# mikhaildubov/AST-text-analysis

Hardware: AMD Instinct MI355X
Metric: corpus chars/sec (SA+annotation build + keyphrase score table) (higher is better)
Workload: dtype u32 (symbols/indices) + f64 (scores); 1 GPU; 1 synthetic 64 MiB random-ASCII word-stream doc(s) per GPU (text mode), 1000 keyphrases, normalized scores, easa-HIP; symbols_per_gpu=61142967, strings_per_gpu=2982949, parallelism=doc-shard x1, all_gather_bytes_per_rank=0

## Files before the change

### ast-text-analysis_amd/csrc/alphabet.h

```cpp
#pragma once
#include "common.h"

#define TEXT_SYMBOLS EAST_HIP_TERMINATOR_START
#define PRESENT_WORDS (TEXT_SYMBOLS / 32)
#define TERM_TAG EAST_HIP_TERMINATOR_TAG
#define HI_SYMBOLS (0x110000u - TEXT_SYMBOLS)
#define HI_WORDS (HI_SYMBOLS / 32u)

__global__ __launch_bounds__(BLOCK) void presence_kernel(const u32 *__restrict__ sym, u32 n, int vec,
                                                         u32 *__restrict__ present)
{
    __shared__ u32 bits[PRESENT_WORDS];
    if (threadIdx.x < PRESENT_WORDS) bits[threadIdx.x] = 0;
    __syncthreads();
    auto mark = [&](u32 c) {
        if (c < TEXT_SYMBOLS && !(((volatile u32 *)bits)[c >> 5] & (1u << (c & 31u))))
            atomicOr(&bits[c >> 5], 1u << (c & 31u));
    };
    const u32 stride = gridDim.x * BLOCK;
    const u32 n4 = vec ? n >> 2 : 0u;
    u32 i = blockIdx.x * BLOCK + threadIdx.x;
    for (; i + 3u * stride < n4; i += 4u * stride) {
        const uint4 a = reinterpret_cast<const uint4 *>(sym)[i], b = reinterpret_cast<const uint4 *>(sym)[i + stride];
        const uint4 c = reinterpret_cast<const uint4 *>(sym)[i + 2u * stride], d = reinterpret_cast<const uint4 *>(sym)[i + 3u * stride];
        mark(a.x); mark(a.y); mark(a.z); mark(a.w);
        mark(b.x); mark(b.y); mark(b.z); mark(b.w);
        mark(c.x); mark(c.y); mark(c.z); mark(c.w);
        mark(d.x); mark(d.y); mark(d.z); mark(d.w);
    }
    for (; i < n4; i += stride) {
        const uint4 c = reinterpret_cast<const uint4 *>(sym)[i];
        mark(c.x); mark(c.y); mark(c.z); mark(c.w);
    }
    for (u32 i = (n4 << 2) + blockIdx.x * BLOCK + threadIdx.x; i < n; i += stride) mark(sym[i]);
    __syncthreads();
    if (threadIdx.x < PRESENT_WORDS && bits[threadIdx.x]) atomicOr(&present[threadIdx.x], bits[threadIdx.x]);
}

#define FLAG_CAPPED 0
#define FLAG_STATUS 1
#define FLAG_SIGMA 2
#define FLAG_KEEP 3
#define FLAG_FAIL 4
#define FLAG_SIGMA_HI 5
#define FLAG_PLACE_FAIL 6
#define FLAG_KG_BAD 7
#define FLAG_SAMPLE 8
#define FLAG_WORDS 32
#define STATUS_NO_TERMINATOR 1u
#define STATUS_N_STRINGS 2u
#define STATUS_SIGMA_GUESS 4u
#define STATUS_BAD_SYMBOL 8u
__device__ __forceinline__ void codemap_block(const u32 *__restrict__ present, u32 assumed, u32 *__restrict__ code_map,
                                              u32 *__restrict__ flags, u32 *__restrict__ guess, int check)
{
    if (guess && threadIdx.x < PRESENT_WORDS) {
        u32 *gp = guess + TEXT_SYMBOLS;
        if (check && gp[threadIdx.x] != present[threadIdx.x]) atomicOr(&flags[FLAG_STATUS], STATUS_SIGMA_GUESS);
        gp[threadIdx.x] = present[threadIdx.x];
    }
    static_assert(TEXT_SYMBOLS == BLOCK * 10, "ten code points per thread");
    __shared__ u32 lds4[WAVES_PER_BLOCK];
    const u32 c0 = threadIdx.x * 10u;
    u32 bits = 0, cnt = 0;
#pragma unroll
    for (u32 i = 0; i < 10; i++) {
        const u32 b = (present[(c0 + i) >> 5] >> ((c0 + i) & 31u)) & 1u;
        bits |= b << i;
        cnt += b;
    }
    u32 total;
    u32 run = block_exclusive_sum(cnt, lds4, total);
#pragma unroll
    for (u32 i = 0; i < 10; i++) {
        const u32 code = ((bits >> i) & 1u) ? ++run : 0u;
        code_map[c0 + i] = code;
        if (guess) guess[c0 + i] = code;
    }
    if (threadIdx.x == 0) {
        flags[FLAG_SIGMA] = total;
        u32 st = 0;
        if (assumed != 0xFFFFFFFFu && assumed != total) st |= STATUS_SIGMA_GUESS;
        if (st) atomicOr(&flags[FLAG_STATUS], st);
    }
}

__global__ __launch_bounds__(BLOCK) void validate_codemap_kernel(const u32 *__restrict__ sym, const u32 *__restrict__ doc_off,
                                                                 u32 n_docs, u32 tagged, const u32 *__restrict__ present,
                                                                 u32 assumed, u32 *__restrict__ code_map,
                                                                 u32 *__restrict__ flags, u32 *__restrict__ guess, int check)
{
    const u32 d = blockIdx.x * BLOCK + threadIdx.x;
    if (d < n_docs) {
        const u32 c = sym[doc_off[d + 1] - 1];
        if (tagged ? !(c >> 31) : c < TEXT_SYMBOLS) atomicOr(&flags[FLAG_STATUS], STATUS_NO_TERMINATOR);
    }
    if (blockIdx.x == 0) codemap_block(present, assumed, code_map, flags, guess, check);
}

#define SAMPLE_N 8192
// ... 256 lines not shown
```

### ast-text-analysis_amd/csrc/build.h

```cpp
#pragma once
#include "dc3.h"
#include "score.h"
#include "tables.h"
#include "upload.h"
#include <chrono>

static bool kgram_reserve(east_hip_index *h, u64 bins, u32 n_docs);

static void annotate(east_hip_index *h, Ctx &ctx, u32 *listed_total = nullptr)
{
    const Pyramid &pyr = h->pyr;
    const u32 n = pyr.len[0];
    Arena &ar = *ctx.arena;
    const size_t mark = ar.mark();
    const u32 n_tiles = ceil_div_u32(n, ANN_TILE);
    u32 *wide_list = ar.alloc<u32>((size_t)n_tiles * ANN_TILE);
    u32 *wide_count = ar.alloc<u32>(n_tiles);
    const bool has_lvl1 = pyr.levels > 1;
    const bool has_lvl2 = pyr.levels > 2;
    LAUNCH(ctx, ann_stream_kernel, n_tiles, pyr.ptr[0], (const u32 *)h->doc_off, (const u32 *)h->n_strings,
           h->build_docs, n, h->ann, has_lvl1 ? (u32 *)pyr.ptr[1] : (u32 *)nullptr, has_lvl1 ? pyr.len[1] : 0u,
           has_lvl1 ? pyr_padded(pyr.len[1]) : 0u, wide_list, wide_count, h->lcp,
           has_lvl2 ? (u32 *)pyr.ptr[2] : (u32 *)nullptr, has_lvl2 ? pyr.len[2] : 0u, has_lvl2 ? pyr_padded(pyr.len[2]) : 0u);
    int l = 3;
// ... 99 lines not shown
    ctx.ht_mean_len = h->ht_mean_len;
}

static void build_impl(east_hip_index *h, Ctx &ctx, const u32 *d_sym, u32 n, u32 n_docs,
                       const i64 *doc_offsets, const int32_t *n_strings, u32 spec_sigma = 0, bool tagged = false)
{
    Arena &ar = *ctx.arena;
    ar.release(0);
    h->s = ar.alloc<u32>((size_t)n + 3);
    h->s8 = ar.alloc<uint8_t>((size_t)n + 64);
    h->sa = ar.alloc<u32>(n);
    h->lcp = ar.alloc<u32>(pyr_padded(n));
    h->ann = ar.alloc<u32>(n);
    h->up = ar.alloc<u32>(n);
    h->down = ar.alloc<u32>(n);
    h->next = ar.alloc<u32>(n);
    h->doc_off = ar.alloc<u32>(2 * (size_t)n_docs + 1);
    h->n_strings = h->doc_off + n_docs + 1;
    constexpr size_t ZEROED_WORDS = FLAG_WORDS + PRESENT_WORDS + 1 + LCP_BUDGET_SLOTS, TOTAL_WORDS = (size_t)RS_TOTAL_SHARDS * RS_BINS;
    h->code_map = ar.alloc<u32>(TEXT_SYMBOLS + ZEROED_WORDS + 3 * TOTAL_WORDS);
    h->hi_bits = tagged ? ar.alloc<u32>(HI_WORDS) : nullptr;
    h->hi_rank = tagged ? ar.alloc<u32>(HI_WORDS) : nullptr;
    Pyramid pyr;
    pyr.levels = 1;
    pyr.ptr[0] = h->lcp;
    pyr.len[0] = n;
    while (pyr.len[pyr.levels - 1] > PYR_FAN) {
        if (pyr.levels >= PYR_MAX_LEVELS) east_throw(EAST_HIP_ERR_INTERNAL, "pyramid too deep");
        const u32 len = ceil_div_u32(pyr.len[pyr.levels - 1], PYR_FAN);
        pyr.ptr[pyr.levels] = ar.alloc<u32>(pyr_padded(len));
        pyr.len[pyr.levels] = len;
        pyr.levels++;
    }
    h->pyr = pyr;
    h->build_docs = n_docs;

    std::vector<u32> off32(2 * (size_t)n_docs + 1);
    u32 longest_doc = ctx.dry ? n : 0;
    if (!ctx.dry) {
        for (u32 d = 0; d <= n_docs; d++) off32[d] = (u32)doc_offsets[d];
        for (u32 d = 0; d < n_docs; d++) longest_doc = std::max(longest_doc, off32[d + 1] - off32[d]);
        for (u32 d = 0; d < n_docs; d++) off32[(size_t)n_docs + 1 + d] = (u32)n_strings[d];
        HIP_CHECK(hipMemcpyAsync(h->doc_off, off32.data(), off32.size() * 4, hipMemcpyHostToDevice, ctx.stream));
    }

    const u32 gn = ceil_div_u32(n, BLOCK);
    u32 sigma_t = TEXT_SYMBOLS - 1, m_total = n;
    u32 sigma_hi = tagged ? HI_SYMBOLS : 0;
    u32 *flags = h->code_map + TEXT_SYMBOLS;
    u32 *capped = flags + FLAG_CAPPED, *status = flags + FLAG_STATUS;
    u32 *present = flags + FLAG_WORDS;
    if (!ctx.dry) HIP_CHECK(hipMemsetAsync(flags, 0, (ZEROED_WORDS + 3 * TOTAL_WORDS) * sizeof(u32), ctx.stream));
    ctx.zeroed_totals = ctx.dry ? nullptr : flags + ZEROED_WORDS + TOTAL_WORDS;
    RsFirstHist first_hist;
    ctx.first_hist = nullptr;
    const Ctx::FirstPassPlan fp = ctx.spec && ctx.knobs.first_hist && n_docs == 1 && !tagged ? h->first_plan : Ctx::FirstPassPlan();
    if (ctx.dry || fp.valid) {
        first_hist.n = n;
        first_hist.n_tiles = ceil_div_u32(n, RS_TILE);
        first_hist.n_groups = ceil_div_u32(first_hist.n_tiles, RS_GROUP);
        first_hist.hist = ar.alloc<u32>((size_t)RS_BINS * first_hist.n_tiles);
        first_hist.group_sum = ar.alloc<u32>((size_t)RS_BINS * first_hist.n_groups);
        first_hist.digit_total = flags + ZEROED_WORDS;
    }
    ctx.lcp_budget.slots = ctx.dry ? nullptr : present + PRESENT_WORDS + 1;
    ctx.lcp_budget.per_slot = std::max<u32>(n / 256u / LCP_BUDGET_SLOTS, 4u);
    ctx.spec_out = flags + FLAG_KEEP;
    ctx.zeroed_word = ctx.dry ? nullptr : flags + FLAG_PLACE_FAIL;
    ctx.spec_fail = flags + FLAG_PLACE_FAIL;
    ctx.kg_bad = ctx.dry ? nullptr : flags + FLAG_KG_BAD;
    {
        const size_t mark = ar.mark();
        u32 *term_ex = ar.alloc<u32>((size_t)n + 1);
        const int vec = ((uintptr_t)d_sym & 15u) == 0;
        const bool fused = ctx.spec && vec && h->guess.p;
        ctx.map_checked = fused && !ctx.dry;
        if (fused && fp.valid && !ctx.dry) {
            first_hist.s8 = h->s8;
            first_hist.key_bytes = fp.key_bytes; first_hist.w = fp.w; first_hist.b = fp.b; first_hist.spare = fp.spare;
            first_hist.term_first = fp.term_first; first_hist.shift = fp.shift; first_hist.mask = fp.mask;
            if (fp.key_bytes == 8)
                LAUNCH_NAMED(ctx, "presence_remap_hist_kernel", (presence_remap_hist_kernel<u64, TextWindowGen<u64>>), first_hist.n_groups,
                             d_sym, n, h->guess.as<const u32>(), present, h->s8,
                             TextWindowGen<u64>{h->s8, n, fp.w, fp.b, fp.spare, fp.term_first, DocKey()}, fp.shift, fp.mask,
                             first_hist.n_tiles, first_hist.hist, first_hist.group_sum, first_hist.digit_total);
            else
                LAUNCH_NAMED(ctx, "presence_remap_hist_kernel", (presence_remap_hist_kernel<u32, TextWindowGen<u32>>), first_hist.n_groups,
                             d_sym, n, h->guess.as<const u32>(), present, h->s8,
                             TextWindowGen<u32>{h->s8, n, fp.w, fp.b, fp.spare, fp.term_first, DocKey()}, fp.shift, fp.mask,
                             first_hist.n_tiles, first_hist.hist, first_hist.group_sum, first_hist.digit_total);
            ctx.first_hist = &first_hist;
        } else if (fused) LAUNCH(ctx, presence_remap_kernel, std::min<u32>(gn, 2048), d_sym, n, h->guess.as<const u32>(), present, h->s8);
        else LAUNCH(ctx, presence_kernel, std::min<u32>(gn, 2048), d_sym, n, vec, present);
        if (tagged) {
            if (!ctx.dry) HIP_CHECK(hipMemsetAsync(h->hi_bits, 0, HI_WORDS * 4, ctx.stream));
            LAUNCH_BLOCK(ctx, presence_hi_kernel, std::min<u32>(ceil_div_u32(n, PRESENCE_HI_THREADS), 256), PRESENCE_HI_THREADS,
                         d_sym, n, h->hi_bits, status);
            LAUNCH(ctx, hi_rank_kernel, 1, (const u32 *)h->hi_bits, h->hi_rank, flags);
        }
        LAUNCH(ctx, validate_codemap_kernel, ceil_div_u32(n_docs, BLOCK), d_sym, (const u32 *)h->doc_off, n_docs, (u32)tagged,
               (const u32 *)present, ctx.spec ? spec_sigma : 0xFFFFFFFFu, h->code_map, flags, h->guess.as<u32>(), (int)fused);
        ctx.sample_n = 0;
        ctx.rep_n = ctx.rep_dup = 0;
        bool sample_plans = false;
        if (!ctx.dry && !ctx.spec && !tagged && n >= 1024u) {
            u32 dl = 0;
            for (u32 d = 1; d < n_docs; d++)
                if (off32[d + 1] - off32[d] > off32[dl + 1] - off32[dl]) dl = d;
            const u32 len = off32[dl + 1] - off32[dl], cnt = std::min<u32>(SAMPLE_N, len);
            sample_plans = n >= 4 * SAMPLE_N && cnt >= SAMPLE_N / 4;
            if (cnt >= 512u)
                LAUNCH_BLOCK(ctx, sample_prefix_kernel, SAMPLE_MAX_L, SAMPLE_THREADS, d_sym, n, off32[dl] + (len - cnt) / 2, cnt,
                             flags + FLAG_SAMPLE);
        }
        if (!ctx.dry) {
            if (ctx.spec) {
                sigma_t = spec_sigma;
            } else {
                u32 hf[FLAG_WORDS];
                HIP_CHECK(hipMemcpyAsync(hf, flags, sizeof(hf), hipMemcpyDeviceToHost, ctx.stream));
                HIP_CHECK(sync_stream(ctx.stream));
                if (hf[FLAG_STATUS] & STATUS_NO_TERMINATOR)
                    east_throw(EAST_HIP_ERR_DOMAIN, tagged ? "a document does not end in a (tagged) string terminator"
                                                           : "a document does not end in a string terminator (>= U+0A00)");
                if (hf[FLAG_STATUS] & STATUS_BAD_SYMBOL)
                    east_throw(EAST_HIP_ERR_DOMAIN, "a symbol is neither a tagged terminator nor a code point < U+110000");
                sigma_t = hf[FLAG_SIGMA];
                sigma_hi = tagged ? hf[FLAG_SIGMA_HI] : 0;
                ctx.sample_n = hf[FLAG_SAMPLE + 2 * SAMPLE_MAX_L];
                for (int l = 1; l <= SAMPLE_MAX_L; l++) {
                    ctx.sample_dup2[l] = hf[FLAG_SAMPLE + 2 * (l - 1)];
                    ctx.sample_dup4[l] = hf[FLAG_SAMPLE + 2 * (l - 1) + 1];
                }
                ctx.rep_n = ctx.sample_n;
                ctx.rep_dup = ctx.sample_dup4[SAMPLE_MAX_L];
                if (!sample_plans) ctx.sample_n = 0;
                if (g_trace && ctx.sample_n) {
                    fprintf(stderr, "[east_hip] sample of %u suffixes, shared prefixes (>= 2 / >= 4 of the sample) by length:", ctx.sample_n);
                    for (int l = 1; l <= SAMPLE_MAX_L; l++) fprintf(stderr, " %d: %u/%u", l, ctx.sample_dup2[l], ctx.sample_dup4[l]);
                    fprintf(stderr, "\n");
                }
            }
// ... 261 lines not shown
    }
    if (sym_on_host) {
        staging = (u32 *)(h->arena.base + (h->arena.cap - (((size_t)n * 4 + 255) & ~(size_t)255)));
        int went = 0;
        if (narrow) {
            static const bool no_bytes = getenv("EAST_HIP_NO_SYMBOL_BYTES") != nullptr;
            bool bytes = !no_bytes && !h->bytes_refused;
            for (u32 i = 0; bytes && i < std::min<u32>(n, 65536u); i++) bytes = sym[i] < 0xFFu || sym[i] >= TEXT_SYMBOLS;
            if (bytes && upload_symbols_narrow<uint8_t>(h, sym, n, staging, (uint8_t *)((char *)staging - narrow_bytes))) went = 2;
            else {
                if (bytes) h->bytes_refused = true;
                (void)upload_symbols_narrow<uint16_t>(h, sym, n, staging, (uint16_t *)((char *)staging - narrow_bytes));
                went = 1;
            }
        } else HIP_CHECK(hipMemcpyAsync(staging, sym, (size_t)n * 4, hipMemcpyHostToDevice, h->stream));
        h->narrow_upload = went;
        sym = staging;
    } else h->narrow_upload = 0;
    h->stats = Stats();
    h->arena.high = 0;
    Ctx ctx = handle_ctx(h, &h->arena, &h->stats);
    ctx.knobs = kn;
    ctx.lean = lean;
    u32 flags[FLAG_WORDS] = {0};
    auto run = [&](bool spec, bool spec_rounds) -> bool {
        ctx.spec = spec;
        ctx.spec_rounds = spec && spec_rounds;
        ctx.plan_wide = spec ? h->plan_wide : -1;
        ctx.plan_fused = spec ? h->plan_fused : -1;
        ctx.plan_ht = spec ? h->plan_ht : -1;
        ctx.plan_persist = spec ? h->plan_persist : -1;
        ctx.did_first = Ctx::FirstPassPlan();
        try {
            build_impl(h, ctx, sym, n, (u32)n_docs, doc_offsets, n_strings, h->hint_sigma, tagged);
        } catch (const SpecAbort &) {
            HIP_CHECK(hipStreamSynchronize(h->stream));
            return false;
        } catch (const EastError &) {
            if (!spec) throw;
            (void)hipStreamSynchronize(h->stream);
            return false;
        }
        HIP_CHECK(hipEventRecord(h->ev1, h->stream));
        HIP_CHECK(hipMemcpyAsync(flags, h->code_map + TEXT_SYMBOLS, sizeof(flags), hipMemcpyDeviceToHost, h->stream));
        HIP_CHECK(sync_stream(h->stream));
        return true;
    };
    HIP_CHECK(hipEventRecord(h->ev0, h->stream));
    const bool speculate = kn.speculate && kn.window_sort && h->hint_valid && h->hint_window && h->hint_sigma <= 254 && !tagged;
    const bool spec_rounds = speculate && h->hint_no_rounds;
    const bool went_through = run(speculate, spec_rounds);
    const bool repeat = speculate && (!went_through || (flags[FLAG_STATUS] & STATUS_SIGMA_GUESS) ||
                                      (spec_rounds && (flags[FLAG_KEEP] || flags[FLAG_FAIL] || flags[FLAG_PLACE_FAIL])));
    if (repeat) {
        if (g_trace) fprintf(stderr, "[east_hip] speculative build guessed wrong: building again\n");
        h->stats = Stats();
        run(false, false);
    }
    const bool map_confirmed = speculate && !repeat && ctx.map_checked;
    const u32 status = flags[FLAG_STATUS];
    if (status & STATUS_NO_TERMINATOR)
        east_throw(EAST_HIP_ERR_DOMAIN, "a document does not end in a string terminator (>= U+0A00)");
    if (flags[FLAG_CAPPED] && !(status & STATUS_N_STRINGS)) {
        finish_capped_lcp(h, ctx);
        HIP_CHECK(hipEventRecord(h->ev1, h->stream));
        HIP_CHECK(hipStreamSynchronize(h->stream));
    }
    if (status & STATUS_N_STRINGS)
        east_throw(EAST_HIP_ERR_DOMAIN, tagged ? "n_strings does not match the tagged terminators found in a document"
                                               : "n_strings does not match the terminators found in a document "
                                                 "(text symbols must be < U+0A00 unless the terminators are tagged)");
    if (flags[FLAG_KG_BAD]) h->kg_marked = false;
    h->hint_valid = !tagged || h->sigma_hi == 0;
    h->hint_sigma = h->sigma_t;
    h->hint_window = h->stats.window_sorted != 0;
    h->plan_wide = h->stats.window_sorted ? ctx.did_wide : -1;
    if (ctx.did_wide && h->stats.first_n > 0 && h->stats.first_kept * 50 < h->stats.first_n) h->plan_wide = -1;
    h->plan_fused = h->stats.window_sorted ? ctx.did_fused : -1;
    h->plan_ht = h->stats.window_sorted ? ctx.did_ht : -1;
    h->plan_persist = h->stats.window_sorted ? ctx.did_persist : -1;
    if (h->stats.first_n > 0 && ((ctx.did_fused && h->stats.first_kept * 20 > h->stats.first_n) ||
                                 (!ctx.did_fused && h->stats.first_kept * 50 < h->stats.first_n)))
        h->plan_fused = -1;
    h->first_plan = h->stats.window_sorted && h->plan_wide >= 0 && h->plan_fused >= 0 ? ctx.did_first : Ctx::FirstPassPlan();
    h->hint_no_rounds = h->stats.window_sorted && h->stats.refine_rounds == 0 && !h->stats.long_repeats;
    h->prof.collect();
    HIP_CHECK(hipEventElapsedTime(&h->last_build_ms, h->ev0, h->ev1));
    h->n = n;
    if (h->n_docs != (u32)n_docs) h->n_kp = 0;
    h->n_docs = (u32)n_docs;
    h->h_doc_off.assign(doc_offsets, doc_offsets + n_docs + 1);
    h->h_n_strings.assign(n_strings, n_strings + n_docs);
    if (map_confirmed) h->map_epoch = map_epoch_before;
    h->built = true;
    ring_pin_later(h);
}
```

### ast-text-analysis_amd/csrc/common.h

```cpp
#pragma once

#include <hip/hip_runtime.h>
#include <stdint.h>
#include <stdio.h>
#include <stdlib.h>
#include <algorithm>
#include <mutex>
#include <string>
#include <type_traits>
#include <vector>

typedef uint32_t u32;
typedef uint64_t u64;
typedef int64_t i64;

#include "../../include/east_hip.h"

#define LCP_DIRECT_CAP (1u << 14)
#define LCP_SOFT_CAP 256u
#define LCP_PARTIAL_BIT 0x80000000u
#define LCP_BUDGET_SLOTS 64u
struct LcpBudget {
    u32 *slots = nullptr;
    u32 per_slot = 0;
// ... 36 lines not shown
        off = end;
        if (off > high) high = off;
        return dry ? (void *)(uintptr_t)(0x1000 + a) : (void *)(base + a);
    }
    template <class T> T *alloc(size_t count) { return (T *)alloc_bytes(count * sizeof(T)); }
};

struct DevBuf {
    char *p = nullptr;
    size_t cap = 0;
    bool try_ensure(size_t bytes, hipStream_t drain = nullptr)
    {
        if (bytes <= cap) return true;
        if (drain) HIP_CHECK(hipStreamSynchronize(drain));
        release();
        void *q = nullptr;
        if (hipMalloc(&q, bytes) != hipSuccess) { (void)hipGetLastError(); return false; }
        p = (char *)q;
        cap = bytes;
        return true;
    }
    void ensure(size_t bytes, const char *what, hipStream_t drain = nullptr)
    {
        if (!try_ensure(bytes, drain))
            east_throw(EAST_HIP_ERR_OOM, "hipMalloc of " + std::to_string(bytes) + " bytes for " + what + " failed");
    }
    void release()
    {
        if (p) (void)hipFree(p);
        p = nullptr;
        cap = 0;
    }
    template <class T> T *as() const { return (T *)p; }
    Arena arena() const
    {
        Arena a;
        a.base = p;
        a.cap = cap;
        return a;
    }
};

struct Stats {
    i64 levels = 0, levels_resolved = 0, refine_rounds = 0, window_sorted = 0, merge_elems = 0, radix_passes = 0, radix_elems = 0, radix_elem_bytes = 0;
    i64 radix_elems_u32 = 0, radix_elems_u64 = 0, radix_passes_u32 = 0, radix_passes_u64 = 0;
    i64 long_repeats = 0;
    i64 lds_sorted = 0;
    i64 first_kept = 0, first_n = 0;
    i64 fused_finish = 0;
    i64 ht_keys = 0;
    i64 seg_sort = 0;
    i64 persist_rounds = 0;
    i64 first_hist_fused = 0;
};

struct Profiler {
    struct Rec { const char *name; hipEvent_t e0, e1; };
    struct Sum { std::string name; i64 count; double ms; };
    std::vector<Rec> recs;
    std::vector<hipEvent_t> pool;
    std::vector<Sum> sums;
    bool enabled = false;
    std::string only;
    bool skipped = false;

    hipEvent_t get()
    {
        if (!pool.empty()) { hipEvent_t e = pool.back(); pool.pop_back(); return e; }
        hipEvent_t e;
        if (hipEventCreate(&e) != hipSuccess) east_throw(EAST_HIP_ERR_HIP, "hipEventCreate failed");
        return e;
    }
    void begin(const char *name, hipStream_t st)
    {
        skipped = !only.empty() && only != name;
        if (skipped) return;
        Rec r{name, get(), get()};
        (void)hipEventRecord(r.e0, st);
        recs.push_back(r);
    }
    void end(hipStream_t st)
    {
        if (!skipped) (void)hipEventRecord(recs.back().e1, st);
    }
    void collect()
    {
        for (auto &r : recs) {
            float ms = 0.f;
            (void)hipEventElapsedTime(&ms, r.e0, r.e1);
            bool found = false;
            for (auto &s : sums)
                if (s.name == r.name) { s.count++; s.ms += ms; found = true; break; }
            if (!found) sums.push_back(Sum{r.name, 1, ms});
            pool.push_back(r.e0);
            pool.push_back(r.e1);
        }
        recs.clear();
    }
    void reset() { collect(); sums.clear(); }
    ~Profiler()
    {
        for (auto &r : recs) { (void)hipEventDestroy(r.e0); (void)hipEventDestroy(r.e1); }
        for (auto e : pool) (void)hipEventDestroy(e);
    }
};

#define SCORE_SCRATCH_BYTES ((size_t)1 << 30)
#define SCORE_GRID_BLOCKS ((u64)1 << 22)
#define TP_RING_SLOT ((size_t)8 << 20)
static int env_int(const char *name, int absent) { const char *v = getenv(name); return v ? atoi(v) : absent; }
struct Knobs {
    bool window_sort = true;
    bool force_lean = false;
    bool force_wide_keys = getenv("EAST_HIP_WIDE_KEYS") != nullptr;
    bool fused_finish = getenv("EAST_HIP_NO_FUSED_FINISH") == nullptr;
    bool force_fused = getenv("EAST_HIP_FORCE_FUSED") != nullptr;
    int ht_mode = env_int("EAST_HIP_HT", -1);
    int seg_mode = env_int("EAST_HIP_SEG", -1);
    bool lds_rounds = getenv("EAST_HIP_NO_LDS_ROUNDS") == nullptr;
    bool fused_classify = getenv("EAST_HIP_NO_FUSED_CLASSIFY") == nullptr;
    bool persist = getenv("EAST_HIP_NO_PERSIST") == nullptr;
    bool persist_large = getenv("EAST_HIP_NO_PERSIST_LARGE") == nullptr;
    bool persist_force_large = getenv("EAST_HIP_PERSIST_FORCE_LARGE") != nullptr;
    int persist_max_wgs = env_int("EAST_HIP_PERSIST_WGS", 0);
    size_t rank_bucket_bytes = (size_t)192 << 20;
    bool speculate = getenv("EAST_HIP_NO_SPECULATION") == nullptr;
    bool first_hist = getenv("EAST_HIP_NO_FIRST_HIST") == nullptr;
    bool kg_pairs = getenv("EAST_HIP_NO_KG_PAIRS") == nullptr;
    bool kg_pairs_forced = false;
    bool score_fused = getenv("EAST_HIP_SCORE_UNFUSED") == nullptr;
    int score_endgame = env_int("EAST_HIP_SCORE_ENDGAME", 1);
    size_t score_scratch_bytes = SCORE_SCRATCH_BYTES;
    u64 score_grid_blocks = SCORE_GRID_BLOCKS;
    i64 tp_stream = getenv("EAST_HIP_TEXT_STREAM") ? atoll(getenv("EAST_HIP_TEXT_STREAM")) : -1;
    int tp_ring = env_int("EAST_HIP_TEXT_RING", -1);
    size_t tp_ring_slot = getenv("EAST_HIP_RING_SLOT") ? std::min<size_t>(TP_RING_SLOT, (size_t)std::max(64, atoi(getenv("EAST_HIP_RING_SLOT")))) : TP_RING_SLOT;
    int term_hash_bits = 0;
    int syn_chunk = 128;
    int top_tile = 64;
    i64 related_chunk = 0;
    i64 cosine_texts_batch = 0;
    u32 plan_epoch = 1;
};
static Knobs g_knobs;
static std::mutex g_knobs_mutex;
static inline Knobs knobs_snapshot()
{
    std::lock_guard<std::mutex> lock(g_knobs_mutex);
    return g_knobs;
}
template <class F> static inline void knobs_update(F f)
{
    std::lock_guard<std::mutex> lock(g_knobs_mutex);
    f(g_knobs);
}

struct Ctx {
    Knobs knobs = knobs_snapshot();
    hipStream_t stream = nullptr;
    Arena *arena = nullptr;
    bool dry = false;
    bool lean = false;
    bool spec = false;
    bool spec_rounds = false;
    u32 *spec_out = nullptr;
    bool map_checked = false;
    u32 *spec_fail = nullptr;
    u32 *zeroed_word = nullptr;
    u32 *zeroed_totals = nullptr;
    const struct RsFirstHist *first_hist = nullptr;
    struct FirstPassPlan {
        bool valid = false;
        int key_bytes = 0, w = 0, b = 0, spare = 0, shift = 0;
        u32 term_first = 0, mask = 0;
    } did_first;
    u32 *kg_bad = nullptr;
    u32 sample_n = 0, sample_dup2[9] = {0}, sample_dup4[9] = {0};
    u32 rep_n = 0, rep_dup = 0;
    int plan_wide = -1, plan_fused = -1;
    int did_wide = 0, did_fused = 0;
    const u32 *ht_enc = nullptr;
    const uint16_t *ht_dec = nullptr;
    int ht_max_len = 0;
    double ht_mean_len = 0.0;
    int plan_ht = -1, did_ht = 0;
    int plan_persist = -1, did_persist = 0;
    int did_seg = 0;
    std::vector<u32> seg_host;
    LcpBudget lcp_budget;
    Stats *stats = nullptr;
    Profiler *prof = nullptr;
};

static bool g_spin_sync = getenv("EAST_HIP_NO_SPIN_SYNC") == nullptr;
static inline hipError_t sync_stream(hipStream_t stream)
{
    if (g_spin_sync) {
        bool waited = false;
        for (int i = 0; i < 20000; i++) {
            const hipError_t e = hipStreamQuery(stream);
            if (e == hipSuccess) {
                if (waited) (void)hipGetLastError();
                return hipSuccess;
            }
            if (e != hipErrorNotReady) return e;
            waited = true;
        }
        (void)hipGetLastError();
    }
    return hipStreamSynchronize(stream);
}

static inline u32 ceil_div_u32(u64 a, u64 b) { return (u32)((a + b - 1) / b); }
static inline int bit_width_u32(u32 x) { int b = 0; while (x) { b++; x >>= 1; } return b; }

#define LAUNCH(ctx, kernel, grid, ...) LAUNCH_NAMED(ctx, #kernel, kernel, grid, __VA_ARGS__)

#define LAUNCH_NAMED(ctx, name, kernel, grid, ...)                                         \
    do {                                                                                   \
        if (!(ctx).dry) {                                                                  \
            const bool _p = (ctx).prof && (ctx).prof->enabled;                             \
            if (_p) (ctx).prof->begin(name, (ctx).stream);                                 \
            hipLaunchKernelGGL(kernel, dim3(grid), dim3(BLOCK), 0, (ctx).stream, __VA_ARGS__); \
            HIP_CHECK(hipGetLastError());                                                  \
            if (_p) (ctx).prof->end((ctx).stream);                                         \
        }                                                                                  \
    } while (0)

// ... 117 lines not shown
```

### ast-text-analysis_amd/csrc/debug_api.h

```cpp
#pragma once

struct DebugScope {
    hipStream_t stream = nullptr;
    Arena arena;
    Stats stats;
    Ctx ctx;
    DebugScope(int device, size_t bytes)
    {
        int c = 0;
        if (hipGetDeviceCount(&c) != hipSuccess || c <= 0)
            east_throw(EAST_HIP_ERR_NO_DEVICE, "no HIP device available (this library has no CPU fallback)");
        if (device < 0 || device >= c) east_throw(EAST_HIP_ERR_NO_DEVICE, "device ordinal out of range");
        use_device_ordinal(device);
        HIP_CHECK(hipStreamCreateWithFlags(&stream, hipStreamNonBlocking));
        void *p = nullptr;
        HIP_CHECK(hipMalloc(&p, bytes));
        arena.base = (char *)p;
        arena.cap = bytes;
        ctx.stream = stream;
        ctx.arena = &arena;
        ctx.stats = &stats;
    }
    ~DebugScope()
    {
// ... 125 lines not shown
    if (!lcp || !doc_off || !n_strings || !up_out || !down_out || !next_out || !left_out || !geometry_out || !listed_out ||
        n64 < 1 || n64 >= (i64)0x7FFFFFF0 || n_docs < 1 || doc_off[0] != 0 || doc_off[n_docs] != n64)
        east_throw(EAST_HIP_ERR_INVALID, "bad child table arguments");
    for (int32_t d = 0; d < n_docs; d++) {
        if (doc_off[d + 1] <= doc_off[d] || doc_off[d + 1] > n64) east_throw(EAST_HIP_ERR_INVALID, "document offsets must increase");
        if (lcp[doc_off[d]] != 0) east_throw(EAST_HIP_ERR_INVALID, "the table must hold 0 at a document's first rank: it bounds the searches");
    }
    for (i64 k = 0; k < n64; k++)
        if (lcp[k] > 0x7FFFFFEFu) east_throw(EAST_HIP_ERR_INVALID, "a value above 0x7FFFFFEF: an LCP value is below n");
    const u32 n = (u32)n64;
    DebugScope sc(device, ((size_t)pyr_padded(n) * 6 + (size_t)n / 8 + (size_t)ceil_div_u32(n, ANN_TILE) * (ANN_TILE + 1) +
                           (size_t)ceil_div_u32(n, CH_TILE) * (CH_TILE + 1) + 2 * (size_t)n_docs) * 4 + (1u << 20));
    Arena &ar = sc.arena;
    east_hip_index h;
    h.up = ar.alloc<u32>(n);
    h.down = ar.alloc<u32>(n);
    h.next = ar.alloc<u32>(n);
    u32 *left = ar.alloc<u32>(n);
    for (u32 *t : {h.up, h.down, h.next, left}) HIP_CHECK(hipMemsetAsync(t, 0xEE, (size_t)n * 4, sc.stream));
    debug_table_handle(sc, h, lcp, n, doc_off, n_docs, n_strings);
    annotate(&h, sc.ctx);
    child_tables(&h, sc.ctx, listed_out);
    for (int32_t d = 0; d < n_docs; d++)
        interval_lefts(&h, sc.ctx, (u32)doc_off[d], (u32)(doc_off[d + 1] - doc_off[d]), left + doc_off[d]);
    HIP_CHECK(hipMemcpyAsync(up_out, h.up, (size_t)n * 4, hipMemcpyDeviceToHost, sc.stream));
    HIP_CHECK(hipMemcpyAsync(down_out, h.down, (size_t)n * 4, hipMemcpyDeviceToHost, sc.stream));
    HIP_CHECK(hipMemcpyAsync(next_out, h.next, (size_t)n * 4, hipMemcpyDeviceToHost, sc.stream));
    HIP_CHECK(hipMemcpyAsync(left_out, left, (size_t)n * 4, hipMemcpyDeviceToHost, sc.stream));
    HIP_CHECK(hipStreamSynchronize(sc.stream));
    geometry_out[0] = CH_TILE;
    geometry_out[1] = CH_HALO;
    geometry_out[2] = CH_NEAR;
    geometry_out[3] = CH_LOCAL;
}

extern "C" {

int east_hip_debug_set_rank_bucket_bytes(int64_t bytes)
{
    if (bytes < 0) return EAST_HIP_ERR_INVALID;
    knobs_update([&](Knobs &k) { k.rank_bucket_bytes = (size_t)bytes; k.plan_epoch++; });
    return EAST_HIP_OK;
}

int east_hip_debug_set_window_sort(int enabled)
{
    knobs_update([&](Knobs &k) {
    k.window_sort = enabled != 0;
    k.force_lean = enabled == 2;
    k.force_wide_keys = enabled == 3 || enabled == 5;
    k.fused_finish = enabled != 4 && enabled != 5 && enabled != 9 && getenv("EAST_HIP_NO_FUSED_FINISH") == nullptr;
    k.force_fused = enabled == 6 || getenv("EAST_HIP_FORCE_FUSED") != nullptr;
    k.ht_mode = enabled == 7 || enabled == 9 ? 1 : enabled == 8 ? 0 : env_int("EAST_HIP_HT", -1);
    k.plan_epoch++;
    });
    return EAST_HIP_OK;
}

int east_hip_debug_set_segmented_sort(int mode)
{
    knobs_update([&](Knobs &k) { k.seg_mode = mode < 0 ? env_int("EAST_HIP_SEG", -1) : (mode != 0); k.plan_epoch++; });
    return EAST_HIP_OK;
}

int east_hip_debug_alphabetic_code(const uint64_t *weights, int32_t n, uint32_t *code, int32_t *len)
{
    if (!weights || !code || !len || n < 1) return EAST_HIP_ERR_INVALID;
    std::vector<u64> w(weights, weights + n);
    std::vector<u32> c;
    std::vector<int> l;
    if (!ht_build_code(w, c, l)) return EAST_HIP_ERR_DOMAIN;
    for (int i = 0; i < n; i++) { code[i] = c[i]; len[i] = l[i]; }
    return EAST_HIP_OK;
}

int east_hip_debug_narrow_symbols(const uint32_t *symbols, int64_t n, uint16_t *out, int vector)
{
    if (!symbols || !out || n < 0) return EAST_HIP_ERR_INVALID;
    if (vector) narrow_symbols(symbols, out, (size_t)n);
    else
        for (int64_t i = 0; i < n; i++) out[i] = symbols[i] < TEXT_SYMBOLS ? (uint16_t)symbols[i] : (uint16_t)SYM_TERMINATOR16;
    return vector && g_have_avx2 ? 1 : EAST_HIP_OK;
}

int east_hip_debug_narrow_symbols8(const uint32_t *symbols, int64_t n, uint8_t *out, int vector)
{
    if (!symbols || !out || n < 0) return EAST_HIP_ERR_INVALID;
    bool ok = true;
    if (vector) ok = narrow_symbols8(symbols, out, (size_t)n);
    else
        for (int64_t i = 0; i < n; i++) { const u32 c = symbols[i]; ok &= !(c >= 0xFFu && c < TEXT_SYMBOLS); out[i] = c < 0xFFu ? (uint8_t)c : (uint8_t)0xFFu; }
    return (ok ? 1 : 0) + (vector && g_have_avx2 ? 2 : 0);
}

int east_hip_debug_set_lds_rounds(int enabled)
{
    knobs_update([&](Knobs &k) {
        k.lds_rounds = enabled != 0;
        k.fused_classify = enabled != 2 && getenv("EAST_HIP_NO_FUSED_CLASSIFY") == nullptr;
        k.persist = enabled == 1 && getenv("EAST_HIP_NO_PERSIST") == nullptr;
    });
    return EAST_HIP_OK;
}

int east_hip_debug_set_persist(int force_large, int max_workgroups)
{
// ... 151 lines not shown
```

### ast-text-analysis_amd/csrc/east_hip.hip

```cpp
#include "common.h"
#include "alphabet.h"
#include "handle.h"
#include "consumer.h"
#include "upload.h"
#include "build.h"
#include "textfront.h"
#include "score_host.h"
#include <string.h>

static thread_local std::string g_last_error;

template <class F> static int guarded(F f)
{
    int rc = EAST_HIP_OK;
    try {
        f();
    } catch (const EastError &e) {
        g_last_error = e.msg;
        rc = e.code;
    } catch (const std::exception &e) {
        g_last_error = e.what();
        rc = EAST_HIP_ERR_INTERNAL;
    }
    restore_device();
// ... 256 lines not shown
        h->arena.release(mark);
    });
}

int east_hip_reset(east_hip_handle_t h)
{
    return guarded([&] {
        if (!h) east_throw(EAST_HIP_ERR_INVALID, "null handle");
        use_device(h);
        HIP_CHECK(hipStreamSynchronize(h->stream));
        h->built = false;
        h->table_scored = false;
        h->n = 0;
        h->n_docs = 0;
        h->n_kp = 0;
        h->n_q = 0;
        h->q_code_epoch = 0;
        h->kg_built = false;
        h->child_built = false;
        h->prep_n = 0;
        h->prep_doc_off.clear();
        h->prep_n_strings.clear();
        h->prep_tagged = false;
        h->tagged_input = false;
        h->sigma_hi = 0;
        h->prof.enabled = false;
        h->prof.only.clear();
        h->plan_wide = h->plan_fused = h->plan_ht = h->plan_persist = -1;
        h->first_plan = Ctx::FirstPassPlan();
        h->ht_valid = false;
        h->stats = Stats();
        const size_t keep = (size_t)64 << 20;
        for (DevBuf *b : h->bufs)
            if (b->cap > keep) b->release();
        for (Consumer *c : h->consumers)
            if (c) c->reset();
    });
}

int east_hip_synchronize(east_hip_handle_t h)
{
    return guarded([&] {
        if (!h) east_throw(EAST_HIP_ERR_INVALID, "null handle");
        use_device(h);
        HIP_CHECK(hipStreamSynchronize(h->stream));
    });
}

void *east_hip_stream(east_hip_handle_t h) { return h ? (void *)h->stream : nullptr; }

int east_hip_build_info(east_hip_handle_t h, int64_t *out, int32_t cap)
{
    if (!h || !out) return EAST_HIP_ERR_INVALID;
    const int64_t v[28] = {h->n, h->n_docs, h->m_total, h->sigma_t, h->bits0, h->stats.levels,
                           (int64_t)h->arena.cap, (int64_t)h->arena.high, h->stats.radix_passes,
                           h->stats.radix_elems, h->stats.radix_elem_bytes, h->stats.radix_passes_u32,
                           h->stats.radix_elems_u32, h->stats.radix_passes_u64, h->stats.radix_elems_u64,
                           h->stats.levels_resolved, h->stats.merge_elems, h->stats.refine_rounds,
                           h->stats.window_sorted, h->stats.lds_sorted, h->stats.fused_finish, h->stats.first_kept,
                           h->stats.first_n, h->stats.ht_keys, h->stats.seg_sort, h->narrow_upload,
                           h->stats.persist_rounds, h->stats.first_hist_fused};
    for (int i = 0; i < 28 && i < cap; i++) out[i] = v[i];
    return 28;
}

int east_hip_profile_enable(east_hip_handle_t h, int on)
{
    if (!h) return EAST_HIP_ERR_INVALID;
    return guarded([&] {
        use_device(h);
        HIP_CHECK(hipStreamSynchronize(h->stream));
        h->prof.reset();
        h->prof.enabled = on != 0;
    });
}

int east_hip_profile_only(east_hip_handle_t h, const char *kernel)
{
    if (!h) return EAST_HIP_ERR_INVALID;
    h->prof.only = kernel ? kernel : "";
    return EAST_HIP_OK;
}

int64_t east_hip_profile_report(east_hip_handle_t h, char *buf, int64_t cap)
{
    if (!h || !buf || cap < 1) return EAST_HIP_ERR_INVALID;
    int cur = -1;
    (void)hipGetDevice(&cur);
    (void)hipSetDevice(h->device);
    (void)hipStreamSynchronize(h->stream);
    h->prof.collect();
    if (cur >= 0 && cur != h->device) (void)hipSetDevice(cur);
    std::string out;
    for (auto &s : h->prof.sums) {
        char line[256];
        snprintf(line, sizeof(line), "%s\t%lld\t%.6f\n", s.name.c_str(), (long long)s.count, s.ms);
        out += line;
    }
    const int64_t nb = (int64_t)out.size() < cap - 1 ? (int64_t)out.size() : cap - 1;
    memcpy(buf, out.data(), (size_t)nb);
    buf[nb] = 0;
    return (int64_t)out.size();
}

int64_t east_hip_plan_arena_bytes(int64_t n_total, int32_t n_docs)
{
    if (n_total < 1 || n_total >= (i64)0x7FFFFFF0 || n_docs < 1) return EAST_HIP_ERR_INVALID;
    int64_t r = EAST_HIP_ERR_INTERNAL;
    guarded([&] { r = (int64_t)plan_arena_bytes((u32)n_total, (u32)n_docs); });
    return r;
}

int64_t east_hip_plan_arena_bytes_lean(int64_t n_total, int32_t n_docs)
{
    if (n_total < 1 || n_total >= (i64)0x7FFFFFF0 || n_docs < 1) return EAST_HIP_ERR_INVALID;
    int64_t r = EAST_HIP_ERR_INTERNAL;
// ... 21 lines not shown
```

### ast-text-analysis_amd/csrc/persist_rounds.h

```cpp
#pragma once
#include "lds_group_sort.h"

#define PR_MAX_ROUNDS 40
#define PR_CTL_BARRIER 0
#define PR_CTL_BAIL 1
#define PR_CTL_ROUNDS 2
#define PR_CTL_ABORT 3
#define PR_CTL_OPEN 8
#ifdef PR_STAMPS
#define PR_CTL_STAMPS (PR_CTL_OPEN + PR_MAX_ROUNDS)
#define PR_CTL_WORDS (PR_CTL_STAMPS + 2 * 8 * PR_MAX_ROUNDS)
#define PR_STAMP(k) do { if (blockIdx.x == 0 && threadIdx.x == 0) ((unsigned long long *)(a.ctl + PR_CTL_STAMPS))[round * 8 + (k)] = wall_clock64(); } while (0)
#else
#define PR_CTL_WORDS (PR_CTL_OPEN + PR_MAX_ROUNDS)
#define PR_STAMP(k) do { } while (0)
#endif
#ifndef PR_FENCE_MODE
#define PR_FENCE_MODE 3
#endif
#define PR_SPIN_LIMIT (1u << 20)

struct PrArgs {
    const u32 *elems, *gstart, *slots;
    u32 m;
    u32 depth;
    int name_bits;
    u32 *name0, *name1;
    u32 *order_g;
    u32 *lcp_hint;
    u32 *ctl;
};

__global__ __launch_bounds__(BLOCK) void persist_names_init_kernel(const u32 *__restrict__ order_g, const u32 *__restrict__ alt,
                                                                   const u64 *__restrict__ keep, u32 n,
                                                                   u32 *__restrict__ name0, u32 *__restrict__ name1)
{
    const u32 i = blockIdx.x * BLOCK + threadIdx.x;
    if (i >= n) return;
    const u32 e = alt && ((keep[i >> 6] >> (i & 63u)) & 1u) ? alt[i] : order_g[i];
    name0[e] = i;
    name1[e] = i;
}

__device__ __forceinline__ void pr_store(u32 *p, u32 v) { __hip_atomic_store(p, v, __ATOMIC_RELAXED, __HIP_MEMORY_SCOPE_AGENT); }
__device__ __forceinline__ u32 pr_load(const u32 *p) { return __hip_atomic_load(p, __ATOMIC_RELAXED, __HIP_MEMORY_SCOPE_AGENT); }

__device__ __forceinline__ bool pr_grid_barrier(u32 *ctl, u32 index, u32 *lds_flag)
{
    asm volatile("s_waitcnt vmcnt(0)" ::: "memory");
    __syncthreads();
    if (threadIdx.x == 0) {
#if PR_FENCE_MODE & 2
        __builtin_amdgcn_fence(__ATOMIC_RELEASE, "agent");
        asm volatile("s_waitcnt vmcnt(0)" ::: "memory");
#endif
        __hip_atomic_fetch_add(&ctl[PR_CTL_BARRIER], 1u, __ATOMIC_RELAXED, __HIP_MEMORY_SCOPE_AGENT);
        const u32 target = gridDim.x * index;
        u32 spins = 0, ok = 1;
        while (__hip_atomic_load(&ctl[PR_CTL_BARRIER], __ATOMIC_RELAXED, __HIP_MEMORY_SCOPE_AGENT) < target) {
            __builtin_amdgcn_s_sleep(4);
            if ((++spins & 63u) == 0u && __hip_atomic_load(&ctl[PR_CTL_ABORT], __ATOMIC_RELAXED, __HIP_MEMORY_SCOPE_AGENT)) { ok = 0; break; }
            if (spins > PR_SPIN_LIMIT) {
                __hip_atomic_store(&ctl[PR_CTL_ABORT], 1u, __ATOMIC_RELAXED, __HIP_MEMORY_SCOPE_AGENT);
                ok = 0;
                break;
            }
        }
#if PR_FENCE_MODE & 1
        __builtin_amdgcn_fence(__ATOMIC_ACQUIRE, "agent");
        asm volatile("s_waitcnt vmcnt(0)" ::: "memory");
#endif
        *lds_flag = ok;
    }
    __syncthreads();
    return *lds_flag != 0u;
}

__device__ __forceinline__ u32 pr_group_start(const u64 *bits, u32 local)
{
    u32 wi = local >> 6;
    u64 x = bits[wi] & (((u64)2 << (local & 63u)) - 1ull);
    while (!x) x = bits[--wi];
    return wi * 64u + 63u - (u32)__builtin_clzll(x);
}

template <int MIN_WAVES>
__global__ __launch_bounds__(LG_THREADS, MIN_WAVES) void refine_persist_kernel(PrArgs a)
{
    __shared__ LgLds lds;
    __shared__ u32 bar_flag, wg_count;
    const u32 lane = lane_id(), w = wave_id();
    const u32 base = blockIdx.x * LG_CHUNK;
// ... 528 lines not shown
```

### ast-text-analysis_amd/csrc/radix_sort.h

```cpp
#pragma once
#include "common.h"
#include "alphabet.h"
#include "scan.h"

#define RS_THREADS 1024
#ifndef RS_IPT
#define RS_IPT 4
#endif
#define RS_TILE (RS_THREADS * RS_IPT)
#define RS_DB 8
#define RS_BINS 256
#ifndef RS_GROUP
#define RS_GROUP 8
#endif
#define RS_HIST_THREADS 256
#ifndef RS_TOTAL_SHARDS
#define RS_TOTAL_SHARDS 8
#endif

#define RS_SEG_MAX_DOCS 65535
struct RsSeg {
    const u32 *group_doc = nullptr;
    const u32 *doc_group0 = nullptr;
    const u32 *doc_off = nullptr;
    u32 n_docs = 0;
    u32 n_groups = 0;
    u32 shards = 1;
    const u32 *big_docs = nullptr;
    u32 n_big = 0;
};
#define RS_SPINE_DOC_GROUPS 64
__device__ __forceinline__ void rs_tile_range(const RsSeg &seg, u32 n, u32 tile, u32 &base, u32 &count)
{
    if (!seg.n_docs) {
        base = tile * (u32)RS_TILE;
        count = n - base < (u32)RS_TILE ? n - base : (u32)RS_TILE;
        return;
    }
    const u32 d = seg.group_doc[tile / RS_GROUP];
    const u32 t_in = tile - seg.doc_group0[d] * RS_GROUP;
    const u32 end = seg.doc_off[d + 1];
    base = seg.doc_off[d] + t_in * (u32)RS_TILE;
    count = base < end ? (end - base < (u32)RS_TILE ? end - base : (u32)RS_TILE) : 0u;
}

template <class K> struct PairSrc {
    static constexpr int MODE = 0;
    const K *keys;
    const u32 *vals;
    __device__ __forceinline__ K key(u32 i) const { return keys[i]; }
    __device__ __forceinline__ u32 val(u32 i) const { return vals[i]; }
};

template <bool CHECK = true> __device__ __forceinline__ void radix_hist_add(u32 *mine, u32 digit)
{
    if constexpr (!CHECK) { atomicAdd(&mine[digit], 1u); return; }
    const u32 first = __builtin_amdgcn_readfirstlane(digit);
    const u64 active = __ballot(1);
    if (__ballot(digit == first) == active) {
        if (digit == first && lane_id() == (u32)(__ffsll((unsigned long long)active) - 1))
            atomicAdd(&mine[first], (u32)__popcll(active));
    } else {
        atomicAdd(&mine[digit], 1u);
    }
}

#ifndef RS_HIST_BATCH
#define RS_HIST_BATCH 8
#endif
#ifndef RS_HIST_COPIES
#define RS_HIST_COPIES 2
#endif
template <class K, class Src, bool CHECK = true>
__global__ __launch_bounds__(RS_HIST_THREADS) void radix_hist_kernel(Src src, u32 n, int shift, u32 mask, u32 n_tiles,
                                                                     u32 *__restrict__ hist, u32 *__restrict__ group_sum,
                                                                     u32 *__restrict__ digit_total, RsSeg seg)
{
    constexpr int UW = RS_HIST_THREADS / WAVE;
    static_assert(RS_HIST_THREADS == RS_BINS, "thread d owns digit d");
    __shared__ u32 bins[RS_GROUP][RS_HIST_COPIES][RS_BINS];
    if constexpr (Src::MODE == 2) src.prepare();
#pragma unroll
    for (int k = 0; k < RS_GROUP; k++)
#pragma unroll
        for (int c = 0; c < RS_HIST_COPIES; c++) bins[k][c][threadIdx.x] = 0;
    __syncthreads();
    const u32 g = blockIdx.x, lane = lane_id();
    const u32 t0 = g * RS_GROUP, t1 = t0 + RS_GROUP < n_tiles ? t0 + RS_GROUP : n_tiles;
    for (u32 tile = t0 + wave_id(); tile < t1; tile += UW) {
        u32 *mine = bins[tile - t0][lane & (RS_HIST_COPIES - 1)];
        u32 base, count;
        rs_tile_range(seg, n, tile, base, count);
        if (count == 0) continue;
        if constexpr (Src::MODE == 0) {
            constexpr u32 PER = 16 / sizeof(K);
            constexpr int LOADS = RS_TILE / (WAVE * PER);
            static_assert(LOADS % RS_HIST_BATCH == 0, "batches of loads");
            if (count == (u32)RS_TILE) {
                const char *p = reinterpret_cast<const char *>(src.keys + base) + 16u * lane;
                for (int j0 = 0; j0 < LOADS; j0 += RS_HIST_BATCH) {
                    uint4 q[RS_HIST_BATCH];
#pragma unroll
                    for (int j = 0; j < RS_HIST_BATCH; j++) __builtin_memcpy(&q[j], p + (size_t)(j0 + j) * WAVE * 16u, 16);
                    __builtin_amdgcn_sched_barrier(0);
#pragma unroll
                    for (int j = 0; j < RS_HIST_BATCH; j++) {
                        if constexpr (sizeof(K) == 8) {
                            const u64 ka = ((u64)q[j].y << 32) | q[j].x, kb = ((u64)q[j].w << 32) | q[j].z;
                            radix_hist_add<CHECK>(mine, (u32)(ka >> shift) & mask);
                            radix_hist_add<CHECK>(mine, (u32)(kb >> shift) & mask);
                        } else {
                            radix_hist_add<CHECK>(mine, (u32)(q[j].x >> shift) & mask);
                            radix_hist_add<CHECK>(mine, (u32)(q[j].y >> shift) & mask);
                            radix_hist_add<CHECK>(mine, (u32)(q[j].z >> shift) & mask);
                            radix_hist_add<CHECK>(mine, (u32)(q[j].w >> shift) & mask);
                        }
                    }
                }
            } else {
                for (u32 i = lane; i < count; i += WAVE) radix_hist_add<CHECK>(mine, (u32)(src.keys[base + i] >> shift) & mask);
            }
        } else if constexpr (Src::MODE == 1) {
            for (u32 i = lane; i < count; i += WAVE) radix_hist_add<CHECK>(mine, (u32)(src.key(base + i) >> shift) & mask);
        } else {
            src.template hist_tile<CHECK>(mine, base, base + count, shift, mask);
        }
    }
    syncthreads_after_lds_atomics();
    u32 run = 0;
#pragma unroll
    for (int k = 0; k < RS_GROUP; k++) {
        if (t0 + k < t1) hist[(size_t)(t0 + k) * RS_BINS + threadIdx.x] = run;
#pragma unroll
        for (int c = 0; c < RS_HIST_COPIES; c++) run += bins[k][c][threadIdx.x];
    }
    group_sum[(size_t)g * RS_BINS + threadIdx.x] = run;
    const u32 row = seg.n_docs ? seg.group_doc[g] * seg.shards + g % seg.shards : g % RS_TOTAL_SHARDS;
    if (run) atomicAdd(&digit_total[(size_t)row * RS_BINS + threadIdx.x], run);
}

#define RS_FIRST_HALO 16u
#ifndef RS_FIRST_PARTS
#define RS_FIRST_PARTS 2
#endif
#define RS_GEN_RUN 8
struct RsFirstHist {
    u32 *hist = nullptr, *group_sum = nullptr, *digit_total = nullptr;
    const uint8_t *s8 = nullptr;
    u32 n = 0, n_tiles = 0, n_groups = 0;
    int key_bytes = 0, w = 0, b = 0, spare = 0;
    u32 term_first = 0;
    int shift = 0;
    u32 mask = 0;
};
template <class Gen> static inline bool rs_first_hist_counted_for(const RsFirstHist &, const Gen &) { return false; }

template <class K, class Gen>
__global__ __launch_bounds__(RS_HIST_THREADS) void presence_remap_hist_kernel(const u32 *__restrict__ sym, u32 n,
                                                                              const u32 *__restrict__ guess, u32 *__restrict__ present,
                                                                              uint8_t *__restrict__ s8, Gen gen, int shift, u32 mask,
                                                                              u32 n_tiles, u32 *__restrict__ hist,
                                                                              u32 *__restrict__ group_sum, u32 *__restrict__ digit_total)
{
    constexpr int UW = RS_HIST_THREADS / WAVE;
    constexpr int PARTS = RS_FIRST_PARTS, SUB = RS_TILE / PARTS;
    constexpr int LOADS = SUB / (WAVE * 4);
    static_assert(SUB * PARTS == RS_TILE && SUB % (WAVE * RS_GEN_RUN) == 0, "stretches of whole runs for every lane");
    static_assert(RS_HIST_THREADS == RS_BINS, "thread d owns digit d");
    static_assert(RS_TILE % (WAVE * RS_GEN_RUN) == 0 && RS_FIRST_HALO % 4 == 0 && RS_FIRST_HALO / 4 <= WAVE, "whole runs, a halo of whole words");
    __shared__ u32 bins[RS_GROUP][RS_HIST_COPIES][RS_BINS];
    __shared__ __attribute__((aligned(16))) u32 tab[TEXT_SYMBOLS / 2];
    __shared__ __attribute__((aligned(16))) u32 bytes[UW][(SUB + RS_FIRST_HALO) / 4];
    typedef uint16_t __attribute__((may_alias)) tab16_t;
    const tab16_t *tab16 = reinterpret_cast<const tab16_t *>(tab);
#pragma unroll
    for (int k = 0; k < RS_GROUP; k++)
#pragma unroll
        for (int c = 0; c < RS_HIST_COPIES; c++) bins[k][c][threadIdx.x] = 0;
    {
        static_assert(TEXT_SYMBOLS % 4 == 0, "whole 16-byte groups");
        constexpr u32 GROUPS = TEXT_SYMBOLS / 4, ROUNDS = (GROUPS + RS_HIST_THREADS - 1) / RS_HIST_THREADS;
        uint4 q[ROUNDS];
#pragma unroll
        for (u32 r = 0; r < ROUNDS; r++) {
            const u32 g = threadIdx.x + r * RS_HIST_THREADS;
            q[r] = reinterpret_cast<const uint4 *>(guess)[g < GROUPS ? g : 0u];
        }
#pragma unroll
        for (u32 r = 0; r < ROUNDS; r++) {
            const u32 g = threadIdx.x + r * RS_HIST_THREADS;
            if (g < GROUPS)
                reinterpret_cast<uint2 *>(tab)[g] = uint2{(q[r].x & 0xFFu) | ((q[r].y & 0xFFu) << 16), (q[r].z & 0xFFu) | ((q[r].w & 0xFFu) << 16)};
        }
    }
    __syncthreads();
    auto mark = [&](u32 c) {
        if (c < TEXT_SYMBOLS) atomicOr(&tab[c >> 1], 0x100u << (16u * (c & 1u)));
    };
    auto word = [&](const uint4 q) -> u32 {
        const u32 vx = tab16[q.x < TEXT_SYMBOLS ? q.x : 0u], vy = tab16[q.y < TEXT_SYMBOLS ? q.y : 0u];
        const u32 vz = tab16[q.z < TEXT_SYMBOLS ? q.z : 0u], vw = tab16[q.w < TEXT_SYMBOLS ? q.w : 0u];
        const u32 bx = q.x < TEXT_SYMBOLS ? vx : 0x1FFu, by = q.y < TEXT_SYMBOLS ? vy : 0x1FFu;
        const u32 bz = q.z < TEXT_SYMBOLS ? vz : 0x1FFu, bw = q.w < TEXT_SYMBOLS ? vw : 0x1FFu;
        if (!(bx & by & bz & bw & 0x100u)) { mark(q.x); mark(q.y); mark(q.z); mark(q.w); }
        return (bx & 0xFFu) | ((by & 0xFFu) << 8) | ((bz & 0xFFu) << 16) | (bw << 24);
    };
    auto code = [&](u32 c) -> u32 {
        if (c >= TEXT_SYMBOLS) return 0xFFu;
        const u32 v = tab16[c];
        if (!(v & 0x100u)) mark(c);
        return v & 0xFFu;
    };
    auto word_slow = [&](u32 g) -> u32 {
        u32 v = 0;
#pragma unroll
        for (u32 k = 0; k < 4; k++) {
            const u64 p = (u64)g * 4u + k;
            if (p < n) v |= code(sym[p]) << (8u * k);
        }
        return v;
    };
    const u32 g = blockIdx.x, lane = lane_id(), n4 = n >> 2;
    const u32 t0 = g * RS_GROUP, t1 = t0 + RS_GROUP < n_tiles ? t0 + RS_GROUP : n_tiles;
    u32 *mine_bytes = bytes[wave_id()];
    u32 *out = reinterpret_cast<u32 *>(s8);
    uint4 q[LOADS];
    auto request = [&](u32 tile, u32 part) {
        const u32 g0 = tile * (u32)(RS_TILE / 4) + part * (u32)(SUB / 4) + lane;
#pragma unroll
        for (int j = 0; j < LOADS; j++) {
            const u32 gi = g0 + (u32)j * WAVE;
            q[j] = gi < n4 ? reinterpret_cast<const uint4 *>(sym)[gi] : uint4{0u, 0u, 0u, 0u};
        }
    };
    u32 tile = t0 + wave_id(), part = 0;
    if (tile < t1) request(tile, 0);
    while (tile < t1) {
        const u32 g0 = tile * (u32)(RS_TILE / 4) + part * (u32)(SUB / 4) + lane;
        const u32 base = tile * (u32)RS_TILE + part * (u32)SUB;
        const u32 count = base < n ? (n - base < (u32)SUB ? n - base : (u32)SUB) : 0u;
#pragma unroll
        for (int j = 0; j < LOADS; j++) {
            const u32 gi = g0 + (u32)j * WAVE;
            u32 v;
            if (gi < n4) { v = word(q[j]); out[gi] = v; }
            else v = word_slow(gi);
            mine_bytes[(u32)j * WAVE + lane] = v;
        }
        if (lane < RS_FIRST_HALO / 4u) {
            const u32 gi = (base + (u32)SUB) / 4u + lane;
            u32 v = 0;
#pragma unroll
            for (u32 k = 0; k < 4; k++) {
                const u64 p = (u64)gi * 4u + k;
                if (p < n) { const u32 c = sym[p]; v |= (c < TEXT_SYMBOLS ? (u32)tab16[c] & 0xFFu : 0xFFu) << (8u * k); }
            }
            mine_bytes[SUB / 4 + lane] = v;
        }
        const u32 next_part = part + 1u < (u32)PARTS ? part + 1u : 0u, next_tile = next_part ? tile : tile + UW;
        if (next_tile < t1) request(next_tile, next_part);
        __builtin_amdgcn_sched_barrier(0);
        __builtin_amdgcn_fence(__ATOMIC_RELEASE, "wavefront");
        __builtin_amdgcn_wave_barrier();
        __builtin_amdgcn_fence(__ATOMIC_ACQUIRE, "wavefront");
        u32 *mine = bins[tile - t0][lane & (RS_HIST_COPIES - 1)];
        for (u32 r0 = lane * RS_GEN_RUN; r0 < count; r0 += WAVE * RS_GEN_RUN) {
            u32 x[6];
            K k[RS_GEN_RUN];
            const uint2 a = *reinterpret_cast<const uint2 *>(&mine_bytes[r0 / 4]), c = *reinterpret_cast<const uint2 *>(&mine_bytes[r0 / 4 + 2]);
            const uint2 e = *reinterpret_cast<const uint2 *>(&mine_bytes[r0 / 4 + 4]);
            x[0] = a.x; x[1] = a.y; x[2] = c.x; x[3] = c.y; x[4] = e.x; x[5] = e.y;
            gen.keys_of_run(x, k);
#pragma unroll
            for (int qq = 0; qq < RS_GEN_RUN; qq++)
                if (r0 + qq < count) radix_hist_add<false>(mine, (u32)(k[qq] >> shift) & mask);
        }
        __builtin_amdgcn_fence(__ATOMIC_RELEASE, "wavefront");
        __builtin_amdgcn_wave_barrier();
        tile = next_tile;
        part = next_part;
    }
    if (blockIdx.x == 0 && threadIdx.x < 20u) {
        const u32 j = (n4 << 2) + threadIdx.x;
        if (j < n) { const u32 c = sym[j]; s8[j] = (uint8_t)(c < TEXT_SYMBOLS ? (u32)tab16[c] & 0xFFu : 0xFFu); }
        else if (j < n + 16u) s8[j] = 0;
    }
    syncthreads_after_lds_atomics();
    u32 run = 0;
#pragma unroll
    for (int k = 0; k < RS_GROUP; k++) {
        if (t0 + k < t1) hist[(size_t)(t0 + k) * RS_BINS + threadIdx.x] = run;
#pragma unroll
        for (int c = 0; c < RS_HIST_COPIES; c++) run += bins[k][c][threadIdx.x];
    }
    group_sum[(size_t)g * RS_BINS + threadIdx.x] = run;
    if (run) atomicAdd(&digit_total[(size_t)(g % RS_TOTAL_SHARDS) * RS_BINS + threadIdx.x], run);
    if (threadIdx.x < PRESENT_WORDS) {
        u32 bits = 0;
#pragma unroll
        for (u32 k = 0; k < 16; k++) {
            const u32 v = tab[threadIdx.x * 16u + k];
            bits |= (((v >> 8) & 1u) | ((v >> 23) & 2u)) << (2u * k);
        }
        if (bits) atomicOr(&present[threadIdx.x], bits);
    }
}

#ifndef RS_SPINE_COLS
#define RS_SPINE_COLS 8
#endif
#define RS_SPINE_PARTS (BLOCK / RS_SPINE_COLS)
#define RS_SPINE_HELD 64u
__global__ __launch_bounds__(BLOCK) void radix_spine_kernel(const u32 *__restrict__ group_sum, u32 n_groups,
                                                            const u32 *__restrict__ digit_total,
                                                            u32 *__restrict__ next_total, u32 *__restrict__ group_prefix,
                                                            RsSeg seg)
{
    static_assert(RS_BINS == BLOCK, "one digit per thread in the scan of the totals");
    __shared__ u32 base_of[RS_BINS];
    __shared__ u32 part_total[RS_SPINE_PARTS][RS_SPINE_COLS];
    __shared__ u32 lds4[WAVES_PER_BLOCK];
    const u32 doc = seg.big_docs ? seg.big_docs[blockIdx.y] : blockIdx.y;
    const u32 g_first = seg.n_docs ? seg.doc_group0[doc] : 0u;
    const u32 g_count = seg.n_docs ? seg.doc_group0[doc + 1] - g_first : n_groups;
    const u32 shards = seg.n_docs ? seg.shards : (u32)RS_TOTAL_SHARDS;
    {
        const size_t row0 = (size_t)doc * shards * RS_BINS;
        u32 t = 0;
        for (u32 k = 0; k < shards; k++) t += digit_total[row0 + k * RS_BINS + threadIdx.x];
        u32 total;
        base_of[threadIdx.x] = block_exclusive_sum(t, lds4, total) + (seg.n_docs ? seg.doc_off[doc] : 0u);
        if (blockIdx.x == 0)
            for (u32 k = 0; k < shards; k++) next_total[row0 + k * RS_BINS + threadIdx.x] = 0;
    }
    const u32 c = threadIdx.x & (RS_SPINE_COLS - 1u), part = threadIdx.x / RS_SPINE_COLS;
    const u32 col = blockIdx.x * RS_SPINE_COLS + c;
    const u32 per = (g_count + RS_SPINE_PARTS - 1u) / RS_SPINE_PARTS;
    const u32 r0 = g_first + (part * per < g_count ? part * per : g_count);
    const u32 r1 = r0 + per < g_first + g_count ? r0 + per : g_first + g_count;
    u32 run = 0;
    if (per <= RS_SPINE_HELD) {
        u32 x[RS_SPINE_HELD];
#pragma unroll
        for (u32 i = 0; i < RS_SPINE_HELD; i++) x[i] = group_sum[(size_t)(r0 + i < r1 ? r0 + i : 0u) * RS_BINS + col];
#pragma unroll
        for (u32 i = 0; i < RS_SPINE_HELD; i++) run += r0 + i < r1 ? x[i] : 0u;
        part_total[part][c] = run;
        __syncthreads();
        u32 before = base_of[col];
        for (u32 k = 0; k < part; k++) before += part_total[k][c];
        run = before;
#pragma unroll
        for (u32 i = 0; i < RS_SPINE_HELD; i++) {
            if (r0 + i < r1) group_prefix[(size_t)(r0 + i) * RS_BINS + col] = run;
            run += x[i];
        }
        return;
    }
#pragma unroll 8
    for (u32 r = r0; r < r1; r++) run += group_sum[(size_t)r * RS_BINS + col];
    part_total[part][c] = run;
    __syncthreads();
    u32 before = base_of[col];
    for (u32 k = 0; k < part; k++) before += part_total[k][c];
    run = before;
#pragma unroll 8
    for (u32 r = r0; r < r1; r++) {
        const u32 v = group_sum[(size_t)r * RS_BINS + col];
        group_prefix[(size_t)r * RS_BINS + col] = run;
        run += v;
    }
}

__global__ __launch_bounds__(BLOCK) void radix_spine_docs_kernel(const u32 *__restrict__ group_sum,
                                                                 const u32 *__restrict__ digit_total,
                                                                 u32 *__restrict__ next_total, u32 *__restrict__ group_prefix,
                                                                 RsSeg seg)
{
    static_assert(RS_BINS == BLOCK, "one digit per thread");
    __shared__ u32 lds4[WAVES_PER_BLOCK];
    const u32 doc = blockIdx.x;
    const u32 g0 = seg.doc_group0[doc], g1 = seg.doc_group0[doc + 1];
    if (g1 - g0 > (u32)RS_SPINE_DOC_GROUPS) return;
    const size_t row0 = (size_t)doc * seg.shards * RS_BINS;
    u32 x[RS_SPINE_DOC_GROUPS];
#pragma unroll
    for (u32 i = 0; i < RS_SPINE_DOC_GROUPS; i++) x[i] = group_sum[(size_t)(g0 + i < g1 ? g0 + i : 0u) * RS_BINS + threadIdx.x];
    u32 t = 0;
    for (u32 k = 0; k < seg.shards; k++) {
        t += digit_total[row0 + k * RS_BINS + threadIdx.x];
        next_total[row0 + k * RS_BINS + threadIdx.x] = 0;
    }
    u32 total;
    u32 run = block_exclusive_sum(t, lds4, total) + seg.doc_off[doc];
#pragma unroll
    for (u32 i = 0; i < RS_SPINE_DOC_GROUPS; i++) {
        if (g0 + i < g1) group_prefix[(size_t)(g0 + i) * RS_BINS + threadIdx.x] = run;
        run += x[i];
    }
}

template <class K> struct ScatterLds {
    alignas(16) K s_keys[RS_TILE];
    u32 wave_cnt[RS_THREADS / WAVE][RS_BINS / 2];
    u32 digit_start[RS_BINS];
    u32 global_base[RS_BINS];
    u32 wsum[RS_THREADS / WAVE];
};

template <class K, class Src, bool FULL>
__device__ __forceinline__ void radix_scatter_tile(ScatterLds<K> &lds, const Src &src, K *__restrict__ keys_out,
                                                   u32 *__restrict__ vals_out, int shift, u32 mask,
                                                   const u32 *__restrict__ hist, const u32 *__restrict__ group_prefix,
                                                   u32 tile, u32 tile_base, u32 tile_count)
{
    constexpr int WAVES = RS_THREADS / WAVE, IPT = RS_IPT, THREADS = RS_THREADS, BINS = RS_BINS, DB = RS_DB;
    constexpr int WAVE_ITEMS = WAVE * IPT;
    u32 *s_vals = reinterpret_cast<u32 *>(lds.s_keys);
    const u32 tid = threadIdx.x, lane = lane_id(), w = wave_id();

    K key[IPT];
    u32 val[IPT];
    if constexpr (Src::MODE != 2) {
#pragma unroll
        for (int j = 0; j < IPT; j++) {
            const u32 local = w * WAVE_ITEMS + j * WAVE + lane;
            const bool valid = FULL || local < tile_count;
            key[j] = valid ? src.key(tile_base + local) : (K)0;
            val[j] = valid ? src.val(tile_base + local) : 0u;
        }
    }
    uint2 out_base = {0u, 0u};
    if (tid < BINS / 2) {
        const uint2 a = reinterpret_cast<const uint2 *>(hist + (size_t)tile * BINS)[tid];
        const uint2 b = reinterpret_cast<const uint2 *>(group_prefix + (size_t)(tile / RS_GROUP) * BINS)[tid];
        out_base = uint2{a.x + b.x, a.y + b.y};
    }
    if constexpr (Src::MODE == 2) {
        src.prepare();
        src.fill_tile(lds.s_keys, tile_base, tile_count);
        __syncthreads();
    }
    for (u32 i = tid; i < WAVES * (BINS / 2); i += THREADS) (&lds.wave_cnt[0][0])[i] = 0;
    __syncthreads();

    u32 slot[IPT];
    if constexpr (Src::MODE == 2) {
#pragma unroll
        for (int j = 0; j < IPT; j++) {
            const u32 local = w * WAVE_ITEMS + j * WAVE + lane;
            key[j] = lds.s_keys[local];
            val[j] = tile_base + local;
        }
    }
#pragma unroll
    for (int j = 0; j < IPT; j++) {
        const u32 local = w * WAVE_ITEMS + j * WAVE + lane;
        const bool valid = FULL || local < tile_count;
        const u32 digit = (u32)(key[j] >> shift) & mask;
        u32 diff_lo = 0, diff_hi = 0;
#pragma unroll
        for (int bit = 0; bit < DB; bit++) {
            const u32 sbit = (u32)__builtin_amdgcn_sbfe((int)digit, (u32)bit, 1u);
            const u64 bal = __ballot((int)sbit < 0);
            diff_lo |= (u32)bal ^ sbit;
            diff_hi |= (u32)(bal >> 32) ^ sbit;
        }
        u64 same = ~(((u64)diff_hi << 32) | diff_lo);
        if (!FULL) {
            same &= __ballot(valid);
            if (!valid) same = 1ull << lane;
        }
        const u32 cnt = (u32)__popcll(same);
        const u32 before = __builtin_amdgcn_mbcnt_hi((u32)(same >> 32), __builtin_amdgcn_mbcnt_lo((u32)same, 0u));
        const int leader = __ffsll((unsigned long long)same) - 1;
        const u32 half = (digit & 1u) * 16u;
        u32 prior = 0;
        if (valid && before == 0) prior = atomicAdd(&lds.wave_cnt[w][digit >> 1], cnt << half);
        prior = (__shfl(prior, leader, WAVE) >> half) & 0xFFFFu;
        slot[j] = prior + before;
    }
    __syncthreads();

    constexpr int PAIRS = BINS / 2;
    u32 tot_lo = 0, tot_hi = 0;
    if (tid < (u32)PAIRS) {
        u32 run = 0;
#pragma unroll
        for (int k = 0; k < WAVES; k++) {
            const u32 c = lds.wave_cnt[k][tid];
            lds.wave_cnt[k][tid] = run;
            run += c;
        }
        tot_lo = run & 0xFFFFu;
        tot_hi = run >> 16;
    }
    const u32 tsum = tot_lo + tot_hi;
    const u32 inc = wave_inclusive_sum(tsum);
    if (lane == 63 && w < (u32)(PAIRS / WAVE)) lds.wsum[w] = inc;
    __syncthreads();
    if (tid < (u32)PAIRS) {
        u32 start = inc - tsum;
#pragma unroll
        for (int k = 0; k < PAIRS / WAVE; k++)
            if ((u32)k < w) start += lds.wsum[k];
        lds.digit_start[2 * tid] = start;
        lds.global_base[2 * tid] = out_base.x - start;
        start += tot_lo;
        lds.digit_start[2 * tid + 1] = start;
        lds.global_base[2 * tid + 1] = out_base.y - start;
    }
    __syncthreads();

#pragma unroll
    for (int j = 0; j < IPT; j++) {
        const u32 local = w * WAVE_ITEMS + j * WAVE + lane;
        if (FULL || local < tile_count) {
            const u32 digit = (u32)(key[j] >> shift) & mask;
            slot[j] = lds.digit_start[digit] + ((lds.wave_cnt[w][digit >> 1] >> ((digit & 1u) * 16u)) & 0xFFFFu) + slot[j];
            lds.s_keys[slot[j]] = key[j];
        }
    }
    __syncthreads();
    u32 dst[IPT];
#pragma unroll
    for (int j = 0; j < IPT; j++) {
        const u32 pos = j * THREADS + tid;
        if (FULL || pos < tile_count) {
            const K k = lds.s_keys[pos];
            dst[j] = lds.global_base[(u32)(k >> shift) & mask] + pos;
            keys_out[dst[j]] = k;
        }
    }
    __syncthreads();
#pragma unroll
    for (int j = 0; j < IPT; j++) {
        const u32 local = w * WAVE_ITEMS + j * WAVE + lane;
        if (FULL || local < tile_count) s_vals[slot[j]] = val[j];
    }
    __syncthreads();
#pragma unroll
    for (int j = 0; j < IPT; j++) {
        const u32 pos = j * THREADS + tid;
        if (FULL || pos < tile_count) vals_out[dst[j]] = s_vals[pos];
    }
}

template <class K, class Src>
__global__ __launch_bounds__(RS_THREADS, (RS_IPT <= 4 ? 8 : 4)) void radix_scatter_kernel(
    Src src, K *__restrict__ keys_out, u32 *__restrict__ vals_out, u32 n, int shift, u32 mask,
    const u32 *__restrict__ hist, const u32 *__restrict__ group_prefix, u32 n_tiles, RsSeg seg)
{
    const u32 per_xcd = (n_tiles + 7u) / 8u;
    const u32 tile = (blockIdx.x & 7u) * per_xcd + (blockIdx.x >> 3);
    if (tile >= n_tiles) return;
    u32 tile_base, tile_count;
    rs_tile_range(seg, n, tile, tile_base, tile_count);
    if (tile_count == 0) return;
    __shared__ ScatterLds<K> lds;
    if (tile_count == (u32)RS_TILE)
        radix_scatter_tile<K, Src, true>(lds, src, keys_out, vals_out, shift, mask, hist, group_prefix, tile, tile_base, tile_count);
    else
        radix_scatter_tile<K, Src, false>(lds, src, keys_out, vals_out, shift, mask, hist, group_prefix, tile, tile_base, tile_count);
}

template <class K> struct SortBufs {
    K *keys[2];
    u32 *vals[2];
};

struct NoGen {
    static constexpr int MODE = 0;
};

static inline int radix_pass_count(int bits) { return (bits + RS_DB - 1) / RS_DB; }

static inline void radix_account(Ctx &ctx, size_t key_bytes, u32 n, bool generated)
{
    if (!ctx.stats) return;
    ctx.stats->radix_passes++;
    if (!generated) {
        ctx.stats->radix_elems += n;
        if (key_bytes == 8) { ctx.stats->radix_elems_u64 += n; ctx.stats->radix_passes_u64++; }
        else { ctx.stats->radix_elems_u32 += n; ctx.stats->radix_passes_u32++; }
    }
    if ((i64)(key_bytes + 4) > ctx.stats->radix_elem_bytes) ctx.stats->radix_elem_bytes = key_bytes + 4;
}

template <class K, class Gen = NoGen>
static int radix_sort_pairs(Ctx &ctx, SortBufs<K> &b, u32 n, int bits, int begin_bit = 0, Gen gen = Gen(), int check_from_bit = 0,
                            RsSeg seg = RsSeg(), const RsFirstHist *pre = nullptr)
{
    constexpr bool HAS_GEN = !std::is_same<Gen, NoGen>::value;
    if (n == 0 || bits <= begin_bit) return 0;
    const u32 n_groups = seg.n_docs ? seg.n_groups : ceil_div_u32(ceil_div_u32(n, RS_TILE), RS_GROUP);
    const u32 n_tiles = seg.n_docs ? n_groups * RS_GROUP : ceil_div_u32(n, RS_TILE);
    const size_t total_words = seg.n_docs ? (size_t)seg.n_docs * seg.shards * RS_BINS : (size_t)RS_TOTAL_SHARDS * RS_BINS;
    const size_t mark = ctx.arena->mark();
    u32 *hist = ctx.arena->alloc<u32>((size_t)RS_BINS * n_tiles);
    u32 *group_sum = ctx.arena->alloc<u32>((size_t)RS_BINS * n_groups);
    u32 *group_prefix = ctx.arena->alloc<u32>((size_t)RS_BINS * n_groups);
    u32 *totals = ctx.arena->alloc<u32>(2 * total_words);
    if (!ctx.dry && !seg.n_docs && ctx.zeroed_totals) {
        totals = ctx.zeroed_totals;
        ctx.zeroed_totals = nullptr;
    } else if (!ctx.dry) HIP_CHECK(hipMemsetAsync(totals, 0, 2 * total_words * sizeof(u32), ctx.stream));
    const bool prof = ctx.prof && ctx.prof->enabled;
    bool counted = false;
    if constexpr (HAS_GEN) {
        counted = pre && !ctx.dry && !seg.n_docs && pre->hist && pre->key_bytes == (int)sizeof(K) && pre->n == n &&
                  pre->n_tiles == n_tiles && pre->n_groups == n_groups && pre->shift == begin_bit &&
                  pre->mask == (1u << std::min(RS_DB, bits - begin_bit)) - 1u && rs_first_hist_counted_for(*pre, gen);
    }
    if (counted && ctx.stats) ctx.stats->first_hist_fused = 1;
    int cur = 0, pass = 0;
    bool first = HAS_GEN;
    for (int shift = begin_bit; shift < bits; shift += RS_DB, pass++) {
        const u32 mask = (1u << std::min(RS_DB, bits - shift)) - 1u;
        const PairSrc<K> src{b.keys[cur], b.vals[cur]};
        const int out = first ? 0 : cur ^ 1;
        u32 *tot = totals + (pass & 1) * total_words, *tot_next = totals + ((pass & 1) ^ 1) * total_words;
        const bool have = first && counted;
        u32 *hist_p = have ? pre->hist : hist, *group_sum_p = have ? pre->group_sum : group_sum;
        if (have) tot = pre->digit_total;
        const char *name_hist = sizeof(K) == 8 ? (first ? "radix_hist_kernel<u64,gen>" : "radix_hist_kernel<u64>")
                                               : (first ? "radix_hist_kernel<u32,gen>" : "radix_hist_kernel<u32>");
        const char *name_scatter = sizeof(K) == 8 ? (first ? "radix_scatter_kernel<u64,gen>" : "radix_scatter_kernel<u64>")
                                                  : (first ? "radix_scatter_kernel<u32,gen>" : "radix_scatter_kernel<u32>");
        if (!ctx.dry && !have) {
            if (prof) ctx.prof->begin(name_hist, ctx.stream);
            const bool check = shift + RS_DB > check_from_bit;
            if constexpr (HAS_GEN) {
                if (first && check)
                    hipLaunchKernelGGL((radix_hist_kernel<K, Gen, true>), dim3(n_groups), dim3(RS_HIST_THREADS), 0, ctx.stream, gen, n,
                                       shift, mask, n_tiles, hist, group_sum, tot, seg);
                else if (first)
                    hipLaunchKernelGGL((radix_hist_kernel<K, Gen, false>), dim3(n_groups), dim3(RS_HIST_THREADS), 0, ctx.stream, gen, n,
                                       shift, mask, n_tiles, hist, group_sum, tot, seg);
            }
            if (!first && check)
                hipLaunchKernelGGL((radix_hist_kernel<K, PairSrc<K>, true>), dim3(n_groups), dim3(RS_HIST_THREADS), 0, ctx.stream, src,
                                   n, shift, mask, n_tiles, hist, group_sum, tot, seg);
            else if (!first)
                hipLaunchKernelGGL((radix_hist_kernel<K, PairSrc<K>, false>), dim3(n_groups), dim3(RS_HIST_THREADS), 0, ctx.stream, src,
                                   n, shift, mask, n_tiles, hist, group_sum, tot, seg);
            HIP_CHECK(hipGetLastError());
            if (prof) ctx.prof->end(ctx.stream);
        }
        if (seg.n_docs) {
            if (seg.n_big < seg.n_docs)
                LAUNCH(ctx, radix_spine_docs_kernel, seg.n_docs, (const u32 *)group_sum_p, (const u32 *)tot, tot_next, group_prefix, seg);
            if (seg.n_big)
                LAUNCH(ctx, radix_spine_kernel, dim3(RS_BINS / RS_SPINE_COLS, seg.n_big), (const u32 *)group_sum_p, n_groups,
                       (const u32 *)tot, tot_next, group_prefix, seg);
        } else {
            LAUNCH(ctx, radix_spine_kernel, dim3(RS_BINS / RS_SPINE_COLS, 1u), (const u32 *)group_sum_p, n_groups, (const u32 *)tot,
                   tot_next, group_prefix, seg);
        }
        if (!ctx.dry) {
            if (prof) ctx.prof->begin(name_scatter, ctx.stream);
            const dim3 grid(8 * ((n_tiles + 7) / 8));
            if constexpr (HAS_GEN) {
                if (first)
                    hipLaunchKernelGGL((radix_scatter_kernel<K, Gen>), grid, dim3(RS_THREADS), 0, ctx.stream, gen, b.keys[out],
                                       b.vals[out], n, shift, mask, (const u32 *)hist_p, (const u32 *)group_prefix, n_tiles, seg);
            }
            if (!first)
                hipLaunchKernelGGL((radix_scatter_kernel<K, PairSrc<K>>), grid, dim3(RS_THREADS), 0, ctx.stream, src, b.keys[out],
                                   b.vals[out], n, shift, mask, (const u32 *)hist_p, (const u32 *)group_prefix, n_tiles, seg);
            HIP_CHECK(hipGetLastError());
            if (prof) ctx.prof->end(ctx.stream);
        }
        cur = out;
        radix_account(ctx, sizeof(K), n, first);
        first = false;
    }
    ctx.arena->release(mark);
    return cur;
}
```

### ast-text-analysis_amd/csrc/window_sort.h

```cpp
#pragma once
#include "common.h"
#include "radix_sort.h"
#include "scan.h"
#include "ht_code.h"
#include <math.h>
#include <algorithm>

__device__ __forceinline__ u32 dc3_sample_pos(u32 t, u32 n0)
{
    return t < n0 ? 3u * t + 1u : 3u * (t - n0) + 2u;
}

__device__ __forceinline__ u32 lvl0_pos(u32 t, u32 n0) { return n0 ? dc3_sample_pos(t, n0) : t; }
#include "lds_group_sort.h"
#include "persist_rounds.h"
static const bool g_trace = getenv("EAST_HIP_TRACE") != nullptr;
struct FusedAbort {};

#define RESOLVE_MAX_LEN 2048

struct DocKey {
    const u32 *doc_off = nullptr;
    u32 n_docs = 1;
    int bits = 0;
// ... 27 lines not shown
struct SegRanks {
    const u32 *doc_off = nullptr;
    u32 n_docs = 0;
};
struct DocHint {
    u32 d0, lo, hi;
};
__device__ __forceinline__ void seg_doc_bounds(const SegRanks &sr, const DocHint &h, u32 j, u32 &lo, u32 &hi)
{
    if (j < h.hi) { lo = h.lo; hi = h.hi; return; }
    u32 d = h.d0 + 1u;
    while (d + 1 < sr.n_docs && j >= sr.doc_off[d + 1]) d++;
    lo = sr.doc_off[d];
    hi = sr.doc_off[d + 1];
}
__device__ __forceinline__ DocHint doc_hint_of_rank(const u32 *__restrict__ doc_off, u32 n_docs, u32 j)
{
    const u32 d = doc_of_rank(doc_off, n_docs, j);
    return DocHint{d, doc_off[d], doc_off[d + 1]};
}

template <class K, int SEG = 2>
__device__ __forceinline__ void kg_mark_key(const KgMark &km, int w, int b, int spare, u32 j, K k, K kp, u32 v,
                                            const DocHint &hint = DocHint{0u, 0u, 0u})
{
    const int top = spare + (w - km.k) * b;
    const bool same = j != 0 && (K)(k >> top) == (K)(kp >> top);
    u32 d = 0, dlo = 0;
    bool by_rank = true;
    if (SEG == 1 || (SEG == 2 && km.by_rank)) {
        if (same && ((u32)(k >> (spare + (w - 1) * b)) & ((1u << b) - 1u)) != km.A - 1u) return;
        d = hint.d0;
        dlo = hint.lo;
        if (j >= hint.hi) {
            d++;
            while (d + 1 < km.n_docs && j >= km.doc_off[d + 1]) d++;
            dlo = km.doc_off[d];
        }
        if (same && j != dlo) return;
    } else {
        if (same) return;
        d = km.n_docs > 1 ? (u32)(k >> (w * b + spare)) : 0u;
        by_rank = false;
    }
    u32 code = 0;
    for (int q = 0; q < km.k; q++) code = code * km.A + ((u32)(k >> (spare + (w - 1 - q) * b)) & ((1u << b) - 1u));
    if (code >= km.bins) return;
    if (!by_rank) dlo = km.n_docs > 1 ? km.doc_off[d] : 0u;
    const u32 jl = j - dlo;
    if (!km.pairs) { km.kg[(size_t)d * (km.bins + 1) + code] = jl; return; }
    reinterpret_cast<uint2 *>(km.kg)[(size_t)d * (km.bins + 1) + code] = uint2{jl, v};
    const int top3 = top + b;
    if (j == 0 || jl == 0 || (K)(k >> top3) != (K)(kp >> top3)) km.kg3[(size_t)d * (km.bins / km.A + 1) + code / km.A] = jl;
}

__global__ __launch_bounds__(BLOCK) void doc_tiles_kernel(const u32 *__restrict__ doc_off, u32 n_docs, u32 n_tiles,
                                                          u32 *__restrict__ tile_doc)
{
    const u32 t = blockIdx.x * BLOCK + threadIdx.x;
    if (t >= n_tiles) return;
    const u32 p = t << DOC_TILE_SHIFT;
    u32 lo = 0, hi = n_docs;
    while (hi - lo > 1) {
        const u32 mid = (lo + hi) >> 1;
        if (doc_off[mid] <= p) lo = mid; else hi = mid;
    }
    tile_doc[t] = lo;
}

template <class K> struct WindowSrc {
    static constexpr int MODE = 1;
    const uint8_t *s8;
    u32 n0;
    int w, b, spare;
    u32 term_first;
    DocKey docs;
    __device__ __forceinline__ K key(u32 u) const
    {
        K key = window(u);
        if (docs.bits) {
            u32 lo = docs.tile_doc[u >> DOC_TILE_SHIFT];
            while (lo + 1 < docs.n_docs && docs.doc_off[lo + 1] <= u) lo++;
            key |= (K)lo << (w * b + spare);
        }
        return key;
    }
    __device__ __forceinline__ K window(u32 u) const
    {
        const u32 p = n0 ? 3u * (u >> 1) + 1u + (u & 1u) : u;
        u64 lo8, hi8;
        __builtin_memcpy(&lo8, s8 + p, 8);
        __builtin_memcpy(&hi8, s8 + p + 8, 8);
        K key = 0;
        bool ended = false;
        for (int i = 0; i < w; i++) {
            const u32 byte = (u32)((i < 8 ? lo8 >> (8 * i) : hi8 >> (8 * (i - 8))) & 0xFFu);
            const u32 x = ended ? 0u : byte;
            ended = ended || x == 0xFFu;
            key = (key << b) | (K)(x == 0xFFu ? term_first : x);
        }
        if (spare > 0) {
            const u32 byte = (u32)((w < 8 ? lo8 >> (8 * w) : hi8 >> (8 * (w - 8))) & 0xFFu);
            const u32 x = ended ? 0u : (byte == 0xFFu ? term_first : byte);
            key = (key << spare) | (K)(x >> (b - spare));
        }
        return key;
    }
    __device__ __forceinline__ u32 val(u32 u) const { return n0 ? ((u & 1u) ? n0 + (u >> 1) : (u >> 1)) : u; }
    __device__ __forceinline__ u32 low_digit(u32 u) const
    {
        const u32 p = n0 ? 3u * (u >> 1) + 1u + (u & 1u) : u;
        u64 lo8, hi8;
        __builtin_memcpy(&lo8, s8 + p, 8);
        __builtin_memcpy(&hi8, s8 + p + 8, 8);
        const u64 zl = ~lo8, zh = ~hi8;
        const u64 tl = (zl - 0x0101010101010101ull) & ~zl & 0x8080808080808080ull;
        const u64 th = (zh - 0x0101010101010101ull) & ~zh & 0x8080808080808080ull;
        const int tpos = tl ? __builtin_ctzll(tl) >> 3 : (th ? 8 + (__builtin_ctzll(th) >> 3) : 16);
        const int m = (8 - spare + b - 1) / b < w ? (8 - spare + b - 1) / b : w;
        u32 acc = 0;
        for (int i = w - m; i < w; i++) {
            const u32 byte = (u32)((i < 8 ? lo8 >> (8 * i) : hi8 >> (8 * (i - 8))) & 0xFFu);
            const u32 x = i > tpos ? 0u : byte;
            acc = (acc << b) | (x == 0xFFu ? term_first : x);
        }
        if (spare > 0) {
            const u32 byte = (u32)((w < 8 ? lo8 >> (8 * w) : hi8 >> (8 * (w - 8))) & 0xFFu);
            const u32 x = w > tpos ? 0u : (byte == 0xFFu ? term_first : byte);
            acc = (acc << spare) | (x >> (b - spare));
        }
        return acc & 255u;
    }
};

#define TW_RUN 8
template <class K> struct TextWindowGen {
    static constexpr int MODE = 2;
    const uint8_t *s8;
    u32 n;
    int w, b, spare;
    u32 term_first;
    DocKey docs;

    __device__ __forceinline__ void prepare() const {}
    template <int RUN = TW_RUN>
    __device__ __forceinline__ void keys_of_run(const u32 (&x)[6], K (&out)[RUN]) const
    {
        const int top = spare + (w - 1) * b;
        const K fmask = ((K)1 << b) - 1;
        K key = 0;
#pragma unroll
        for (int q = RUN + 12; q >= 0; q--) {
            if (q > RUN + w) continue;
            const u32 c = (x[q >> 2] >> ((q & 3) * 8)) & 0xFFu;
            const bool term = c == 0xFFu;
            const K body = key >> spare;
            const K rest = (K)((body >> b) << spare) | (K)((body & fmask) >> (b - spare));
            key = ((K)(term ? term_first : c) << top) | (term ? (K)0 : rest);
            if (q < RUN) out[q] = key;
        }
    }
    __device__ __forceinline__ void load_run(u32 p0, u32 (&x)[6]) const
    {
        uint2 a, c, e;
        __builtin_memcpy(&a, s8 + p0, 8);
        __builtin_memcpy(&c, s8 + p0 + 8, 8);
        __builtin_memcpy(&e, s8 + p0 + 16, 8);
        x[0] = a.x; x[1] = a.y; x[2] = c.x; x[3] = c.y; x[4] = e.x; x[5] = e.y;
    }
    __device__ __forceinline__ void add_docs(u32 p0, K (&out)[TW_RUN]) const
    {
        u32 lo = docs.tile_doc[p0 >> DOC_TILE_SHIFT];
        const int at = w * b + spare;
        while (lo + 1 < docs.n_docs && docs.doc_off[lo + 1] <= p0) lo++;
        u32 next_off = lo + 1 < docs.n_docs ? docs.doc_off[lo + 1] : 0xFFFFFFFFu;
#pragma unroll
        for (int q = 0; q < TW_RUN; q++) {
            while (p0 + q >= next_off) {
                lo++;
                next_off = lo + 1 < docs.n_docs ? docs.doc_off[lo + 1] : 0xFFFFFFFFu;
            }
            out[q] |= (K)lo << at;
        }
    }
    __device__ __forceinline__ void fill_tile(K *s_keys, u32 tile_base, u32 tile_count) const
    {
        if (!docs.bits) {
            constexpr int HALF = TW_RUN / 2;
            for (u32 r = threadIdx.x; r < (u32)RS_TILE / HALF; r += RS_THREADS) {
                if (r * HALF >= tile_count) break;
                u32 x[6];
                K k[HALF];
                load_run(tile_base + r * HALF, x);
                keys_of_run<HALF>(x, k);
                if constexpr (sizeof(K) == 4) *reinterpret_cast<uint4 *>(&s_keys[r * HALF]) = uint4{(u32)k[0], (u32)k[1], (u32)k[2], (u32)k[3]};
                else {
#pragma unroll
                    for (int q = 0; q < HALF; q++) s_keys[r * HALF + q] = k[q];
                }
            }
            return;
        }
        for (u32 r = threadIdx.x; r < (u32)RS_TILE / TW_RUN; r += RS_THREADS) {
            if (r * TW_RUN >= tile_count) break;
            u32 x[6];
            K k[TW_RUN];
            load_run(tile_base + r * TW_RUN, x);
            keys_of_run(x, k);
            if (docs.bits) add_docs(tile_base + r * TW_RUN, k);
#pragma unroll
            for (int q = 0; q < TW_RUN; q++) s_keys[r * TW_RUN + q] = k[q];
        }
    }
    template <bool CHECK = true> __device__ __forceinline__ void hist_tile(u32 *mine, u32 e0, u32 e1, int shift, u32 mask) const
    {
        const bool need_docs = docs.bits && w * b + spare < shift + 12;
        for (u32 p0 = e0 + lane_id() * TW_RUN; p0 < e1; p0 += WAVE * TW_RUN) {
            u32 x[6];
            K k[TW_RUN];
            load_run(p0, x);
            keys_of_run(x, k);
            if (need_docs) add_docs(p0, k);
#pragma unroll
            for (int q = 0; q < TW_RUN; q++)
                if (p0 + q < e1) radix_hist_add<CHECK>(mine, (u32)(k[q] >> shift) & mask);
        }
    }
};

static_assert(TW_RUN == RS_GEN_RUN, "presence_remap_hist_kernel rolls out the same runs");
template <class K> static inline bool rs_first_hist_counted_for(const RsFirstHist &p, const TextWindowGen<K> &g)
{
    return !g.docs.bits && !g.docs.seg.n_docs && p.s8 == g.s8 && p.n == g.n && p.key_bytes == (int)sizeof(K) && p.w == g.w &&
           p.b == g.b && p.spare == g.spare && p.term_first == g.term_first;
}

__device__ __forceinline__ u32 *ht_enc_lds()
{
    __shared__ u32 t[256];
    return t;
}
static_assert(HT_MAX_STREAM / HT_MIN_LEN <= 16, "HtWindowGen looks 16 symbols ahead: a key must not hold more");
template <class K> struct HtWindowGen {
    static constexpr int MODE = 2;
    const uint8_t *s8;
    u32 n;
    int sb;
    const u32 *enc;
    DocKey docs;

    __device__ __forceinline__ void prepare() const
    {
        u32 *t = ht_enc_lds();
        for (u32 i = threadIdx.x; i < 256u; i += blockDim.x) t[i] = enc[i];
        __syncthreads();
    }
    __device__ __forceinline__ void keys_of_run(const u32 (&x)[6], K (&out)[TW_RUN]) const
    {
        const u32 *t = ht_enc_lds();
        K st = 0;
#pragma unroll
        for (int q = 23; q >= 0; q--) {
            const u32 c = (x[q >> 2] >> ((q & 3) * 8)) & 0xFFu;
            const u32 e = t[c];
            const int len = (int)(e & 0xFFu);
            const K rest = c == 0xFFu ? (K)0 : (K)(st >> len);
            st = ((K)(e >> 8) << (sb - len)) | rest;
            if (q < TW_RUN) out[q] = st;
        }
    }
    __device__ __forceinline__ void load_run(u32 p0, u32 (&x)[6]) const
    {
        uint2 a, c, e;
        __builtin_memcpy(&a, s8 + p0, 8);
        __builtin_memcpy(&c, s8 + p0 + 8, 8);
        __builtin_memcpy(&e, s8 + p0 + 16, 8);
        x[0] = a.x; x[1] = a.y; x[2] = c.x; x[3] = c.y; x[4] = e.x; x[5] = e.y;
    }
    __device__ __forceinline__ void add_docs(u32 p0, K (&out)[TW_RUN]) const
    {
        u32 lo = docs.tile_doc[p0 >> DOC_TILE_SHIFT];
        while (lo + 1 < docs.n_docs && docs.doc_off[lo + 1] <= p0) lo++;
        u32 next_off = lo + 1 < docs.n_docs ? docs.doc_off[lo + 1] : 0xFFFFFFFFu;
#pragma unroll
        for (int q = 0; q < TW_RUN; q++) {
            while (p0 + q >= next_off) {
                lo++;
                next_off = lo + 1 < docs.n_docs ? docs.doc_off[lo + 1] : 0xFFFFFFFFu;
            }
            out[q] |= (K)lo << sb;
        }
    }
    __device__ __forceinline__ void fill_tile(K *s_keys, u32 tile_base, u32 tile_count) const
    {
        for (u32 r = threadIdx.x; r < (u32)RS_TILE / TW_RUN; r += RS_THREADS) {
            if (r * TW_RUN >= tile_count) break;
            u32 x[6];
            K k[TW_RUN];
            load_run(tile_base + r * TW_RUN, x);
            keys_of_run(x, k);
            if (docs.bits) add_docs(tile_base + r * TW_RUN, k);
#pragma unroll
            for (int q = 0; q < TW_RUN; q++) s_keys[r * TW_RUN + q] = k[q];
        }
    }
    template <bool CHECK = true> __device__ __forceinline__ void hist_tile(u32 *mine, u32 e0, u32 e1, int shift, u32 mask) const
    {
        const bool need_docs = docs.bits && sb < shift + 12;
        for (u32 p0 = e0 + lane_id() * TW_RUN; p0 < e1; p0 += WAVE * TW_RUN) {
            u32 x[6];
            K k[TW_RUN];
            load_run(p0, x);
            keys_of_run(x, k);
            if (need_docs) add_docs(p0, k);
#pragma unroll
            for (int q = 0; q < TW_RUN; q++)
                if (p0 + q < e1) radix_hist_add<CHECK>(mine, (u32)(k[q] >> shift) & mask);
        }
    }
};

static int lvl0_spare_bits(int used, int key_bits, int bt, int w)
{
    const int total = std::min(radix_pass_count(used) * RS_DB, key_bits);
    return w < 12 ? std::min(total - used, bt - 1) : 0;
}

template <class K> struct KeyNeqWindowIn {
    static constexpr bool HAS_KEYS = true;
    const K *keys;
    K rep_t, ones, highs;
    int ht_sb = 0, ht_wmin = 0;
    const uint16_t *ht_dec = nullptr;
    __device__ __forceinline__ K ht_stream(K k) const
    {
        return ht_sb >= (int)sizeof(K) * 8 ? k : (K)(k << ((int)sizeof(K) * 8 - ht_sb));
    }
    __device__ __forceinline__ int ht_common_bits(K k, K kp) const
    {
        const K d = k ^ kp;
        if (!d) return ht_sb;
        int hb;
        if constexpr (sizeof(K) == 4) hb = 31 - __clz((u32)d); else hb = 63 - __clzll((u64)d);
        return hb >= ht_sb ? -1 : ht_sb - 1 - hb;
    }
    template <class Table> __device__ __forceinline__ HtScan ht_read(K k, K kp, const Table &dec, int tb = 0) const
    {
        const int cb = ht_common_bits(k, kp);
        return ht_scan<K>(ht_stream(k), ht_sb, dec, cb < 0 ? 0 : cb, tb);
    }
    static KeyNeqWindowIn make(const K *keys, int w, int b, int spare, u32 term_first)
    {
        KeyNeqWindowIn f{keys, 0, 0, 0};
        for (int j = 0; j < w; j++) {
            f.rep_t |= (K)term_first << (spare + j * b);
            f.ones |= (K)1 << (spare + j * b);
            f.highs |= (K)1 << (spare + j * b + b - 1);
        }
        return f;
    }
    __device__ __forceinline__ u32 operator()(u32 i) const
    {
        const K k = keys[i];
        if (ht_sb) return (i == 0 || k != keys[i - 1] || ht_read(k, k, ht_dec).term) ? 1u : 0u;
        const K x = k ^ rep_t;
        const bool has_term = ((x - ones) & ~x & highs) != 0;
        return (i == 0 || has_term || k != keys[i - 1]) ? 1u : 0u;
    }
};

__global__ __launch_bounds__(BLOCK) void dc3_scatter_names_kernel(const u32 *__restrict__ vals,
                                                                  const u32 *__restrict__ names,
                                                                  u32 n02, u32 *__restrict__ s12)
// ... 139 lines not shown
            const u64 v = first_step ? ns.k2[x - ns.first] : load_u64_unaligned(s8 + p2 + h);
            const u64 d = u ^ v, z = ~u;
            const u64 tz = (z - 0x0101010101010101ull) & ~z & 0x8080808080808080ull;
            const u32 mism = d ? (u32)__builtin_ctzll(d) >> 3 : 8u;
            const u32 term = tz ? (u32)__builtin_ctzll(tz) >> 3 : 8u;
            if (term < mism) { less = p2 < p; decided = true; h += term; break; }
            if (mism < 8u) { less = ((v >> (8 * mism)) & 0xFFu) < ((u >> (8 * mism)) & 0xFFu); decided = true; h += mism; break; }
        }
        if (!decided) {
            if (lr.mode == 1) atomicOr(&lr.bad[a >> 5], 1u << (a & 31u));
            else atomicOr(fail, 1u);
            return 0;
        }
        if (less) { r++; best = h > best ? h : best; }
    }
    if (lr.mode == 1) return 0;
    const u32 at = a + r;
    const u32 at_g = first ? at : slot[at];
    order_g[at_g] = e;
    if (names_g) names_g[first ? j : slot[j]] = 1;
    if (name_of) name_of[p] = at_g;
    if (lcp_g) {
        if (r > 0) lcp_g[at_g] = best;
        else if (first) lcp_g[at_g] = lcp_first(at);
    }
    return 0;
}

template <class K> __device__ __forceinline__ void fin_load4(const K *p, K (&out)[5])
{
    if constexpr (sizeof(K) == 4) {
        const uint4 q = *reinterpret_cast<const uint4 *>(p);
        out[0] = q.x; out[1] = q.y; out[2] = q.z; out[3] = q.w;
    } else {
        const uint4 q0 = reinterpret_cast<const uint4 *>(p)[0], q1 = reinterpret_cast<const uint4 *>(p)[1];
        out[0] = ((u64)q0.y << 32) | q0.x; out[1] = ((u64)q0.w << 32) | q0.z;
        out[2] = ((u64)q1.y << 32) | q1.x; out[3] = ((u64)q1.w << 32) | q1.z;
    }
}

struct NoLcp {
    __device__ __forceinline__ u32 operator()(u32) const { return 0u; }
};

#define PLACE_IPT 4
template <class K, bool ENDGAME_LIMITS, bool OPTIMISTIC, bool HT = false>
__global__ __launch_bounds__(BLOCK) void lvl0_place_kernel(KeyNeqWindowIn<K> f, const u32 *__restrict__ vals, u32 m,
                                                          const uint8_t *__restrict__ s8, u32 n0, int w, int b,
                                                          int spare, u32 *__restrict__ order_g,
                                                          u32 *__restrict__ names_g, u32 *__restrict__ lcp_g,
                                                          u64 *__restrict__ keep, u32 *__restrict__ block_keep,
                                                          u32 *__restrict__ fail, LongRepeats lr_arg, KgMark km,
                                                          uint8_t *__restrict__ xdep0 = nullptr, SegRanks sr = SegRanks(),
                                                          u32 *__restrict__ spec_keep = nullptr)
{
    const LongRepeats lr = OPTIMISTIC ? LongRepeats() : lr_arg;
    constexpr u32 limit = ENDGAME_LIMITS ? REFINE_ENDGAME_GROUP : REFINE_SMALL_GROUP;
    constexpr u32 max_len = ENDGAME_LIMITS ? REFINE_ENDGAME_LEN : RESOLVE_MAX_LEN;
    __shared__ u32 keep_bits[BLOCK * PLACE_IPT / 32];
    __shared__ u32 work[BLOCK * PLACE_IPT];
    __shared__ u64 next8[BLOCK * PLACE_IPT];
    __shared__ __attribute__((aligned(16))) K key_tile[BLOCK * PLACE_IPT + 2 * PLACE_HALO];
    __shared__ __attribute__((aligned(16))) u32 val_tile[BLOCK * PLACE_IPT + 2 * PLACE_HALO];
    __shared__ u32 n_keep, n_work;
    constexpr int TB_WORDS = (BLOCK * PLACE_IPT + 2 * PLACE_HALO + 31) / 32 + 1;
    __shared__ __attribute__((aligned(16))) uint16_t dec_lds[HT ? HT_DEC_SIZE : 8];
    __shared__ u32 term_bits[HT ? TB_WORDS : 1];
    __shared__ uint8_t dep_tile[HT ? BLOCK * PLACE_IPT : 1];
    __shared__ DocHint kg_hint;
    if (threadIdx.x < BLOCK * PLACE_IPT / 32) keep_bits[threadIdx.x] = 0;
    if (threadIdx.x == 0) { n_keep = 0; n_work = 0; }
    if constexpr (HT) {
        static_assert(HT_DEC_SIZE == BLOCK * 16, "two 16-byte loads per thread");
        const uint4 *src = reinterpret_cast<const uint4 *>(f.ht_dec) + threadIdx.x * 2u;
        const uint4 d0 = src[0], d1 = src[1];
        uint4 *dst = reinterpret_cast<uint4 *>(dec_lds) + threadIdx.x * 2u;
        dst[0] = d0; dst[1] = d1;
        if (threadIdx.x < TB_WORDS) term_bits[threadIdx.x] = 0;
    }
    const u32 j0 = (blockIdx.x * BLOCK + threadIdx.x) * PLACE_IPT;
    u32 my_keep = 0;
    const u32 stretch0 = blockIdx.x * (BLOCK * PLACE_IPT);
    const bool halo_left = threadIdx.x < PLACE_HALO;
    const u32 halo_q = halo_left ? threadIdx.x : threadIdx.x - PLACE_HALO;
    const u64 halo_g = halo_left ? (u64)stretch0 + halo_q - PLACE_HALO : (u64)stretch0 + BLOCK * PLACE_IPT + halo_q;
    const bool has_halo = threadIdx.x < 2 * PLACE_HALO && (!halo_left || stretch0 >= PLACE_HALO) && halo_g < (u64)m + 8;
    const u64 halo_at = has_halo ? halo_g : 0u;
    const K halo_k = f.keys[halo_at];
    const u32 halo_v = vals[halo_at];
    K k[PLACE_IPT + 2];
    u32 v[PLACE_IPT];
    u32 work_mask = 0;
    {
        const u32 jl = j0 < m ? j0 : 0u;
        K k4[5];
        fin_load4<K>(f.keys + jl, k4);
#pragma unroll
        for (int e = 0; e < PLACE_IPT; e++) k[e + 1] = k4[e];
        const uint4 q = *reinterpret_cast<const uint4 *>(vals + jl);
        v[0] = q.x; v[1] = q.y; v[2] = q.z; v[3] = q.w;
        if constexpr (HT) {
            k[0] = jl > 0 ? f.keys[jl - 1] : (K)0;
            k[PLACE_IPT + 1] = f.keys[jl + PLACE_IPT];
        }
    }
    if (threadIdx.x == 0)
        kg_hint = sr.n_docs ? doc_hint_of_rank(sr.doc_off, sr.n_docs, blockIdx.x * (BLOCK * PLACE_IPT)) : DocHint{0u, 0u, 0u};
    __syncthreads();
    if (has_halo) {
        const u32 at = halo_left ? halo_q : PLACE_HALO + BLOCK * PLACE_IPT + halo_q;
        key_tile[at] = halo_k;
// ... 155 lines not shown
        const u32 j = work[i];
        const u32 dep = HT ? (u32)dep_tile[j - stretch] : (u32)w;
        next8[j - stretch] = load_u64_unaligned(s8 + lvl0_pos(val_tile[PLACE_HALO + j - stretch], n0) + dep);
    }
    __syncthreads();
    const NextSymbols ns{next8, stretch, (u32)(BLOCK * PLACE_IPT)};
    const u32 t_first = stretch >= PLACE_HALO ? stretch - PLACE_HALO : stretch;
    const u32 t_skip = stretch >= PLACE_HALO ? 0u : (u32)PLACE_HALO;
    const u64 t_end = std::min<u64>((u64)stretch + BLOCK * PLACE_IPT + PLACE_HALO, (u64)m + 8);
    const u32 t_count = (u32)(t_end - t_first);
    const TileStarts<K> tstarts{f, key_tile + t_skip, t_first, t_count, HT ? term_bits : (const u32 *)nullptr, t_skip};
    const TileElems telems{vals, val_tile + t_skip, t_first, t_count};
    for (u32 i = threadIdx.x; i < todo; i += BLOCK) {
        const u32 j = work[i];
        auto lcp_first = [&](u32 at) -> u32 {
            bool whole;
            if constexpr (HT) return at > 0 ? f.ht_read(tstarts.key(at), tstarts.key(at - 1), dec_lds).common : 0u;
            else return at > 0 ? lvl0_lcp_of_key_pair(f, w, b, spare, tstarts.key(at), tstarts.key(at - 1), whole) : 0u;
        };
        const u32 dep = HT ? (u32)dep_tile[j - stretch] : (u32)w;
        if (lvl0_place_tied(j, telems, tstarts, (const u32 *)nullptr, m, s8, n0, dep, order_g, names_g, lcp_g, lcp_first, fail,
                            limit, max_len, (u32 *)nullptr, lr, ns)) {
            const u32 local = j - blockIdx.x * (BLOCK * PLACE_IPT);
            atomicOr(&keep_bits[local >> 5], 1u << (local & 31u));
            my_keep++;
        }
    }
    my_keep = wave_sum(my_keep);
    if (lane_id() == 0 && my_keep) atomicAdd(&n_keep, my_keep);
    __syncthreads();
    if (threadIdx.x < BLOCK * PLACE_IPT / 64)
        keep[(size_t)blockIdx.x * (BLOCK * PLACE_IPT / 64) + threadIdx.x] =
            ((u64)keep_bits[2 * threadIdx.x + 1] << 32) | keep_bits[2 * threadIdx.x];
    if (threadIdx.x == 0) {
        block_keep[blockIdx.x] = n_keep;
        if (spec_keep && n_keep) spec_keep[0] = 1u;
    }
}

#define FIN_IPT 4
#define FIN_CHUNK (BLOCK * FIN_IPT)
template <int G> struct FinGeom {
    static constexpr int LEFT = G + 4;
    static constexpr int RIGHT = G + 4;
    static constexpr int STAGE = LEFT + FIN_CHUNK + RIGHT;
    static constexpr int WORDS = (STAGE + 31) / 32 + 1;
    static constexpr int SCAN_WORDS = (G + 4 + 31) / 32 + 1;
};

template <class K> struct FinishArgs {
    const K *keys;
    const u32 *vals;
    u32 m;
    const uint8_t *s8;
    int w, b, spare, low_bits;
    u32 inv_b;
    K rep_t, ones, highs;
    K top_mask;
    int kg_top;
    u32 *order_g, *lcp_g;
    u64 *keep, *gstart;
    u32 *block_keep, *fail, *kg_bad;
    u32 *spec_keep = nullptr;
    KgMark km;
    int ht_sb = 0, ht_wmin = 0;
    const uint16_t *ht_dec = nullptr;
    uint8_t *xdep0 = nullptr;
};

template <class GE> __device__ __forceinline__ int fin_prev_bit(const u32 *fl, int i, int lo)
{
    int found = -1;
    int wi = i >> 5;
    u32 word = fl[wi] & (0xFFFFFFFFu >> (31 - (i & 31)));
#pragma unroll
    for (int step = 0; step < GE::SCAN_WORDS; step++) {
        if (found < 0 && word) found = (wi << 5) + 31 - __clz(word);
        if (found < 0 && wi > 0) { wi--; word = fl[wi]; } else word = 0;
    }
    return found >= lo ? found : -1;
}
template <class GE> __device__ __forceinline__ int fin_next_bit(const u32 *fl, int i, int hi)
{
    int found = -1;
    int wi = i >> 5;
    u32 word = fl[wi] & (0xFFFFFFFFu << (i & 31));
#pragma unroll
    for (int step = 0; step < GE::SCAN_WORDS; step++) {
        if (found < 0 && word) found = (wi << 5) + __ffs(word) - 1;
        if (found < 0 && wi + 1 < GE::WORDS) { wi++; word = fl[wi]; } else word = 0;
    }
    return found >= 0 && found <= hi ? found : -1;
}

template <class K>
__device__ __forceinline__ u32 fin_lcp_of_key_pair(const FinishArgs<K> &a, K k, K kp)
{
    const int w = a.w, b = a.b, spare = a.spare;
    const K d = k ^ kp;
    u32 mism = (u32)w;
    if (d) {
        int hb;
        if constexpr (sizeof(K) == 4) hb = 31 - __clz((u32)d); else hb = 63 - __clzll((u64)d);
        if (hb >= spare + w * b) mism = 0;
        else if (hb >= spare) mism = (u32)w - 1u - (((u32)(hb - spare) * a.inv_b) >> 16);
    }
// ... 42 lines not shown
            else h += 4;
        }
        for (; h < depth + max_len && !decided; h += 8) {
            const u64 u = load_u64_unaligned(s8 + p + h), v = load_u64_unaligned(s8 + p2 + h);
            const u64 d = u ^ v, z = ~u;
            const u64 tz = (z - 0x0101010101010101ull) & ~z & 0x8080808080808080ull;
            const u32 mism = d ? (u32)__builtin_ctzll(d) >> 3 : 8u;
            const u32 term = tz ? (u32)__builtin_ctzll(tz) >> 3 : 8u;
            if (term < mism) { less = p2 < p; decided = true; h += term; break; }
            if (mism < 8u) { less = ((v >> (8 * mism)) & 0xFFu) < ((u >> (8 * mism)) & 0xFFu); decided = true; h += mism; break; }
        }
        if (!decided) { atomicOr(a.fail, 1u); return 0; }
        if (less) { r++; best = h > best ? h : best; }
    }
    const int at = lo + (int)r;
    const u32 at_g = base + (u32)at;
    a.order_g[at_g] = p;
    if (a.lcp_g) {
        u32 h = best;
        if (r == 0) {
            if (at_g == 0) h = 0;
            else if (a.ht_sb) {
                const KeyNeqWindowIn<K> hf{nullptr, 0, 0, 0, a.ht_sb, a.ht_wmin, a.ht_dec};
                h = hf.ht_read(kt[at], kt[at - 1], dec8).common;
            } else h = fin_lcp_of_key_pair(a, kt[at], kt[at - 1]);
        }
        a.lcp_g[at_g] = h;
    }
    return 0;
}

template <class K, bool ENDGAME_LIMITS, int FIN_G, bool HT = false, bool SEG = false>
__global__ __launch_bounds__(BLOCK) void lvl0_finish_kernel(FinishArgs<K> a)
{
    using GE = FinGeom<FIN_G>;
    constexpr int FIN_LEFT = GE::LEFT, FIN_STAGE = GE::STAGE, FIN_WORDS = GE::WORDS;
    constexpr u32 limit = ENDGAME_LIMITS ? (REFINE_ENDGAME_GROUP < FIN_G ? REFINE_ENDGAME_GROUP : FIN_G) : REFINE_SMALL_GROUP;
    constexpr u32 max_len = ENDGAME_LIMITS ? REFINE_ENDGAME_LEN : RESOLVE_MAX_LEN;
    constexpr int HELD = FIN_IPT + 1;
    constexpr int G = FIN_G;
    __shared__ __attribute__((aligned(16))) K kt[FIN_STAGE];
    __shared__ __attribute__((aligned(16))) u32 vt[FIN_STAGE];
    __shared__ u32 next4[FIN_STAGE];
    __shared__ uint16_t work[FIN_CHUNK + FIN_G];
    __shared__ u32 fl[FIN_WORDS];
    __shared__ u32 keep_bits[FIN_WORDS], gs_bits[FIN_WORDS];
    __shared__ u32 n_keep, n_work;
    __shared__ DocHint kg_hint;
    __shared__ __attribute__((aligned(16))) uint8_t dec8[HT ? HT_DEC_SIZE : 16];
    __shared__ uint8_t wdep[HT ? FIN_CHUNK + FIN_G : 1];
    const KeyNeqWindowIn<K> hf{a.keys, a.rep_t, a.ones, a.highs, a.ht_sb, a.ht_wmin, a.ht_dec};
    u32 *comp = next4;
    const u32 m = a.m;
    const u32 c0 = blockIdx.x * FIN_CHUNK;
    const u32 base = c0 - FIN_LEFT;
    const int L = a.low_bits;
    const u32 tid = threadIdx.x;
    if (tid < FIN_WORDS) { fl[tid] = 0; keep_bits[tid] = 0; gs_bits[tid] = 0; }
    if (tid == 0) {
        n_keep = 0; n_work = 0;
        if constexpr (SEG) kg_hint = doc_hint_of_rank(a.km.doc_off, a.km.n_docs, c0);
    }
    K key[HELD];
    u32 val[HELD];
    const int i0 = (int)(FIN_LEFT + tid * FIN_IPT);
    const int ih = (int)(FIN_LEFT + FIN_CHUNK + tid);
    const u32 j0 = c0 + tid * FIN_IPT;
    u32 valid = 0;
    {
        if (j0 + FIN_IPT <= m) {
            fin_load4<K>(a.keys + j0, key);
            const uint4 q = *reinterpret_cast<const uint4 *>(a.vals + j0);
            val[0] = q.x; val[1] = q.y; val[2] = q.z; val[3] = q.w;
            valid = 15u;
        } else {
#pragma unroll
            for (int e = 0; e < FIN_IPT; e++) {
                const bool ok = j0 + e < m;
                key[e] = ok ? a.keys[j0 + e] : (K)0;
                val[e] = ok ? a.vals[j0 + e] : 0u;
                valid |= ok ? 1u << e : 0u;
            }
        }
        key[FIN_IPT] = 0; val[FIN_IPT] = 0;
        if (tid <= (u32)G) {
            const u32 jr = c0 + FIN_CHUNK + tid;
            if (jr < m) { key[FIN_IPT] = a.keys[jr]; val[FIN_IPT] = a.vals[jr]; valid |= 16u; }
        }
        K key_l = 0;
        u32 val_l = 0;
        if (tid < (u32)FIN_LEFT) {
            const u32 jl = base + tid;
            if (jl < m) { key_l = a.keys[jl]; val_l = a.vals[jl]; }
        }
        if constexpr (HT) {
            static_assert(HT_DEC_SIZE == BLOCK * 16, "two 16-byte loads per thread");
            const uint4 *src = reinterpret_cast<const uint4 *>(a.ht_dec) + tid * 2u;
            const uint4 d0 = src[0], d1 = src[1];
            auto lows = [](u32 x, u32 y) { return (x & 0xFFu) | ((x >> 8) & 0xFF00u) | ((y & 0xFFu) << 16) | ((y << 8) & 0xFF000000u); };
            *reinterpret_cast<uint4 *>(&dec8[tid * 16u]) = uint4{lows(d0.x, d0.y), lows(d0.z, d0.w), lows(d1.x, d1.y), lows(d1.z, d1.w)};
        }
        if constexpr (sizeof(K) == 4) *reinterpret_cast<uint4 *>(&kt[i0]) = uint4{(u32)key[0], (u32)key[1], (u32)key[2], (u32)key[3]};
        else {
#pragma unroll
            for (int e = 0; e < FIN_IPT; e++) kt[i0 + e] = key[e];
        }
// ... 593 lines not shown
    int sb = 0;
};
template <class K>
static bool dc3_level0_bytes(Ctx &ctx, const uint8_t *s8, u32 n0, u32 n02, int w, int bt, u32 term_first, u32 *sa12,
                             u32 *s12, u32 &n_names, u32 *lcp_out = nullptr, u32 *lcp_capped = nullptr,
                             DocKey docs = DocKey(), KgMark *kg_mark = nullptr, bool allow_fused = false, u32 longest = 0,
                             const HtKeys *ht = nullptr)
{
    Arena &ar = *ctx.arena;
    const u32 g02 = ceil_div_u32((u64)n02 + 1, BLOCK);
    const int ht_sb = ht ? ht->sb : 0;
    const int spare = ht ? 0 : lvl0_spare_bits(w * bt + docs.bits, (int)sizeof(K) * 8, bt, w);
    const int total_bits = ht ? ht_sb + docs.bits : w * bt + spare + docs.bits;
    int depth0 = 0;
    for (int j = 0; j < w; j++)
        if (spare + j * bt >= FIN_LOW_BITS) depth0++;
    if (ht) depth0 = (ht_sb - FIN_LOW_BITS) / ht->max_len;
    bool fused = allow_fused && ctx.knobs.fused_finish && n0 == 0 && total_bits >= 2 * FIN_LOW_BITS && depth0 >= 1;
    bool fin_small_halo = false;
    if (fused && !ctx.dry) {
        if (ctx.knobs.force_fused) {
        } else if (ctx.plan_fused >= 0) {
            fused = ctx.plan_fused != 0;
            fin_small_halo = ctx.plan_fused == 2 && !ht;
        } else if (ht) {
        } else {
            double top_codes = pow((double)term_first, depth0);
            const int part = (spare + (w - depth0) * bt) - FIN_LOW_BITS;
            if (part > 0) top_codes *= std::max(1.0, (double)term_first / (double)(1u << (bt - part)));
            const double expected = (double)(longest ? longest : n02) / top_codes;
            fused = expected <= FIN_MAX_EXPECTED;
            fin_small_halo = expected <= 10.0;
            if (fused && ctx.sample_n && sizeof(K) == 4)
                fused = (u64)ctx.sample_dup4[std::min(depth0 + 1, 8)] * 20u <= ctx.sample_n;
        }
    }
    const int low_bits = fused ? FIN_LOW_BITS : 0;
    if (g_trace && n0 == 0 && !ctx.dry)
        fprintf(stderr, "[east_hip] level-0 keys: %d-bit, w = %d x %d bits + %d spare%s, %d key bits, global passes from bit %d, fused finish %d%s, "
                        "top part holds %d symbols, segmented by document %d\n", (int)sizeof(K) * 8, w, bt, spare, ht ? " (variable-length)" : "",
                total_bits, low_bits, (int)fused, fin_small_halo ? " (halo 32)" : "", depth0, (int)(docs.seg.n_docs != 0));
    if (ht) w = fused ? depth0 : ht_sb / ht->max_len;
    if (n0 == 0) ctx.did_fused = fused ? (fin_small_halo ? 2 : 1) : 0;
    if (ctx.stats && n0 == 0) ctx.stats->fused_finish = fused;
    SortBufs<K> sb;
    const size_t n_alloc = (size_t)(n02 > 56 ? n02 : 56) + 8;
    for (int k = 0; k < 2; k++) { sb.keys[k] = ar.alloc<K>(n_alloc); sb.vals[k] = ar.alloc<u32>(n_alloc); }
    if (docs.bits) {
        const u32 n_dt = (n02 >> DOC_TILE_SHIFT) + 1;
        u32 *tile_doc = ar.alloc<u32>(n_dt);
        LAUNCH(ctx, doc_tiles_kernel, ceil_div_u32(n_dt, BLOCK), docs.doc_off, docs.n_docs, n_dt, tile_doc);
        docs.tile_doc = tile_doc;
    }
    const int r = n0 ? radix_sort_pairs<K, WindowSrc<K>>(ctx, sb, n02, total_bits, 0,
                                                         WindowSrc<K>{s8, n0, w, bt, spare, term_first, docs})
                : ht ? radix_sort_pairs<K, HtWindowGen<K>>(ctx, sb, n02, total_bits, low_bits,
                                                           HtWindowGen<K>{s8, n02, ht_sb, ht->enc, docs},
                                                           docs.bits ? total_bits - docs.bits : total_bits + RS_DB, docs.seg)
                     : radix_sort_pairs<K, TextWindowGen<K>>(ctx, sb, n02, total_bits, low_bits,
                                                             TextWindowGen<K>{s8, n02, w, bt, spare, term_first, docs},
                                                             docs.bits ? total_bits - docs.bits : total_bits + RS_DB, docs.seg,
                                                             ctx.first_hist);
    if (n0 == 0 && !ctx.dry) {
        Ctx::FirstPassPlan &fp = ctx.did_first;
        fp.valid = !ht && !docs.bits && !docs.seg.n_docs && total_bits > low_bits;
        fp.key_bytes = (int)sizeof(K); fp.w = w; fp.b = bt; fp.spare = spare; fp.term_first = term_first;
        fp.shift = low_bits; fp.mask = (1u << std::min(RS_DB, total_bits - low_bits)) - 1u;
    }
    KeyNeqWindowIn<K> starts = KeyNeqWindowIn<K>::make(sb.keys[r], ht ? 0 : w, bt, spare, term_first);
    if (ht) { starts.ht_sb = ht_sb; starts.ht_wmin = w; starts.ht_dec = ht->dec; }
    const u32 *sorted_vals = sb.vals[r];
    u64 *keep = (u64 *)sb.keys[r ^ 1];
    u64 *gstart_bits = ar.alloc<u64>(((size_t)n02 >> 6) + 2);
    u32 *idx = sb.vals[r ^ 1];
    u32 *names_g = s12 ? ar.alloc<u32>(n02) : nullptr;
    u32 *fail = ar.alloc<u32>(1);
    const bool fail_is_zero = ctx.zeroed_word != nullptr;
    if (fail_is_zero) { fail = ctx.zeroed_word; ctx.zeroed_word = nullptr; }
    const u32 gp = ceil_div_u32((u64)n02 + 1, BLOCK * PLACE_IPT);
    u32 *block_keep = ar.alloc<u32>(gp);
    const u32 nb = ceil_div_u32(gp, SCAN_TILE);
    u32 *block_sums = ar.alloc<u32>(nb);
    u32 *bad = ar.alloc<u32>(((size_t)n02 >> 5) + 2);
    uint8_t *xdep0 = ht || ctx.dry ? ar.alloc<uint8_t>((size_t)n02 + 16) : nullptr;
    if (!ctx.dry && !fail_is_zero) HIP_CHECK(hipMemsetAsync(fail, 0, sizeof(u32), ctx.stream));

    KgMark km;
    ClearRegions clears;
    const bool repetitive_text = n0 == 0 && !ctx.dry && ctx.knobs.lds_rounds && ctx.knobs.persist && n02 >= 4u * PR_CTL_WORDS &&
                                 (ctx.rep_n ? ctx.rep_dup * 2u > ctx.rep_n : ctx.plan_persist == 1);
    const bool small_input = n02 <= REFINE_SMALL_INPUT && !repetitive_text;
    if (kg_mark) kg_mark->k = kg_mark->kg && n0 == 0 && !ctx.dry && !small_input && !ht ? kg_mark->k : 0;
    if (kg_mark && kg_mark->k > 0) {
        km = *kg_mark;
        km.k = std::min(km.k, w);
        km.bins = 1;
        for (int i = 0; i < km.k; i++) km.bins *= km.A;
        km.pairs = km.kg3 && km.k >= 2;
        km.by_rank = docs.seg.n_docs != 0;
        clear_add(ctx, clears, km.kg, (size_t)(km.bins + 1) * km.n_docs * (km.pairs ? 8 : 4), 0xFF);
        if (km.pairs) clear_add(ctx, clears, km.kg3, (size_t)(km.bins / km.A + 1) * km.n_docs * sizeof(u32), 0xFF);
        *kg_mark = km;
    }
    u32 m = n02, m_next = n02, h_fail = 0;
    FinishArgs<K> fa;
    const SegRanks sr{docs.seg.n_docs ? docs.seg.doc_off : nullptr, docs.seg.n_docs};
    if (fused) {
        fa.keys = sb.keys[r]; fa.vals = sorted_vals; fa.m = n02; fa.s8 = s8;
        fa.w = w; fa.b = bt; fa.spare = spare; fa.low_bits = low_bits;
        fa.inv_b = (65536u + (u32)bt - 1u) / (u32)bt;
        fa.rep_t = starts.rep_t; fa.ones = starts.ones; fa.highs = starts.highs;
        fa.top_mask = 0;
        for (int j = 0; j < w; j++)
            if (spare + j * bt >= low_bits) fa.top_mask |= (K)(((K)1 << bt) - 1) << (spare + j * bt);
        fa.kg_top = spare + (w - km.k) * bt < low_bits;
        fa.order_g = sa12; fa.lcp_g = lcp_out; fa.keep = keep; fa.gstart = gstart_bits;
        fa.block_keep = block_keep; fa.fail = fail; fa.kg_bad = ctx.kg_bad ? ctx.kg_bad : fail;
        fa.km = small_input ? KgMark() : km;
        if (ht) { fa.ht_sb = ht_sb; fa.ht_wmin = w; fa.ht_dec = ht->dec; fa.xdep0 = xdep0; }
        if (sr.n_docs) { fa.km.by_rank = 1; fa.km.doc_off = sr.doc_off; fa.km.n_docs = sr.n_docs; }
        clear_add(ctx, clears, keep, (((size_t)n02 >> 6) + 2) * sizeof(u64), 0);
        clear_add(ctx, clears, gstart_bits, (((size_t)n02 >> 6) + 2) * sizeof(u64), 0);
    }
    clear_run(ctx, clears);
    const bool spec_direct = ctx.spec_rounds && n0 == 0 && !ctx.dry && ctx.spec_out && fail_is_zero && fail == ctx.spec_fail;
    auto place = [&](int mode) {
        u32 *spec_keep = spec_direct && mode == 0 ? ctx.spec_out : nullptr;
        if (fused) {
            if (mode != 0) throw FusedAbort();
            fa.spec_keep = spec_keep;
            const bool sg = sr.n_docs != 0;
            if (ht && small_input && sg) LAUNCH_NAMED(ctx, "lvl0_finish_kernel", (lvl0_finish_kernel<K, true, 64, true, true>), gp, fa);
            else if (ht && small_input) LAUNCH_NAMED(ctx, "lvl0_finish_kernel", (lvl0_finish_kernel<K, true, 64, true>), gp, fa);
            else if (ht && sg) LAUNCH_NAMED(ctx, "lvl0_finish_kernel", (lvl0_finish_kernel<K, false, 64, true, true>), gp, fa);
            else if (ht) LAUNCH_NAMED(ctx, "lvl0_finish_kernel", (lvl0_finish_kernel<K, false, 64, true>), gp, fa);
            else if (small_input && sg) LAUNCH_NAMED(ctx, "lvl0_finish_kernel", (lvl0_finish_kernel<K, true, 64, false, true>), gp, fa);
            else if (small_input) LAUNCH_NAMED(ctx, "lvl0_finish_kernel", (lvl0_finish_kernel<K, true, 64>), gp, fa);
            else if (fin_small_halo && sg) LAUNCH_NAMED(ctx, "lvl0_finish_kernel", (lvl0_finish_kernel<K, false, 32, false, true>), gp, fa);
            else if (fin_small_halo) LAUNCH_NAMED(ctx, "lvl0_finish_kernel", (lvl0_finish_kernel<K, false, 32>), gp, fa);
            else if (sg) LAUNCH_NAMED(ctx, "lvl0_finish_kernel", (lvl0_finish_kernel<K, false, 64, false, true>), gp, fa);
            else LAUNCH_NAMED(ctx, "lvl0_finish_kernel", (lvl0_finish_kernel<K, false, 64>), gp, fa);
        } else if (ht && small_input)
            LAUNCH_NAMED(ctx, "lvl0_place_kernel", (lvl0_place_kernel<K, true, false, true>), gp, starts, sorted_vals, n02, s8, n0, w,
                         bt, spare, sa12, names_g, lcp_out, keep, block_keep, fail, LongRepeats{bad, mode}, KgMark(), xdep0, sr, spec_keep);
        else if (ht && mode == 0)
            LAUNCH_NAMED(ctx, "lvl0_place_kernel", (lvl0_place_kernel<K, false, true, true>), gp, starts, sorted_vals, n02, s8, n0, w,
                         bt, spare, sa12, names_g, lcp_out, keep, block_keep, fail, LongRepeats{bad, mode}, KgMark(), xdep0, sr, spec_keep);
        else if (ht)
            LAUNCH_NAMED(ctx, "lvl0_place_kernel", (lvl0_place_kernel<K, false, false, true>), gp, starts, sorted_vals, n02, s8, n0, w,
                         bt, spare, sa12, names_g, lcp_out, keep, block_keep, fail, LongRepeats{bad, mode}, KgMark(), xdep0, sr, spec_keep);
        else if (small_input)
            LAUNCH_NAMED(ctx, "lvl0_place_kernel", (lvl0_place_kernel<K, true, false>), gp, starts, sorted_vals, n02, s8, n0, w,
                         bt, spare, sa12, names_g, lcp_out, keep, block_keep, fail, LongRepeats{bad, mode}, KgMark(), (uint8_t *)nullptr, sr, spec_keep);
        else if (mode == 0)
            LAUNCH_NAMED(ctx, "lvl0_place_kernel", (lvl0_place_kernel<K, false, true>), gp, starts, sorted_vals, n02, s8, n0, w,
                         bt, spare, sa12, names_g, lcp_out, keep, block_keep, fail, LongRepeats{bad, mode}, km, (uint8_t *)nullptr, sr, spec_keep);
        else
            LAUNCH_NAMED(ctx, "lvl0_place_kernel", (lvl0_place_kernel<K, false, false>), gp, starts, sorted_vals, n02, s8, n0, w,
                         bt, spare, sa12, names_g, lcp_out, keep, block_keep, fail, LongRepeats{bad, mode}, KgMark(), (uint8_t *)nullptr, sr, spec_keep);
        if (mode == 1 || ctx.dry) return;
        if (ctx.spec_rounds && mode == 0 && n0 == 0) {
            if (!spec_direct)
                LAUNCH(ctx, spec_counts_kernel, ceil_div_u32(gp, SPEC_COUNT_TILE), (const u32 *)block_keep, gp, (const u32 *)fail,
                       ctx.spec_out);
            m_next = 0;
            h_fail = 0;
            return;
        }
        LAUNCH(ctx, (scan_reduce_kernel<ArrIn>), nb, ArrIn{block_keep}, gp, block_sums);
        std::vector<u32> h_sums(nb);
        HIP_CHECK(hipMemcpyAsync(h_sums.data(), block_sums, (size_t)nb * 4, hipMemcpyDeviceToHost, ctx.stream));
        HIP_CHECK(hipMemcpyAsync(&h_fail, fail, 4, hipMemcpyDeviceToHost, ctx.stream));
        HIP_CHECK(sync_stream(ctx.stream));
        m_next = 0;
        for (u32 x : h_sums) m_next += x;
        if (ctx.stats && n0 == 0 && mode == 0) { ctx.stats->first_kept = m_next; ctx.stats->first_n = n02; }
        if (g_trace)
            fprintf(stderr, "[east_hip] level-0 (%s, %u elements, w = %d): %u in large groups%s\n", n0 ? "sample" : "all suffixes",
                    n02, w, m_next, h_fail ? ", a repeat too long to order directly" : "");
    };
    place(0);
    if (ctx.dry) LAUNCH(ctx, (scan_reduce_kernel<ArrIn>), nb, ArrIn{block_keep}, gp, block_sums);
    bool long_repeats = false;
    if (h_fail) {
        if (fused) throw FusedAbort();
        long_repeats = true;
        if (ctx.stats) ctx.stats->long_repeats++;
        LAUNCH(ctx, (dc3_refine_restore_kernel<KeyNeqWindowIn<K>>), g02, sorted_vals, starts, (const u32 *)nullptr, n02, sa12,
               names_g);
        HIP_CHECK(hipMemsetAsync(fail, 0, sizeof(u32), ctx.stream));
        HIP_CHECK(hipMemsetAsync(bad, 0, (((size_t)n02 >> 5) + 2) * sizeof(u32), ctx.stream));
        place(1);
        place(2);
        if (h_fail) east_throw(EAST_HIP_ERR_INTERNAL, "level 0: undecided comparison after the marking pass");
    }
    if (!ctx.dry && m_next == 0) {
        if (ctx.stats) ctx.stats->levels_resolved++;
        return true;
    }

    u32 *lcp_redo = lcp_out ? ar.alloc<u32>((size_t)n02 + 1) : nullptr;
    u32 redo_n = 0;
    bool redo_pending = false, redo_hinted = false;
    bool done = false;
    bool lcp_from_rounds = true;
    if (!ctx.lean) {
        const size_t mark_rounds = ar.mark();
        const u32 cap = n02 + 1;
        u32 *ebuf[3], *sbuf[2], *fbuf[2];
        for (auto &e : ebuf) e = ar.alloc<u32>(cap);
        for (auto &e : sbuf) e = ar.alloc<u32>(cap);
        for (auto &e : fbuf) e = ar.alloc<u32>(cap);
        u32 *gstart = ar.alloc<u32>(cap), *group = ar.alloc<u32>(cap);
        SortBufs<u64> rb;
        for (int k = 0; k < 2; k++) { rb.keys[k] = ar.alloc<u64>(cap); rb.vals[k] = ar.alloc<u32>(cap); }
        u32 *name_of = n0 == 0 ? ar.alloc<u32>(n02) : nullptr;
        uint8_t *xbuf[2] = {nullptr, nullptr};
        if (ht || ctx.dry) for (auto &x : xbuf) x = ar.alloc<uint8_t>((size_t)cap + 16);
        int x_dom = 0;
        bool have_x = false;
        uint2 *cover = ar.alloc<uint2>((size_t)cap / LG_CHUNK + 2);
        u32 *sub_idx = ar.alloc<u32>((size_t)cap + 1), *full_idx = ar.alloc<u32>(cap);
        u32 *rest_cnt = ar.alloc<u32>((size_t)cap / LG_CHUNK + 3), *rest_pre = ar.alloc<u32>((size_t)cap / LG_CHUNK + 3);
        if (ctx.dry) {
            device_scan<BitIn, false>(ctx, BitIn{keep}, n02 + 1, idx);
            (void)radix_sort_pairs<u64>(ctx, rb, cap, 8);
        }
        bool doubling = false;
        PersistCap persist_caps = ctx.knobs.lds_rounds && ctx.knobs.persist && !ctx.dry ? persist_capacity() : PersistCap();
        if (ctx.knobs.persist_max_wgs > 0) {
            const u32 cap_wgs = (u32)ctx.knobs.persist_max_wgs;
            persist_caps.one_per_cu = std::min(persist_caps.one_per_cu, cap_wgs);
            persist_caps.large = std::min(persist_caps.large, cap_wgs);
        }
        u32 persist_cap = persist_caps.one_per_cu;
        u32 depth = fused ? (u32)depth0 : (u32)w;
        const u32 *elem = fused ? (const u32 *)sa12 : sorted_vals, *slot = nullptr, *flag = nullptr;
        int e_dom = -1, s_dom = 0, f_dom = 0;
        bool have_idx = false;
        int stalled = 0;
        for (int round = 0; !ctx.dry; round++) {
            if (m_next == 0) { done = true; break; }
            stalled = (round > 0 && m_next > m - m / 32) ? stalled + 1 : 0;
            if (round == REFINE_MAX_ROUNDS || (stalled == 2 && !doubling && !name_of)) break;
            const u32 gm = ceil_div_u32((u64)m + 1, BLOCK);
            const bool slow = round > 0 && m_next > m / 2;
            const bool repetitive = repetitive_text;
            const bool try_persist = persist_cap > 0 && name_of && !doubling && n02 >= 4u * PR_CTL_WORDS &&
                                     (m_next <= persist_cap * LG_CHUNK || (persist_caps.large > 0 && ctx.knobs.persist_large)) &&
                                     (n02 <= PERSIST_SMALL_INPUT || n02 / 8u <= m_next) &&
                                     (round == 0 ? repetitive || m_next >= n02 - n02 / 20u : slow);
            if (name_of && !doubling && slow && !try_persist) {
                doubling = true;
                lcp_from_rounds = false;
                redo_pending = lcp_redo != nullptr;
                LAUNCH(ctx, dc3_names_init_kernel, ceil_div_u32(n02, BLOCK), (const u32 *)sa12, n02, name_of);
                device_scan<ArrIn, true>(ctx, ArrIn{flag}, m, group);
                LAUNCH(ctx, dc3_group_starts_kernel, gm, flag, (const u32 *)group, slot, m, gstart);
                LAUNCH(ctx, dc3_names_update_kernel, gm, elem, (const u32 *)group, (const u32 *)gstart, m, (const u64 *)keep,
                       name_of);
                if (g_trace) fprintf(stderr, "[east_hip]   switching to prefix doubling at depth %u\n", depth);
            }
            if (!have_idx) device_scan<PopIn, false>(ctx, PopIn{keep, (m >> 6) + 1u}, (m >> 6) + 2u, idx);
            const int e_c = (e_dom + 4) % 3, e_out = (e_dom + 5) % 3;
            u32 *slot_c = sbuf[s_dom ^ 1];
            const u32 gc = ceil_div_u32((u64)m + 1, BLOCK * COMPACT_IPT);
            const uint8_t *x_in = have_x ? (const uint8_t *)xbuf[x_dom] : !slot && ht ? (const uint8_t *)xdep0 : (const uint8_t *)nullptr;
            uint8_t *x_out = ht && !doubling ? xbuf[x_dom ^ 1] : (uint8_t *)nullptr;
            if (!slot && fused)
                LAUNCH_NAMED(ctx, "dc3_refine_compact_kernel", (dc3_refine_compact_kernel<BitStarts>), gc, elem,
                             BitStarts{gstart_bits}, slot, BitIn{keep}, BitRank{keep, idx}, m, slot_c, ebuf[e_c], gstart,
                             (u32 *)nullptr, 0, 0, 0, x_in, x_out);
            else if (!slot)
                LAUNCH_NAMED(ctx, "dc3_refine_compact_kernel", (dc3_refine_compact_kernel<KeyNeqWindowIn<K>>), gc, elem,
                             starts, slot, BitIn{keep}, BitRank{keep, idx}, m, slot_c, ebuf[e_c], gstart, lcp_out, w, bt, spare,
                             x_in, x_out);
            else
                LAUNCH_NAMED(ctx, "dc3_refine_compact_kernel", (dc3_refine_compact_kernel<FlagArrIn>), gc, elem,
                             FlagArrIn{flag}, slot, BitIn{keep}, BitRank{keep, idx}, m, slot_c, ebuf[e_c], gstart,
                             (u32 *)nullptr, 0, 0, 0, x_in, x_out);
            if (x_out) { x_dom ^= 1; have_x = true; } else have_x = false;
            if (redo_pending) {
                HIP_CHECK(hipMemcpyAsync(lcp_redo, slot_c, (size_t)m_next * 4, hipMemcpyDeviceToDevice, ctx.stream));
                redo_n = m_next;
                redo_pending = false;
            }
            const uint8_t *xdep = have_x ? (const uint8_t *)xbuf[x_dom] : (const uint8_t *)nullptr;
            m = m_next;
            if (try_persist) {
                u32 *name1 = (u32 *)rb.keys[0], *ctl = rb.vals[0];
                HIP_CHECK(hipMemsetAsync(ctl, 0, PR_CTL_WORDS * sizeof(u32), ctx.stream));
                LAUNCH(ctx, persist_names_init_kernel, ceil_div_u32(n02, BLOCK), (const u32 *)sa12,
                       !slot && !fused ? sorted_vals : (const u32 *)nullptr, (const u64 *)keep, n02, name_of, name1);
                const int name_bits = bit_width_u32(n02 > 1 ? n02 - 1 : 1);
                const PrArgs pa{ebuf[e_c], gstart, slot_c, m, depth, name_bits, name_of, name1, sa12, lcp_redo ? lcp_out : (u32 *)nullptr, ctl};
                const u32 tiles = ceil_div_u32(m, LG_CHUNK);
                const Pr2Args pa2{ebuf[e_c], slot_c, gstart, full_idx, m, depth, name_bits, name_of, sa12, lcp_redo ? lcp_out : (u32 *)nullptr,
                                  ctl, cover, rest_cnt, tiles};
                u32 h_ctl[4] = {0, 0, 0, 0};
                {
                    std::lock_guard<std::mutex> lock(g_persist_mutex);
                    const bool force_large = ctx.knobs.persist_force_large && persist_caps.large > 0;
                    if (tiles <= persist_caps.one_per_cu && !force_large) LAUNCH_BLOCK(ctx, refine_persist_kernel<4>, tiles, LG_THREADS, pa);
                    else LAUNCH_BLOCK(ctx, refine_persist2_kernel, std::min(tiles, persist_caps.large), LG_THREADS, pa2);
                    HIP_CHECK(hipMemcpyAsync(h_ctl, ctl, sizeof(h_ctl), hipMemcpyDeviceToHost, ctx.stream));
                    HIP_CHECK(sync_stream(ctx.stream));
                }
                if (h_ctl[PR_CTL_ABORT])
                    east_throw(EAST_HIP_ERR_INTERNAL, h_ctl[PR_CTL_ABORT] == 2 ? "persistent rounds: groups still open after the last round"
                                                                                : "persistent rounds: a grid barrier timed out");
                if (g_trace)
                    fprintf(stderr, "[east_hip]   round %d: persistent launch over a domain of %u at depth %u: %s\n", round, m, depth,
                            h_ctl[PR_CTL_BAIL] ? "a group too long for a tile, the rounds go on launch by launch" : "done");
                if (h_ctl[PR_CTL_BAIL] && slow) persist_cap = 0;
#ifdef PR_STAMPS
                if (g_trace && !h_ctl[PR_CTL_BAIL]) {
                    std::vector<unsigned long long> st(8 * PR_MAX_ROUNDS);
                    HIP_CHECK(hipMemcpy(st.data(), ctl + PR_CTL_STAMPS, st.size() * 8, hipMemcpyDeviceToHost));
                    for (u32 r = 0; r < h_ctl[PR_CTL_ROUNDS]; r++) {
                        auto d = [&](int x, int y) { return (double)(long long)(st[r * 8 + x] - st[r * 8 + y]) * 0.01; };
                        fprintf(stderr, "[east_hip]     round %u (block 0): gather+test %.2f us, sort %.2f, bounds %.2f, held loads %.2f, names+stores %.2f, count %.2f, barrier %.2f\n",
                                r, d(1, 0), d(2, 1), d(5, 2), d(6, 5), d(7, 6), d(3, 7), d(4, 3));
                    }
                    const u32 nwg = ceil_div_u32(m, LG_CHUNK);
                    std::vector<unsigned long long> ab(2 * (size_t)nwg);
                    HIP_CHECK(hipMemcpy(ab.data(), ctl + PR_CTL_WORDS, ab.size() * 8, hipMemcpyDeviceToHost));
                    if (h_ctl[PR_CTL_ROUNDS] > 3) {
                        unsigned long long t0 = ~0ull;
                        for (u32 b = 0; b < nwg; b++) t0 = std::min(t0, ab[2 * b]);
                        fprintf(stderr, "[east_hip]     round 3, arrival / departure of every 16th block (us after the first arrival):");
                        for (u32 b = 0; b < nwg; b += 16) fprintf(stderr, " %u:%.1f/%.1f", b, (ab[2 * b] - t0) * 0.01, (ab[2 * b + 1] - t0) * 0.01);
                        double mx = 0; u32 who = 0;
                        for (u32 b = 0; b < nwg; b++) if ((ab[2 * b] - t0) * 0.01 > mx) { mx = (ab[2 * b] - t0) * 0.01; who = b; }
                        fprintf(stderr, "\n[east_hip]     last arrival: block %u at %.1f us\n", who, mx);
                    }
                }
#endif
                if (!h_ctl[PR_CTL_BAIL]) {
                    if (ctx.stats) {
                        ctx.stats->refine_rounds += h_ctl[PR_CTL_ROUNDS];
                        ctx.stats->persist_rounds += h_ctl[PR_CTL_ROUNDS];
                        ctx.stats->lds_sorted += (i64)m * h_ctl[PR_CTL_ROUNDS];
                    }
                    if (lcp_redo) {
                        HIP_CHECK(hipMemcpyAsync(lcp_redo, slot_c, (size_t)m * 4, hipMemcpyDeviceToDevice, ctx.stream));
                        redo_n = m;
// ... 272 lines not shown
```

### ast-text-analysis_amd/east/hip_backend.py

```python
import atexit
import ctypes
import os

import numpy as np

from east import exceptions

_HERE = os.path.dirname(os.path.abspath(__file__))
LIB_PATH = os.environ.get("EAST_HIP_LIBRARY", os.path.join(_HERE, "_lib", "libeast_hip.so"))

_c_i64p = ctypes.POINTER(ctypes.c_int64)
_c_i32p = ctypes.POINTER(ctypes.c_int32)
_c_u32p = ctypes.POINTER(ctypes.c_uint32)
_c_u64p = ctypes.POINTER(ctypes.c_uint64)
_c_dblp = ctypes.POINTER(ctypes.c_double)

SIGNATURES = {
    "east_hip_version": (ctypes.c_char_p, []),
    "east_hip_last_error": (ctypes.c_char_p, []),
    "east_hip_device_count": (ctypes.c_int, []),
    "east_hip_create": (ctypes.c_int, [ctypes.c_int, ctypes.c_int64, ctypes.POINTER(ctypes.c_void_p)]),
    "east_hip_reset": (ctypes.c_int, [ctypes.c_void_p]),
    "east_hip_destroy": (None, [ctypes.c_void_p]),
    "east_hip_build": (ctypes.c_int, [ctypes.c_void_p, _c_u32p, ctypes.c_int64, _c_i64p, _c_i32p, ctypes.c_int32]),
# ... 87 lines not shown
    "east_hip_cosine_set_classes": (ctypes.c_int, [ctypes.c_void_p, _c_i32p, ctypes.c_int32]),
    "east_hip_cosine_lookup": (ctypes.c_int, [ctypes.c_void_p, _c_u32p, _c_i64p, ctypes.c_int32, _c_i32p]),
    "east_hip_cosine_score_table": (ctypes.c_int, [ctypes.c_void_p, _c_i32p, _c_i64p, ctypes.c_int64, ctypes.c_int32,
                                                   ctypes.c_int32, _c_dblp]),
    "east_hip_debug_set_term_hash_bits": (ctypes.c_int, [ctypes.c_int]),
    "east_hip_graph_build_resident": (ctypes.c_int, [ctypes.c_void_p, ctypes.c_int32, _c_i32p, ctypes.c_int64, ctypes.c_double,
                                                     ctypes.c_double, ctypes.c_double, _c_i64p]),
    "east_hip_graph_build_host": (ctypes.c_int, [ctypes.c_void_p, _c_dblp, ctypes.c_int32, ctypes.c_int32, _c_i32p,
                                                 ctypes.c_int64, ctypes.c_double, ctypes.c_double, ctypes.c_double, _c_i64p]),
    "east_hip_graph_fetch": (ctypes.c_int, [ctypes.c_void_p] + [_c_i32p] * 5),
    "east_hip_last_graph_ms": (ctypes.c_double, [ctypes.c_void_p]),
    "east_hip_synonyms_build": (ctypes.c_int, [ctypes.c_void_p, _c_i32p, _c_i32p, _c_i32p, ctypes.c_int64, _c_i32p,
                                               ctypes.c_int32, ctypes.c_int32]),
    "east_hip_synonyms_info": (ctypes.c_int, [ctypes.c_void_p, _c_i64p, ctypes.c_int32]),
    "east_hip_synonyms_get_rows": (ctypes.c_int, [ctypes.c_void_p, _c_i64p, _c_i32p, _c_i32p, _c_dblp, _c_dblp]),
    "east_hip_synonyms_similarity": (ctypes.c_int, [ctypes.c_void_p, _c_i32p, _c_i32p, ctypes.c_int64, _c_dblp]),
    "east_hip_synonyms_pairs": (ctypes.c_int, [ctypes.c_void_p, _c_i32p, ctypes.c_int32, ctypes.c_double, _c_i64p]),
    "east_hip_synonyms_fetch": (ctypes.c_int, [ctypes.c_void_p, _c_i32p, _c_i32p, _c_dblp]),
    "east_hip_last_synonyms_ms": (ctypes.c_double, [ctypes.c_void_p]),
    "east_hip_debug_set_synonyms_chunk": (ctypes.c_int, [ctypes.c_int]),
    "east_hip_top_build_resident": (ctypes.c_int, [ctypes.c_void_p, ctypes.c_int32, ctypes.c_int32, ctypes.c_int32,
                                                   ctypes.c_double, _c_i64p]),
    "east_hip_top_build_host": (ctypes.c_int, [ctypes.c_void_p, _c_dblp, ctypes.c_int32, ctypes.c_int32, ctypes.c_int32,
                                               ctypes.c_int32, ctypes.c_double, _c_i64p]),
    "east_hip_top_fetch": (ctypes.c_int, [ctypes.c_void_p, _c_i32p, _c_i32p, _c_dblp]),
    "east_hip_last_top_ms": (ctypes.c_double, [ctypes.c_void_p]),
    "east_hip_debug_set_top_tile": (ctypes.c_int, [ctypes.c_int]),
    "east_hip_similarity_build_resident": (ctypes.c_int, [ctypes.c_void_p, ctypes.c_int32, ctypes.c_int32, _c_i64p]),
    "east_hip_similarity_build_host": (ctypes.c_int, [ctypes.c_void_p, _c_dblp, ctypes.c_int32, ctypes.c_int32, ctypes.c_int32,
                                                      _c_i64p]),
    "east_hip_similarity_fetch": (ctypes.c_int, [ctypes.c_void_p, _c_dblp, _c_dblp]),
    "east_hip_last_similarity_ms": (ctypes.c_double, [ctypes.c_void_p]),
    "east_hip_related_build": (ctypes.c_int, [ctypes.c_void_p, ctypes.c_int, ctypes.c_int32, _c_i64p]),
    "east_hip_related_fetch": (ctypes.c_int, [ctypes.c_void_p, _c_dblp, _c_dblp, _c_i32p]),
    "east_hip_last_related_ms": (ctypes.c_double, [ctypes.c_void_p]),
    "east_hip_debug_set_related_chunk": (ctypes.c_int, [ctypes.c_int64]),
    "east_hip_text_similarity_build": (ctypes.c_int, [ctypes.c_void_p, ctypes.c_int32, _c_i64p]),
    "east_hip_text_similarity_fetch": (ctypes.c_int, [ctypes.c_void_p, _c_dblp, _c_dblp, _c_i32p]),
    "east_hip_last_text_similarity_ms": (ctypes.c_double, [ctypes.c_void_p]),
    "east_hip_debug_set_text_similarity_batch": (ctypes.c_int, [ctypes.c_int64]),
    "east_hip_clusters_build_resident": (ctypes.c_int, [ctypes.c_void_p, ctypes.c_int32, _c_i64p]),
    "east_hip_clusters_build_host": (ctypes.c_int, [ctypes.c_void_p, _c_dblp, ctypes.c_int32, _c_i64p]),
    "east_hip_clusters_fetch": (ctypes.c_int, [ctypes.c_void_p, _c_i32p, _c_i32p, _c_dblp]),
    "east_hip_clusters_cut_threshold": (ctypes.c_int, [ctypes.c_void_p, ctypes.c_double, _c_i32p, _c_i64p]),
    "east_hip_clusters_cut_count": (ctypes.c_int, [ctypes.c_void_p, ctypes.c_int32, _c_i32p, _c_i64p]),
    "east_hip_last_clusters_ms": (ctypes.c_double, [ctypes.c_void_p]),
}

BUILD_INFO_FIELDS = ("n_total", "n_docs", "n_strings", "sigma_text", "bits_level0", "dc3_levels", "arena_bytes",
                     "arena_high_water", "radix_passes", "radix_elements", "radix_element_bytes",
                     "radix_passes_u32", "radix_elements_u32", "radix_passes_u64", "radix_elements_u64",
                     "dc3_levels_resolved", "merge_elements", "refine_rounds", "window_sorted", "lds_sorted",
                     "fused_finish", "first_kept", "first_n", "ht_keys", "seg_sort", "narrow_upload", "persist_rounds",
                     "first_hist_fused")
COSINE_INFO_FIELDS = ("built", "n_docs", "kept_tokens", "words", "terms", "classes", "postings", "hash_attempts", "build_us",
                      "score_us")

GRAPH_SOURCE_AST, GRAPH_SOURCE_COSINE, GRAPH_SOURCE_UPLOADED = 0, 1, 2
GRAPH_SOURCE_SIMILARITY = 3
GRAPH_SOURCE_RELATED = 4
GRAPH_SOURCE_COSINE_TEXTS = 5
COSINE_TEXTS_CHUNK, COSINE_TEXTS_SEG = 32, 8192
COSINE_TEXTS_INFO_FIELDS = ("n_docs", "units", "postings", "tiles", "segments", "launches", "chunk_units", "segment_units")
CLUSTERS_INFO_FIELDS = ("members", "merges", "rounds", "launches")
RELATED_DIRECTED, RELATED_SYMMETRIC = 0, 1
TOP_BY_TEXT, TOP_BY_KEYPHRASE = 0, 1
TOP_MAX_N = 1024

_lib = None


def load():
    global _lib
    if _lib is None:
        if not os.path.exists(LIB_PATH):
            raise exceptions.HipBackendError(
                reason="%s not found -- build it with `make -C ast-text-analysis_amd/csrc` "
                       "(python -c 'import __graft_entry__ as g; g.build()'); there is no CPU fallback" % LIB_PATH)
        try:
            lib = ctypes.CDLL(LIB_PATH)
        except OSError as e:
            raise exceptions.HipBackendError(reason="cannot load %s: %s" % (LIB_PATH, e))
        for name, (res, args) in SIGNATURES.items():
            fn = getattr(lib, name)
            fn.restype = res
            fn.argtypes = args
        _lib = lib
    return _lib


def _check(rc):
    if rc != 0:
        msg = load().east_hip_last_error()
        raise exceptions.HipBackendError(reason="%s (code %d)" % (msg.decode("utf-8", "replace") if msg else "?", rc))


def _ptr(a, t):
    return a.ctypes.data_as(t)


def device_count():
    c = load().east_hip_device_count()
    return c if c > 0 else 0


def default_device():
    for var in ("EAST_HIP_DEVICE", "LOCAL_RANK"):
# ... 766 lines not shown
```

Baseline: 43.23 billion chars/s.

## Route terminator-led suffixes to a tail digit and skip them in level-0 refinement

Counts terminator bytes while building the first radix histogram and redirects suffixes that start with a terminator to a reserved tail digit. Those suffixes are written straight into their final slots at the end of the suffix array, and the later level-0 place, finish and refine stages run over fewer elements. The count is speculated from n_strings and checked afterwards; a mismatch forces a full rebuild without the tail path. This adds per-tile popcount work, extra branches in the scatter, and a risk of repeated builds when the guess is wrong.

```diff
diff --git a/ast-text-analysis_amd/csrc/alphabet.h b/ast-text-analysis_amd/csrc/alphabet.h
--- a/ast-text-analysis_amd/csrc/alphabet.h
+++ b/ast-text-analysis_amd/csrc/alphabet.h
@@ -46,6 +46,7 @@
 #define FLAG_PLACE_FAIL 6
 #define FLAG_KG_BAD 7
 #define FLAG_SAMPLE 8
+#define FLAG_TERM_TOTAL 25
 #define FLAG_WORDS 32
 #define STATUS_NO_TERMINATOR 1u
 #define STATUS_N_STRINGS 2u
diff --git a/ast-text-analysis_amd/csrc/build.h b/ast-text-analysis_amd/csrc/build.h
--- a/ast-text-analysis_amd/csrc/build.h
+++ b/ast-text-analysis_amd/csrc/build.h
@@ -175,6 +175,9 @@
     u32 *present = flags + FLAG_WORDS;
     if (!ctx.dry) HIP_CHECK(hipMemsetAsync(flags, 0, (ZEROED_WORDS + 3 * TOTAL_WORDS) * sizeof(u32), ctx.stream));
     ctx.zeroed_totals = ctx.dry ? nullptr : flags + ZEROED_WORDS + TOTAL_WORDS;
+    ctx.term_guess = !ctx.dry && ctx.knobs.term_tail && !ctx.no_tail && n_docs == 1 ? (u32)n_strings[0] : 0u;
+    ctx.term_total = ctx.dry ? nullptr : flags + FLAG_TERM_TOTAL;
+    ctx.did_tail = 0;
     RsFirstHist first_hist;
     ctx.first_hist = nullptr;
     const Ctx::FirstPassPlan fp = ctx.spec && ctx.knobs.first_hist && n_docs == 1 && !tagged ? h->first_plan : Ctx::FirstPassPlan();
@@ -202,15 +205,17 @@
             first_hist.s8 = h->s8;
             first_hist.key_bytes = fp.key_bytes; first_hist.w = fp.w; first_hist.b = fp.b; first_hist.spare = fp.spare;
             first_hist.term_first = fp.term_first; first_hist.shift = fp.shift; first_hist.mask = fp.mask;
+            TextWindowGen<u64> gen64{h->s8, n, fp.w, fp.b, fp.spare, fp.term_first, DocKey()};
+            TextWindowGen<u32> gen32{h->s8, n, fp.w, fp.b, fp.spare, fp.term_first, DocKey()};
+            first_hist.tail = ctx.term_guess != 0 && lvl0_digit255_free(fp.w, fp.b, fp.spare, fp.term_first, fp.shift, fp.mask);
+            gen64.tail.on = gen32.tail.on = first_hist.tail;
             if (fp.key_bytes == 8)
                 LAUNCH_NAMED(ctx, "presence_remap_hist_kernel", (presence_remap_hist_kernel<u64, TextWindowGen<u64>>), first_hist.n_groups,
-                             d_sym, n, h->guess.as<const u32>(), present, h->s8,
-                             TextWindowGen<u64>{h->s8, n, fp.w, fp.b, fp.spare, fp.term_first, DocKey()}, fp.shift, fp.mask,
+                             d_sym, n, h->guess.as<const u32>(), present, h->s8, gen64, fp.shift, fp.mask,
                              first_hist.n_tiles, first_hist.hist, first_hist.group_sum, first_hist.digit_total);
             else
                 LAUNCH_NAMED(ctx, "presence_remap_hist_kernel", (presence_remap_hist_kernel<u32, TextWindowGen<u32>>), first_hist.n_groups,
-                             d_sym, n, h->guess.as<const u32>(), present, h->s8,
-                             TextWindowGen<u32>{h->s8, n, fp.w, fp.b, fp.spare, fp.term_first, DocKey()}, fp.shift, fp.mask,
+                             d_sym, n, h->guess.as<const u32>(), present, h->s8, gen32, fp.shift, fp.mask,
                              first_hist.n_tiles, first_hist.hist, first_hist.group_sum, first_hist.digit_total);
             ctx.first_hist = &first_hist;
         } else if (fused) LAUNCH(ctx, presence_remap_kernel, std::min<u32>(gn, 2048), d_sym, n, h->guess.as<const u32>(), present, h->s8);
@@ -578,10 +583,18 @@
     const bool went_through = run(speculate, spec_rounds);
     const bool repeat = speculate && (!went_through || (flags[FLAG_STATUS] & STATUS_SIGMA_GUESS) ||
                                       (spec_rounds && (flags[FLAG_KEEP] || flags[FLAG_FAIL] || flags[FLAG_PLACE_FAIL])));
-    if (repeat) {
-        if (g_trace) fprintf(stderr, "[east_hip] speculative build guessed wrong: building again\n");
+    auto tail_missed = [&]() { return ctx.did_tail && flags[FLAG_TERM_TOTAL] != ctx.term_guess; };
+    const bool missed = went_through && tail_missed() && !(flags[FLAG_STATUS] & STATUS_NO_TERMINATOR);
+    if (repeat || missed) {
+        if (g_trace) fprintf(stderr, "[east_hip] %s: building again\n", missed ? "n_strings is not the number of terminators" : "speculative build guessed wrong");
+        ctx.no_tail = missed && !repeat;
         h->stats = Stats();
         run(false, false);
+        if (!ctx.no_tail && tail_missed() && !(flags[FLAG_STATUS] & STATUS_NO_TERMINATOR)) {
+            ctx.no_tail = true;
+            h->stats = Stats();
+            run(false, false);
+        }
     }
     const bool map_confirmed = speculate && !repeat && ctx.map_checked;
     const u32 status = flags[FLAG_STATUS];
diff --git a/ast-text-analysis_amd/csrc/common.h b/ast-text-analysis_amd/csrc/common.h
--- a/ast-text-analysis_amd/csrc/common.h
+++ b/ast-text-analysis_amd/csrc/common.h
@@ -112,6 +112,7 @@
     i64 seg_sort = 0;
     i64 persist_rounds = 0;
     i64 first_hist_fused = 0;
+    i64 excluded_suffixes = 0;
 };
 
 struct Profiler {
@@ -175,6 +176,7 @@
     bool force_wide_keys = getenv("EAST_HIP_WIDE_KEYS") != nullptr;
     bool fused_finish = getenv("EAST_HIP_NO_FUSED_FINISH") == nullptr;
     bool force_fused = getenv("EAST_HIP_FORCE_FUSED") != nullptr;
+    bool term_tail = getenv("EAST_HIP_NO_TERM_TAIL") == nullptr;
     int ht_mode = env_int("EAST_HIP_HT", -1);
     int seg_mode = env_int("EAST_HIP_SEG", -1);
     bool lds_rounds = getenv("EAST_HIP_NO_LDS_ROUNDS") == nullptr;
@@ -234,6 +236,10 @@
         int key_bytes = 0, w = 0, b = 0, spare = 0, shift = 0;
         u32 term_first = 0, mask = 0;
     } did_first;
+    u32 term_guess = 0;
+    u32 *term_total = nullptr;
+    int did_tail = 0;
+    bool no_tail = false;
     u32 *kg_bad = nullptr;
     u32 sample_n = 0, sample_dup2[9] = {0}, sample_dup4[9] = {0};
     u32 rep_n = 0, rep_dup = 0;
diff --git a/ast-text-analysis_amd/csrc/debug_api.h b/ast-text-analysis_amd/csrc/debug_api.h
--- a/ast-text-analysis_amd/csrc/debug_api.h
+++ b/ast-text-analysis_amd/csrc/debug_api.h
@@ -201,6 +201,7 @@
     k.fused_finish = enabled != 4 && enabled != 5 && enabled != 9 && getenv("EAST_HIP_NO_FUSED_FINISH") == nullptr;
     k.force_fused = enabled == 6 || getenv("EAST_HIP_FORCE_FUSED") != nullptr;
     k.ht_mode = enabled == 7 || enabled == 9 ? 1 : enabled == 8 ? 0 : env_int("EAST_HIP_HT", -1);
+    k.term_tail = enabled != 10 && getenv("EAST_HIP_NO_TERM_TAIL") == nullptr;
     k.plan_epoch++;
     });
     return EAST_HIP_OK;
diff --git a/ast-text-analysis_amd/csrc/east_hip.hip b/ast-text-analysis_amd/csrc/east_hip.hip
--- a/ast-text-analysis_amd/csrc/east_hip.hip
+++ b/ast-text-analysis_amd/csrc/east_hip.hip
@@ -332,16 +332,16 @@
 int east_hip_build_info(east_hip_handle_t h, int64_t *out, int32_t cap)
 {
     if (!h || !out) return EAST_HIP_ERR_INVALID;
-    const int64_t v[28] = {h->n, h->n_docs, h->m_total, h->sigma_t, h->bits0, h->stats.levels,
+    const int64_t v[29] = {h->n, h->n_docs, h->m_total, h->sigma_t, h->bits0, h->stats.levels,
                            (int64_t)h->arena.cap, (int64_t)h->arena.high, h->stats.radix_passes,
                            h->stats.radix_elems, h->stats.radix_elem_bytes, h->stats.radix_passes_u32,
                            h->stats.radix_elems_u32, h->stats.radix_passes_u64, h->stats.radix_elems_u64,
                            h->stats.levels_resolved, h->stats.merge_elems, h->stats.refine_rounds,
                            h->stats.window_sorted, h->stats.lds_sorted, h->stats.fused_finish, h->stats.first_kept,
                            h->stats.first_n, h->stats.ht_keys, h->stats.seg_sort, h->narrow_upload,
-                           h->stats.persist_rounds, h->stats.first_hist_fused};
-    for (int i = 0; i < 28 && i < cap; i++) out[i] = v[i];
-    return 28;
+                           h->stats.persist_rounds, h->stats.first_hist_fused, h->stats.excluded_suffixes};
+    for (int i = 0; i < 29 && i < cap; i++) out[i] = v[i];
+    return 29;
 }
 
 int east_hip_profile_enable(east_hip_handle_t h, int on)
diff --git a/ast-text-analysis_amd/csrc/persist_rounds.h b/ast-text-analysis_amd/csrc/persist_rounds.h
--- a/ast-text-analysis_amd/csrc/persist_rounds.h
+++ b/ast-text-analysis_amd/csrc/persist_rounds.h
@@ -32,12 +32,12 @@
 };
 
 __global__ __launch_bounds__(BLOCK) void persist_names_init_kernel(const u32 *__restrict__ order_g, const u32 *__restrict__ alt,
-                                                                   const u64 *__restrict__ keep, u32 n,
+                                                                   const u64 *__restrict__ keep, u32 n, u32 n_sorted,
                                                                    u32 *__restrict__ name0, u32 *__restrict__ name1)
 {
     const u32 i = blockIdx.x * BLOCK + threadIdx.x;
     if (i >= n) return;
-    const u32 e = alt && ((keep[i >> 6] >> (i & 63u)) & 1u) ? alt[i] : order_g[i];
+    const u32 e = alt && i < n_sorted && ((keep[i >> 6] >> (i & 63u)) & 1u) ? alt[i] : order_g[i];
     name0[e] = i;
     name1[e] = i;
 }
diff --git a/ast-text-analysis_amd/csrc/radix_sort.h b/ast-text-analysis_amd/csrc/radix_sort.h
--- a/ast-text-analysis_amd/csrc/radix_sort.h
+++ b/ast-text-analysis_amd/csrc/radix_sort.h
@@ -43,6 +43,15 @@
     base = seg.doc_off[d] + t_in * (u32)RS_TILE;
     count = base < end ? (end - base < (u32)RS_TILE ? end - base : (u32)RS_TILE) : 0u;
 }
+
+struct RsTermTail {
+    bool on = false;
+    u32 *total = nullptr;
+    u32 *order_g = nullptr, *lcp_g = nullptr;
+    u32 n = 0, guess = 0;
+};
+#define RS_TAIL_DIGIT 255u
+template <class Gen> static inline RsTermTail rs_term_tail_of(const Gen &) { return RsTermTail(); }
 
 template <class K> struct PairSrc {
     static constexpr int MODE = 0;
@@ -146,6 +155,7 @@
 #define RS_GEN_RUN 8
 struct RsFirstHist {
     u32 *hist = nullptr, *group_sum = nullptr, *digit_total = nullptr;
+    bool tail = false;
     const uint8_t *s8 = nullptr;
     u32 n = 0, n_tiles = 0, n_groups = 0;
     int key_bytes = 0, w = 0, b = 0, spare = 0;
@@ -171,6 +181,8 @@
     __shared__ u32 bins[RS_GROUP][RS_HIST_COPIES][RS_BINS];
     __shared__ __attribute__((aligned(16))) u32 tab[TEXT_SYMBOLS / 2];
     __shared__ __attribute__((aligned(16))) u32 bytes[UW][(SUB + RS_FIRST_HALO) / 4];
+    __shared__ u32 tile_terms[RS_GROUP];
+    if (threadIdx.x < RS_GROUP) tile_terms[threadIdx.x] = 0;
     typedef uint16_t __attribute__((may_alias)) tab16_t;
     const tab16_t *tab16 = reinterpret_cast<const tab16_t *>(tab);
 #pragma unroll
@@ -234,6 +246,8 @@
         }
     };
     u32 tile = t0 + wave_id(), part = 0;
+    const bool tail_on = gen.tail.on;
+    u32 terms = 0;
     if (tile < t1) request(tile, 0);
     while (tile < t1) {
         const u32 g0 = tile * (u32)(RS_TILE / 4) + part * (u32)(SUB / 4) + lane;
@@ -246,6 +260,7 @@
             if (gi < n4) { v = word(q[j]); out[gi] = v; }
             else v = word_slow(gi);
             mine_bytes[(u32)j * WAVE + lane] = v;
+            terms += (u32)__popc(((v & 0x7F7F7F7Fu) + 0x01010101u) & v & 0x80808080u);
         }
         if (lane < RS_FIRST_HALO / 4u) {
             const u32 gi = (base + (u32)SUB) / 4u + lane;
@@ -275,6 +290,11 @@
             for (int qq = 0; qq < RS_GEN_RUN; qq++)
                 if (r0 + qq < count) radix_hist_add<false>(mine, (u32)(k[qq] >> shift) & mask);
         }
+        if (tail_on && next_part == 0u) {
+            terms = wave_sum(terms);
+            if (lane == 0) tile_terms[tile - t0] = terms;
+            terms = 0;
+        }
         __builtin_amdgcn_fence(__ATOMIC_RELEASE, "wavefront");
         __builtin_amdgcn_wave_barrier();
         tile = next_tile;
@@ -286,12 +306,15 @@
         else if (j < n + 16u) s8[j] = 0;
     }
     syncthreads_after_lds_atomics();
+    const bool term_bin = tail_on && threadIdx.x == ((u32)(gen.term_key() >> shift) & mask);
     u32 run = 0;
 #pragma unroll
     for (int k = 0; k < RS_GROUP; k++) {
         if (t0 + k < t1) hist[(size_t)(t0 + k) * RS_BINS + threadIdx.x] = run;
 #pragma unroll
         for (int c = 0; c < RS_HIST_COPIES; c++) run += bins[k][c][threadIdx.x];
+        if (term_bin) run -= tile_terms[k];
+        if (tail_on && threadIdx.x == RS_TAIL_DIGIT) run += tile_terms[k];
     }
     group_sum[(size_t)g * RS_BINS + threadIdx.x] = run;
     if (run) atomicAdd(&digit_total[(size_t)(g % RS_TOTAL_SHARDS) * RS_BINS + threadIdx.x], run);
@@ -314,7 +337,7 @@
 __global__ __launch_bounds__(BLOCK) void radix_spine_kernel(const u32 *__restrict__ group_sum, u32 n_groups,
                                                             const u32 *__restrict__ digit_total,
                                                             u32 *__restrict__ next_total, u32 *__restrict__ group_prefix,
-                                                            RsSeg seg)
+                                                            RsSeg seg, RsTermTail tail = RsTermTail())
 {
     static_assert(RS_BINS == BLOCK, "one digit per thread in the scan of the totals");
     __shared__ u32 base_of[RS_BINS];
@@ -330,6 +353,16 @@
         for (u32 k = 0; k < shards; k++) t += digit_total[row0 + k * RS_BINS + threadIdx.x];
         u32 total;
         base_of[threadIdx.x] = block_exclusive_sum(t, lds4, total) + (seg.n_docs ? seg.doc_off[doc] : 0u);
+        if (tail.on && blockIdx.x == 0) {
+            __shared__ u32 tail_m;
+            if (threadIdx.x == RS_TAIL_DIGIT) { tail_m = t; *tail.total = t; }
+            __syncthreads();
+            if (tail_m < tail.guess && tail.guess <= tail.n)
+                for (u32 j = tail.n - tail.guess + threadIdx.x; j < tail.n - tail_m; j += BLOCK) {
+                    tail.order_g[j] = 0;
+                    if (tail.lcp_g) tail.lcp_g[j] = 0;
+                }
+        }
         if (blockIdx.x == 0)
             for (u32 k = 0; k < shards; k++) next_total[row0 + k * RS_BINS + threadIdx.x] = 0;
     }
@@ -408,7 +441,7 @@
     u32 wsum[RS_THREADS / WAVE];
 };
 
-template <class K, class Src, bool FULL>
+template <class K, class Src, bool FULL, bool TAIL = false>
 __device__ __forceinline__ void radix_scatter_tile(ScatterLds<K> &lds, const Src &src, K *__restrict__ keys_out,
                                                    u32 *__restrict__ vals_out, int shift, u32 mask,
                                                    const u32 *__restrict__ hist, const u32 *__restrict__ group_prefix,
@@ -416,6 +449,11 @@
 {
     constexpr int WAVES = RS_THREADS / WAVE, IPT = RS_IPT, THREADS = RS_THREADS, BINS = RS_BINS, DB = RS_DB;
     constexpr int WAVE_ITEMS = WAVE * IPT;
+    auto digit_of = [&](K k) -> u32 {
+        const u32 d = (u32)(k >> shift) & mask;
+        if constexpr (TAIL) return src.term_led(k) ? RS_TAIL_DIGIT : d;
+        else return d;
+    };
     u32 *s_vals = reinterpret_cast<u32 *>(lds.s_keys);
     const u32 tid = threadIdx.x, lane = lane_id(), w = wave_id();
 
@@ -457,7 +495,7 @@
     for (int j = 0; j < IPT; j++) {
         const u32 local = w * WAVE_ITEMS + j * WAVE + lane;
         const bool valid = FULL || local < tile_count;
-        const u32 digit = (u32)(key[j] >> shift) & mask;
+        const u32 digit = digit_of(key[j]);
         u32 diff_lo = 0, diff_hi = 0;
 #pragma unroll
         for (int bit = 0; bit < DB; bit++) {
@@ -516,20 +554,22 @@
     for (int j = 0; j < IPT; j++) {
         const u32 local = w * WAVE_ITEMS + j * WAVE + lane;
         if (FULL || local < tile_count) {
-            const u32 digit = (u32)(key[j] >> shift) & mask;
+            const u32 digit = digit_of(key[j]);
             slot[j] = lds.digit_start[digit] + ((lds.wave_cnt[w][digit >> 1] >> ((digit & 1u) * 16u)) & 0xFFFFu) + slot[j];
             lds.s_keys[slot[j]] = key[j];
         }
     }
     __syncthreads();
     u32 dst[IPT];
+    u32 tail_rows = 0;
 #pragma unroll
     for (int j = 0; j < IPT; j++) {
         const u32 pos = j * THREADS + tid;
         if (FULL || pos < tile_count) {
             const K k = lds.s_keys[pos];
-            dst[j] = lds.global_base[(u32)(k >> shift) & mask] + pos;
+            dst[j] = lds.global_base[digit_of(k)] + pos;
             keys_out[dst[j]] = k;
+            if constexpr (TAIL) tail_rows |= src.term_led(k) ? 1u << j : 0u;
         }
     }
     __syncthreads();
@@ -542,7 +582,16 @@
 #pragma unroll
     for (int j = 0; j < IPT; j++) {
         const u32 pos = j * THREADS + tid;
-        if (FULL || pos < tile_count) vals_out[dst[j]] = s_vals[pos];
+        if (FULL || pos < tile_count) {
+            const u32 v = s_vals[pos];
+            vals_out[dst[j]] = v;
+            if constexpr (TAIL) {
+                if (((tail_rows >> j) & 1u) && dst[j] < src.tail.n) {
+                    src.tail.order_g[dst[j]] = v;
+                    if (src.tail.lcp_g) src.tail.lcp_g[dst[j]] = 0;
+                }
+            }
+        }
     }
 }
 
@@ -558,6 +607,17 @@
     rs_tile_range(seg, n, tile, tile_base, tile_count);
     if (tile_count == 0) return;
     __shared__ ScatterLds<K> lds;
+    if constexpr (Src::MODE == 2) {
+        if constexpr (Src::HAS_TAIL) {
+            if (src.tail.on) {
+                if (tile_count == (u32)RS_TILE)
+                    radix_scatter_tile<K, Src, true, true>(lds, src, keys_out, vals_out, shift, mask, hist, group_prefix, tile, tile_base, tile_count);
+                else
+                    radix_scatter_tile<K, Src, false, true>(lds, src, keys_out, vals_out, shift, mask, hist, group_prefix, tile, tile_base, tile_count);
+                return;
+            }
+        }
+    }
     if (tile_count == (u32)RS_TILE)
         radix_scatter_tile<K, Src, true>(lds, src, keys_out, vals_out, shift, mask, hist, group_prefix, tile, tile_base, tile_count);
     else
@@ -593,8 +653,9 @@
 {
     constexpr bool HAS_GEN = !std::is_same<Gen, NoGen>::value;
     if (n == 0 || bits <= begin_bit) return 0;
-    const u32 n_groups = seg.n_docs ? seg.n_groups : ceil_div_u32(ceil_div_u32(n, RS_TILE), RS_GROUP);
-    const u32 n_tiles = seg.n_docs ? n_groups * RS_GROUP : ceil_div_u32(n, RS_TILE);
+    u32 n_groups = seg.n_docs ? seg.n_groups : ceil_div_u32(ceil_div_u32(n, RS_TILE), RS_GROUP);
+    u32 n_tiles = seg.n_docs ? n_groups * RS_GROUP : ceil_div_u32(n, RS_TILE);
+    const RsTermTail tail = HAS_GEN && !seg.n_docs ? rs_term_tail_of(gen) : RsTermTail();
     const size_t total_words = seg.n_docs ? (size_t)seg.n_docs * seg.shards * RS_BINS : (size_t)RS_TOTAL_SHARDS * RS_BINS;
     const size_t mark = ctx.arena->mark();
     u32 *hist = ctx.arena->alloc<u32>((size_t)RS_BINS * n_tiles);
@@ -610,7 +671,8 @@
     if constexpr (HAS_GEN) {
         counted = pre && !ctx.dry && !seg.n_docs && pre->hist && pre->key_bytes == (int)sizeof(K) && pre->n == n &&
                   pre->n_tiles == n_tiles && pre->n_groups == n_groups && pre->shift == begin_bit &&
-                  pre->mask == (1u << std::min(RS_DB, bits - begin_bit)) - 1u && rs_first_hist_counted_for(*pre, gen);
+                  pre->mask == (1u << std::min(RS_DB, bits - begin_bit)) - 1u && rs_first_hist_counted_for(*pre, gen) &&
+                  pre->tail == tail.on;
     }
     if (counted && ctx.stats) ctx.stats->first_hist_fused = 1;
     int cur = 0, pass = 0;
@@ -652,10 +714,10 @@
                 LAUNCH(ctx, radix_spine_docs_kernel, seg.n_docs, (const u32 *)group_sum_p, (const u32 *)tot, tot_next, group_prefix, seg);
             if (seg.n_big)
                 LAUNCH(ctx, radix_spine_kernel, dim3(RS_BINS / RS_SPINE_COLS, seg.n_big), (const u32 *)group_sum_p, n_groups,
-                       (const u32 *)tot, tot_next, group_prefix, seg);
+                       (const u32 *)tot, tot_next, group_prefix, seg, RsTermTail());
         } else {
             LAUNCH(ctx, radix_spine_kernel, dim3(RS_BINS / RS_SPINE_COLS, 1u), (const u32 *)group_sum_p, n_groups, (const u32 *)tot,
-                   tot_next, group_prefix, seg);
+                   tot_next, group_prefix, seg, first ? tail : RsTermTail());
         }
         if (!ctx.dry) {
             if (prof) ctx.prof->begin(name_scatter, ctx.stream);
@@ -673,6 +735,12 @@
         }
         cur = out;
         radix_account(ctx, sizeof(K), n, first);
+        if (first && tail.on) {
+            n -= tail.guess;
+            n_tiles = ceil_div_u32(n, RS_TILE);
+            n_groups = ceil_div_u32(n_tiles, RS_GROUP);
+            if (n == 0) break;
+        }
         first = false;
     }
     ctx.arena->release(mark);
diff --git a/ast-text-analysis_amd/csrc/window_sort.h b/ast-text-analysis_amd/csrc/window_sort.h
--- a/ast-text-analysis_amd/csrc/window_sort.h
+++ b/ast-text-analysis_amd/csrc/window_sort.h
@@ -103,6 +103,16 @@
     reinterpret_cast<uint2 *>(km.kg)[(size_t)d * (km.bins + 1) + code] = uint2{jl, v};
     const int top3 = top + b;
     if (j == 0 || jl == 0 || (K)(k >> top3) != (K)(kp >> top3)) km.kg3[(size_t)d * (km.bins / km.A + 1) + code / km.A] = jl;
+}
+
+__device__ __forceinline__ void kg_mark_tail(const KgMark &km, u32 j, u32 v)
+{
+    u32 code = km.A - 1u;
+    for (int q = 1; q < km.k; q++) code *= km.A;
+    if (code >= km.bins) return;
+    if (!km.pairs) { km.kg[code] = j; return; }
+    reinterpret_cast<uint2 *>(km.kg)[code] = uint2{j, v};
+    km.kg3[code / km.A] = j;
 }
 
 __global__ __launch_bounds__(BLOCK) void doc_tiles_kernel(const u32 *__restrict__ doc_off, u32 n_docs, u32 n_tiles,
@@ -192,8 +202,12 @@
     int w, b, spare;
     u32 term_first;
     DocKey docs;
+    static constexpr bool HAS_TAIL = true;
+    RsTermTail tail;
 
     __device__ __forceinline__ void prepare() const {}
+    __device__ __forceinline__ bool term_led(K k) const { return (u32)(k >> (spare + (w - 1) * b)) == term_first; }
+    __device__ __forceinline__ K term_key() const { return (K)term_first << (spare + (w - 1) * b); }
     template <int RUN = TW_RUN>
     __device__ __forceinline__ void keys_of_run(const u32 (&x)[6], K (&out)[RUN]) const
     {
@@ -266,6 +280,8 @@
     template <bool CHECK = true> __device__ __forceinline__ void hist_tile(u32 *mine, u32 e0, u32 e1, int shift, u32 mask) const
     {
         const bool need_docs = docs.bits && w * b + spare < shift + 12;
+        const bool tail_on = tail.on;
+        u32 terms = 0;
         for (u32 p0 = e0 + lane_id() * TW_RUN; p0 < e1; p0 += WAVE * TW_RUN) {
             u32 x[6];
             K k[TW_RUN];
@@ -273,9 +289,13 @@
             keys_of_run(x, k);
             if (need_docs) add_docs(p0, k);
 #pragma unroll
-            for (int q = 0; q < TW_RUN; q++)
-                if (p0 + q < e1) radix_hist_add<CHECK>(mine, (u32)(k[q] >> shift) & mask);
-        }
+            for (int q = 0; q < TW_RUN; q++) {
+                if (p0 + q >= e1) continue;
+                if (tail_on && term_led(k[q])) terms++;
+                else radix_hist_add<CHECK>(mine, (u32)(k[q] >> shift) & mask);
+            }
+        }
+        if (tail_on && terms) atomicAdd(&mine[RS_TAIL_DIGIT], terms);
     }
 };
 
@@ -285,6 +305,8 @@
     return !g.docs.bits && !g.docs.seg.n_docs && p.s8 == g.s8 && p.n == g.n && p.key_bytes == (int)sizeof(K) && p.w == g.w &&
            p.b == g.b && p.spare == g.spare && p.term_first == g.term_first;
 }
+
+template <class K> static inline RsTermTail rs_term_tail_of(const TextWindowGen<K> &g) { return g.tail; }
 
 __device__ __forceinline__ u32 *ht_enc_lds()
 {
@@ -299,6 +321,7 @@
     int sb;
     const u32 *enc;
     DocKey docs;
+    static constexpr bool HAS_TAIL = false;
 
     __device__ __forceinline__ void prepare() const
     {
@@ -370,6 +393,28 @@
         }
     }
 };
+
+static bool lvl0_digit255_free(int w, int b, int spare, u32 term_first, int shift, u32 mask)
+{
+    if (mask != 255u || term_first <= 1u) return true;
+    const int lo = shift, hi = shift + 8;
+    auto ones = [&](int pos, int width, u32 c_max, int drop) {
+        const int a = std::max(pos, lo), e = std::min(pos + width, hi);
+        const u32 pm = (1u << (e - a)) - 1u;
+        for (u32 c = 1; c <= c_max; c++)
+            if ((((c >> drop) >> (a - pos)) & pm) == pm) return true;
+        return false;
+    };
+    auto inside = [&](int pos, int width) { return std::max(pos, lo) < std::min(pos + width, hi); };
+    for (int q = 0; q < w; q++) {
+        const int pos = spare + (w - 1 - q) * b;
+        if (!inside(pos, b)) continue;
+        const bool lowest = pos <= lo && !(spare > 0 && inside(0, spare));
+        if (!ones(pos, b, lowest && q > 0 ? term_first : term_first - 1u, 0)) return true;
+    }
+    if (spare > 0 && inside(0, spare) && !ones(0, spare, term_first, b - spare)) return true;
+    return false;
+}
 
 static int lvl0_spare_bits(int used, int key_bits, int bt, int w)
 {
@@ -615,11 +660,13 @@
                                                           u64 *__restrict__ keep, u32 *__restrict__ block_keep,
                                                           u32 *__restrict__ fail, LongRepeats lr_arg, KgMark km,
                                                           uint8_t *__restrict__ xdep0 = nullptr, SegRanks sr = SegRanks(),
-                                                          u32 *__restrict__ spec_keep = nullptr)
+                                                          u32 *__restrict__ spec_keep = nullptr,
+                                                          u32 tail = 0)
 {
     const LongRepeats lr = OPTIMISTIC ? LongRepeats() : lr_arg;
     constexpr u32 limit = ENDGAME_LIMITS ? REFINE_ENDGAME_GROUP : REFINE_SMALL_GROUP;
     constexpr u32 max_len = ENDGAME_LIMITS ? REFINE_ENDGAME_LEN : RESOLVE_MAX_LEN;
+    if (OPTIMISTIC && km.kg && tail && blockIdx.x == 0 && threadIdx.x == 0) kg_mark_tail(km, m, order_g[m]);
     __shared__ u32 keep_bits[BLOCK * PLACE_IPT / 32];
     __shared__ u32 work[BLOCK * PLACE_IPT];
     __shared__ u64 next8[BLOCK * PLACE_IPT];
@@ -881,6 +928,7 @@
     const K *keys;
     const u32 *vals;
     u32 m;
+    u32 tail = 0;
     const uint8_t *s8;
     int w, b, spare, low_bits;
     u32 inv_b;
@@ -1029,6 +1077,7 @@
     const KeyNeqWindowIn<K> hf{a.keys, a.rep_t, a.ones, a.highs, a.ht_sb, a.ht_wmin, a.ht_dec};
     u32 *comp = next4;
     const u32 m = a.m;
+    if (a.tail && a.km.kg && blockIdx.x == 0 && threadIdx.x == 0) kg_mark_tail(a.km, m, a.order_g[m]);
     const u32 c0 = blockIdx.x * FIN_CHUNK;
     const u32 base = c0 - FIN_LEFT;
     const int L = a.low_bits;
@@ -1728,13 +1777,25 @@
         LAUNCH(ctx, doc_tiles_kernel, ceil_div_u32(n_dt, BLOCK), docs.doc_off, docs.n_docs, n_dt, tile_doc);
         docs.tile_doc = tile_doc;
     }
+    const bool tail_on = n0 == 0 && !ht && !docs.bits && !docs.seg.n_docs && allow_fused && ctx.knobs.term_tail && !ctx.dry &&
+                         ctx.term_total && ctx.term_guess > 0 && ctx.term_guess <= n02 &&
+                         lvl0_digit255_free(w, bt, spare, term_first, low_bits, (1u << std::min(RS_DB, total_bits - low_bits)) - 1u);
+    TextWindowGen<K> text_gen{s8, n02, w, bt, spare, term_first, docs};
+    if (tail_on) {
+        RsTermTail &tl = text_gen.tail;
+        tl.on = true; tl.total = ctx.term_total; tl.order_g = sa12; tl.lcp_g = lcp_out; tl.n = n02; tl.guess = ctx.term_guess;
+    }
+    const u32 ns = tail_on ? n02 - ctx.term_guess : n02;
+    if (n0 == 0 && !ctx.dry) {
+        ctx.did_tail = tail_on;
+        if (ctx.stats) ctx.stats->excluded_suffixes = tail_on ? ctx.term_guess : 0;
+    }
     const int r = n0 ? radix_sort_pairs<K, WindowSrc<K>>(ctx, sb, n02, total_bits, 0,
                                                          WindowSrc<K>{s8, n0, w, bt, spare, term_first, docs})
                 : ht ? radix_sort_pairs<K, HtWindowGen<K>>(ctx, sb, n02, total_bits, low_bits,
                                                            HtWindowGen<K>{s8, n02, ht_sb, ht->enc, docs},
                                                            docs.bits ? total_bits - docs.bits : total_bits + RS_DB, docs.seg)
-                     : radix_sort_pairs<K, TextWindowGen<K>>(ctx, sb, n02, total_bits, low_bits,
-                                                             TextWindowGen<K>{s8, n02, w, bt, spare, term_first, docs},
+                     : radix_sort_pairs<K, TextWindowGen<K>>(ctx, sb, n02, total_bits, low_bits, text_gen,
                                                              docs.bits ? total_bits - docs.bits : total_bits + RS_DB, docs.seg,
                                                              ctx.first_hist);
     if (n0 == 0 && !ctx.dry) {
@@ -1753,7 +1814,7 @@
     u32 *fail = ar.alloc<u32>(1);
     const bool fail_is_zero = ctx.zeroed_word != nullptr;
     if (fail_is_zero) { fail = ctx.zeroed_word; ctx.zeroed_word = nullptr; }
-    const u32 gp = ceil_div_u32((u64)n02 + 1, BLOCK * PLACE_IPT);
+    const u32 gp = ceil_div_u32((u64)ns + 1, BLOCK * PLACE_IPT);
     u32 *block_keep = ar.alloc<u32>(gp);
     const u32 nb = ceil_div_u32(gp, SCAN_TILE);
     u32 *block_sums = ar.alloc<u32>(nb);
@@ -1778,11 +1839,11 @@
         if (km.pairs) clear_add(ctx, clears, km.kg3, (size_t)(km.bins / km.A + 1) * km.n_docs * sizeof(u32), 0xFF);
         *kg_mark = km;
     }
-    u32 m = n02, m_next = n02, h_fail = 0;
+    u32 m = ns, m_next = ns, h_fail = 0;
     FinishArgs<K> fa;
     const SegRanks sr{docs.seg.n_docs ? docs.seg.doc_off : nullptr, docs.seg.n_docs};
     if (fused) {
-        fa.keys = sb.keys[r]; fa.vals = sorted_vals; fa.m = n02; fa.s8 = s8;
+        fa.keys = sb.keys[r]; fa.vals = sorted_vals; fa.m = ns; fa.tail = n02 - ns; fa.s8 = s8;
         fa.w = w; fa.b = bt; fa.spare = spare; fa.low_bits = low_bits;
         fa.inv_b = (65536u + (u32)bt - 1u) / (u32)bt;
         fa.rep_t = starts.rep_t; fa.ones = starts.ones; fa.highs = starts.highs;
@@ -1795,8 +1856,8 @@
         fa.km = small_input ? KgMark() : km;
         if (ht) { fa.ht_sb = ht_sb; fa.ht_wmin = w; fa.ht_dec = ht->dec; fa.xdep0 = xdep0; }
         if (sr.n_docs) { fa.km.by_rank = 1; fa.km.doc_off = sr.doc_off; fa.km.n_docs = sr.n_docs; }
-        clear_add(ctx, clears, keep, (((size_t)n02 >> 6) + 2) * sizeof(u64), 0);
-        clear_add(ctx, clears, gstart_bits, (((size_t)n02 >> 6) + 2) * sizeof(u64), 0);
+        clear_add(ctx, clears, keep, (((size_t)ns >> 6) + 2) * sizeof(u64), 0);
+        clear_add(ctx, clears, gstart_bits, (((size_t)ns >> 6) + 2) * sizeof(u64), 0);
     }
     clear_run(ctx, clears);
     const bool spec_direct = ctx.spec_rounds && n0 == 0 && !ctx.dry && ctx.spec_out && fail_is_zero && fail == ctx.spec_fail;
@@ -1817,23 +1878,23 @@
             else if (sg) LAUNCH_NAMED(ctx, "lvl0_finish_kernel", (lvl0_finish_kernel<K, false, 64, false, true>), gp, fa);
             else LAUNCH_NAMED(ctx, "lvl0_finish_kernel", (lvl0_finish_kernel<K, false, 64>), gp, fa);
         } else if (ht && small_input)
-            LAUNCH_NAMED(ctx, "lvl0_place_kernel", (lvl0_place_kernel<K, true, false, true>), gp, starts, sorted_vals, n02, s8, n0, w,
-                         bt, spare, sa12, names_g, lcp_out, keep, block_keep, fail, LongRepeats{bad, mode}, KgMark(), xdep0, sr, spec_keep);
+            LAUNCH_NAMED(ctx, "lvl0_place_kernel", (lvl0_place_kernel<K, true, false, true>), gp, starts, sorted_vals, ns, s8, n0, w,
+                         bt, spare, sa12, names_g, lcp_out, keep, block_keep, fail, LongRepeats{bad, mode}, KgMark(), xdep0, sr, spec_keep, n02 - ns);
         else if (ht && mode == 0)
-            LAUNCH_NAMED(ctx, "lvl0_place_kernel", (lvl0_place_kernel<K, false, true, true>), gp, starts, sorted_vals, n02, s8, n0, w,
-                         bt, spare, sa12, names_g, lcp_out, keep, block_keep, fail, LongRepeats{bad, mode}, KgMark(), xdep0, sr, spec_keep);
+            LAUNCH_NAMED(ctx, "lvl0_place_kernel", (lvl0_place_kernel<K, false, true, true>), gp, starts, sorted_vals, ns, s8, n0, w,
+                         bt, spare, sa12, names_g, lcp_out, keep, block_keep, fail, LongRepeats{bad, mode}, KgMark(), xdep0, sr, spec_keep, n02 - ns);
         else if (ht)
-            LAUNCH_NAMED(ctx, "lvl0_place_kernel", (lvl0_place_kernel<K, false, false, true>), gp, starts, sorted_vals, n02, s8, n0, w,
-                         bt, spare, sa12, names_g, lcp_out, keep, block_keep, fail, LongRepeats{bad, mode}, KgMark(), xdep0, sr, spec_keep);
+            LAUNCH_NAMED(ctx, "lvl0_place_kernel", (lvl0_place_kernel<K, false, false, true>), gp, starts, sorted_vals, ns, s8, n0, w,
+                         bt, spare, sa12, names_g, lcp_out, keep, block_keep, fail, LongRepeats{bad, mode}, KgMark(), xdep0, sr, spec_keep, n02 - ns);
         else if (small_input)
-            LAUNCH_NAMED(ctx, "lvl0_place_kernel", (lvl0_place_kernel<K, true, false>), gp, starts, sorted_vals, n02, s8, n0, w,
-                         bt, spare, sa12, names_g, lcp_out, keep, block_keep, fail, LongRepeats{bad, mode}, KgMark(), (uint8_t *)nullptr, sr, spec_keep);
+            LAUNCH_NAMED(ctx, "lvl0_place_kernel", (lvl0_place_kernel<K, true, false>), gp, starts, sorted_vals, ns, s8, n0, w,
+                         bt, spare, sa12, names_g, lcp_out, keep, block_keep, fail, LongRepeats{bad, mode}, KgMark(), (uint8_t *)nullptr, sr, spec_keep, n02 - ns);
         else if (mode == 0)
-            LAUNCH_NAMED(ctx, "lvl0_place_kernel", (lvl0_place_kernel<K, false, true>), gp, starts, sorted_vals, n02, s8, n0, w,
-                         bt, spare, sa12, names_g, lcp_out, keep, block_keep, fail, LongRepeats{bad, mode}, km, (uint8_t *)nullptr, sr, spec_keep);
+            LAUNCH_NAMED(ctx, "lvl0_place_kernel", (lvl0_place_kernel<K, false, true>), gp, starts, sorted_vals, ns, s8, n0, w,
+                         bt, spare, sa12, names_g, lcp_out, keep, block_keep, fail, LongRepeats{bad, mode}, km, (uint8_t *)nullptr, sr, spec_keep, n02 - ns);
         else
-            LAUNCH_NAMED(ctx, "lvl0_place_kernel", (lvl0_place_kernel<K, false, false>), gp, starts, sorted_vals, n02, s8, n0, w,
-                         bt, spare, sa12, names_g, lcp_out, keep, block_keep, fail, LongRepeats{bad, mode}, KgMark(), (uint8_t *)nullptr, sr, spec_keep);
+            LAUNCH_NAMED(ctx, "lvl0_place_kernel", (lvl0_place_kernel<K, false, false>), gp, starts, sorted_vals, ns, s8, n0, w,
+                         bt, spare, sa12, names_g, lcp_out, keep, block_keep, fail, LongRepeats{bad, mode}, KgMark(), (uint8_t *)nullptr, sr, spec_keep, n02 - ns);
         if (mode == 1 || ctx.dry) return;
         if (ctx.spec_rounds && mode == 0 && n0 == 0) {
             if (!spec_direct)
@@ -1850,7 +1911,7 @@
         HIP_CHECK(sync_stream(ctx.stream));
         m_next = 0;
         for (u32 x : h_sums) m_next += x;
-        if (ctx.stats && n0 == 0 && mode == 0) { ctx.stats->first_kept = m_next; ctx.stats->first_n = n02; }
+        if (ctx.stats && n0 == 0 && mode == 0) { ctx.stats->first_kept = m_next; ctx.stats->first_n = ns; }
         if (g_trace)
             fprintf(stderr, "[east_hip] level-0 (%s, %u elements, w = %d): %u in large groups%s\n", n0 ? "sample" : "all suffixes",
                     n02, w, m_next, h_fail ? ", a repeat too long to order directly" : "");
@@ -1862,7 +1923,7 @@
         if (fused) throw FusedAbort();
         long_repeats = true;
         if (ctx.stats) ctx.stats->long_repeats++;
-        LAUNCH(ctx, (dc3_refine_restore_kernel<KeyNeqWindowIn<K>>), g02, sorted_vals, starts, (const u32 *)nullptr, n02, sa12,
+        LAUNCH(ctx, (dc3_refine_restore_kernel<KeyNeqWindowIn<K>>), g02, sorted_vals, starts, (const u32 *)nullptr, ns, sa12,
                names_g);
         HIP_CHECK(hipMemsetAsync(fail, 0, sizeof(u32), ctx.stream));
         HIP_CHECK(hipMemsetAsync(bad, 0, (((size_t)n02 >> 5) + 2) * sizeof(u32), ctx.stream));
@@ -1967,7 +2028,7 @@
                 u32 *name1 = (u32 *)rb.keys[0], *ctl = rb.vals[0];
                 HIP_CHECK(hipMemsetAsync(ctl, 0, PR_CTL_WORDS * sizeof(u32), ctx.stream));
                 LAUNCH(ctx, persist_names_init_kernel, ceil_div_u32(n02, BLOCK), (const u32 *)sa12,
-                       !slot && !fused ? sorted_vals : (const u32 *)nullptr, (const u64 *)keep, n02, name_of, name1);
+                       !slot && !fused ? sorted_vals : (const u32 *)nullptr, (const u64 *)keep, n02, ns, name_of, name1);
                 const int name_bits = bit_width_u32(n02 > 1 ? n02 - 1 : 1);
                 const PrArgs pa{ebuf[e_c], gstart, slot_c, m, depth, name_bits, name_of, name1, sa12, lcp_redo ? lcp_out : (u32 *)nullptr, ctl};
                 const u32 tiles = ceil_div_u32(m, LG_CHUNK);
diff --git a/ast-text-analysis_amd/east/hip_backend.py b/ast-text-analysis_amd/east/hip_backend.py
--- a/ast-text-analysis_amd/east/hip_backend.py
+++ b/ast-text-analysis_amd/east/hip_backend.py
@@ -163,7 +163,7 @@
                      "radix_passes_u32", "radix_elements_u32", "radix_passes_u64", "radix_elements_u64",
                      "dc3_levels_resolved", "merge_elements", "refine_rounds", "window_sorted", "lds_sorted",
                      "fused_finish", "first_kept", "first_n", "ht_keys", "seg_sort", "narrow_upload", "persist_rounds",
-                     "first_hist_fused")
+                     "first_hist_fused", "excluded_suffixes")
 COSINE_INFO_FIELDS = ("built", "n_docs", "kept_tokens", "words", "terms", "classes", "postings", "hash_attempts", "build_us",
                       "score_us")
 
```

Result: no change. 43.65 billion chars/s, median of 6 (+1.0%).
